# meffmadd/intro-tc-vae

Hardware: AMD Instinct MI355X
Metric: images/sec (64x64x3, z=128, bs=64) intro-TC step (higher is better)
Workload: dtype f32 in/out/accumulate, conv products on split-fp16 MFMA (two scaled fp16 planes, 3 products, fp32-class)

## Files before the change

intro-tc-vae_amd/csrc/abi.hip:

```cpp
#include "conv_shared.h"

#include <vector>

namespace itcv {
thread_local char g_err[512] = "";

struct ProfRec {
  int code;
  double flop;
  hipEvent_t start, stop;
};
static bool g_prof_on = false;
static std::vector<ProfRec> g_prof;

static thread_local int g_prof_depth = 0;
ProfScope::ProfScope(hipStream_t stream, ProfKind kind, int ks, int bm, int up2, int ns, double flop) : st(stream), slot(-1) {
  if (++g_prof_depth > 1 || !g_prof_on) return;
  ProfRec r;
  r.code = kind | (ks << 4) | (bm << 8) | (up2 << 16) | (ns << 20);
  r.flop = flop;
  if (hipEventCreate(&r.start) != hipSuccess || hipEventCreate(&r.stop) != hipSuccess) return;
  g_prof.push_back(r);
  slot = (int)g_prof.size() - 1;
  g_prof_start = r.start, g_prof_stop = r.stop;
}
ProfScope::~ProfScope() {
  if (--g_prof_depth > 0) return;
  if (slot >= 0 && g_prof_start) {
    (void)hipEventDestroy(g_prof[slot].start);
    (void)hipEventDestroy(g_prof[slot].stop);
    g_prof.pop_back();
  }
  g_prof_start = g_prof_stop = nullptr;
}
thread_local hipEvent_t g_prof_start = nullptr, g_prof_stop = nullptr;
Options g_opt;
extern int g_sw_lds_rows, g_sw_max_blocks;
}

extern "C" {
int itcv_abi_version(void) { return ITCV_ABI_VERSION; }

int itcv_set_option(const char* name, int value) {
  if (!name) return itcv::fail("%s: null option name", "itcv_set_option");
  if (!strcmp(name, "band_m16")) {
    if (value != 0 && value != 1) return itcv::fail("%s: band_m16 takes 0 or 1 (got %lld)", "itcv_set_option", value);
    itcv::g_opt.band_m16 = value;
    return 0;
  }
  if (!strcmp(name, "band_persist_blocks")) {
    if (value < 0 || value > 1024) return itcv::fail("%s: band_persist_blocks takes 0..1024 (got %lld)", "itcv_set_option", value);
    itcv::g_opt.band_persist_blocks = value;
    return 0;
  }
  if (!strcmp(name, "wgrad_m16")) {
    if (value != 0 && value != 1) return itcv::fail("%s: wgrad_m16 takes 0 or 1 (got %lld)", "itcv_set_option", value);
    itcv::g_opt.wgrad_m16 = value;
    return 0;
  }
  if (!strcmp(name, "planes_mfma_waves")) {
    if (value != 4 && value != 8) return itcv::fail("%s: planes_mfma_waves takes 4 or 8 (got %lld)", "itcv_set_option", value);
    itcv::g_opt.planes_mfma_waves = value;
    return 0;
  }
  if (!strcmp(name, "sw_lds_rows")) {
    if (value < 0 || value > 4096) return itcv::fail("%s: sw_lds_rows takes 0..4096 (got %lld)", "itcv_set_option", value);
    itcv::g_sw_lds_rows = value;
    return 0;
  }
  if (!strcmp(name, "sw_max_blocks")) {
    if (value < 0 || value > 1024) return itcv::fail("%s: sw_max_blocks takes 0..1024 (got %lld)", "itcv_set_option", value);
    itcv::g_sw_max_blocks = value;
    return 0;
  }
  return itcv::fail("%s: unknown option", "itcv_set_option");
}
int itcv_get_option(const char* name) {
  if (name && !strcmp(name, "band_m16")) return itcv::g_opt.band_m16;
  if (name && !strcmp(name, "band_persist_blocks")) return itcv::g_opt.band_persist_blocks;
  if (name && !strcmp(name, "wgrad_m16")) return itcv::g_opt.wgrad_m16;
  if (name && !strcmp(name, "planes_mfma_waves")) return itcv::g_opt.planes_mfma_waves;
  if (name && !strcmp(name, "sw_lds_rows")) return itcv::g_sw_lds_rows;
  if (name && !strcmp(name, "sw_max_blocks")) return itcv::g_sw_max_blocks;
  return -1;
}
const char* itcv_last_error(void) { return itcv::g_err; }

int itcv_profile_begin(void) {
  itcv::g_prof.clear();
  itcv::g_prof_on = true;
  return 0;
}
int itcv_profile_end(void) {
  itcv::g_prof_on = false;
  for (auto& r : itcv::g_prof) (void)hipEventSynchronize(r.stop);
  return (int)itcv::g_prof.size();
}
int itcv_profile_get(int i, int* code, double* flop, float* ms) {
  if (i < 0 || i >= (int)itcv::g_prof.size()) return itcv::fail("%s: index out of range", "itcv_profile_get");
  const auto& r = itcv::g_prof[i];
  *code = r.code;
  *flop = r.flop;
  if (hipEventElapsedTime(ms, r.start, r.stop) != hipSuccess) *ms = -1.f;
  return 0;
}
int itcv_profile_clear(void) {
  for (auto& r : itcv::g_prof) {
    (void)hipEventDestroy(r.start);
    (void)hipEventDestroy(r.stop);
  }
  itcv::g_prof.clear();
  return 0;
}
}
```

intro-tc-vae_amd/csrc/common.h:

```cpp
#pragma once
#include <hip/hip_runtime.h>
#include <hip/hip_ext.h>
#include <float.h>
#include <math.h>
#include <stdint.h>
#include <stdio.h>
#include <string.h>

#include <type_traits>

#include "../../include/itcv_hip.h"

namespace itcv {

extern thread_local char g_err[512];

inline int fail(const char* fmt, const char* a = "", long long b = 0, long long c = 0) {
  snprintf(g_err, sizeof(g_err), fmt, a, b, c);
  return 1;
}

#define ITCV_CHECK_LAUNCH(name)                                                        \
  do {                                                                                 \
    hipError_t e_ = hipGetLastError();                                                 \
    if (e_ != hipSuccess) return itcv::fail("%s: launch failed: %lld", name, (long long)e_); \
  } while (0)

#define ITCV_REQUIRE(cond, name)                                              \
  do {                                                                        \
    if (!(cond)) return itcv::fail("%s: requirement failed: " #cond, name);   \
  } while (0)

inline bool finite(double x) { return fabs(x) <= DBL_MAX; }

inline int need_pointers(const char* name, bool all) { return all ? 0 : fail("%s: a required pointer is NULL", name); }
inline int need_dim(const char* name, const char* what, long long v, long long lo, long long hi, const char* range) {
  if (v >= lo && v <= hi) return 0;
  char fmt[128];
  snprintf(fmt, sizeof(fmt), "%%s: %s is outside %s", what, range);
  return fail(fmt, name, v);
}
inline int need_stride(const char* name, const char* whose, size_t ld, const char* dim, long long width) {
  if (ld >= (size_t)width) return 0;
  char fmt[128];
  snprintf(fmt, sizeof(fmt), "%%s: %s row stride of %%lld is below %s = %%lld", whose, dim);
  return fail(fmt, name, (long long)ld, width);
}

inline hipStream_t S(void* s) { return reinterpret_cast<hipStream_t>(s); }

__host__ __device__ inline int cdiv(int a, int b) { return (a + b - 1) / b; }
inline size_t cdivz(size_t a, size_t b) { return (a + b - 1) / b; }
inline size_t align_up(size_t a, size_t b) { return cdivz(a, b) * b; }

constexpr int kWave = 64;

inline int stream_grid(size_t n, int per_thread) {
  size_t b = cdivz(cdivz(n, per_thread), 256);
  return (int)(b > 2048 ? 2048 : (b < 1 ? 1 : b));
}

template <typename T>
__device__ __forceinline__ T wave_sum(T v) {
#pragma unroll
  for (int o = 32; o > 0; o >>= 1) v += __shfl_xor(v, o, 64);
  return v;
}
template <typename T>
__device__ __forceinline__ T wave_max(T v) {
#pragma unroll
  for (int o = 32; o > 0; o >>= 1) {
    T u = __shfl_xor(v, o, 64);
    v = u > v ? u : v;
  }
  return v;
}
template <typename T>
__device__ __forceinline__ T wave_min(T v) {
#pragma unroll
  for (int o = 32; o > 0; o >>= 1) {
    T u = __shfl_xor(v, o, 64);
    v = u < v ? u : v;
  }
  return v;
}
template <typename T>
__device__ __forceinline__ T block_sum(T v, T* scratch) {
  const int lane = threadIdx.x & 63, wid = threadIdx.x >> 6, nw = (blockDim.x + 63) >> 6;
  v = wave_sum(v);
  __syncthreads();
  if (lane == 0) scratch[wid] = v;
  __syncthreads();
  T r = 0;
  for (int i = 0; i < nw; ++i) r += scratch[i];
  return r;
}

__device__ __forceinline__ __amdgpu_buffer_rsrc_t make_rsrc(const void* p, uint32_t num_bytes) {
  return __builtin_amdgcn_make_buffer_rsrc(const_cast<void*>(p), 0, num_bytes, 0x00020000);
}
__device__ __forceinline__ float buf_load(__amdgpu_buffer_rsrc_t r, uint32_t byte_off) {
  return __builtin_bit_cast(float, __builtin_amdgcn_raw_buffer_load_b32(r, byte_off, 0, 0));
}
constexpr uint32_t kOOB = 0xFFFFFFFFu;

template <typename T>
__device__ __forceinline__ T fold_strided(T init, const T* __restrict__ p, size_t stride, int n) {
  T s = init;
  int k = 0;
  for (; k + 8 <= n; k += 8) {
    T v[8];
#pragma unroll
    for (int u = 0; u < 8; ++u) v[u] = p[(size_t)(k + u) * stride];
#pragma unroll
    for (int u = 0; u < 8; ++u) s += v[u];
  }
  for (; k + 2 <= n; k += 2) {
    const T v0 = p[(size_t)k * stride], v1 = p[(size_t)(k + 1) * stride];
    s += v0;
    s += v1;
  }
  for (; k < n; ++k) s += p[(size_t)k * stride];
  return s;
}

typedef __bf16 bf16x8 __attribute__((ext_vector_type(8)));
typedef _Float16 f16x8 __attribute__((ext_vector_type(8)));
typedef unsigned int u32x4 __attribute__((ext_vector_type(4)));

struct ScaleRec {
  float scale, inv;
  float pad[2];
};
constexpr int kWeightScaleLog2 = 8;

__host__ __device__ inline float scale_for_bound(float bound) {
  if (!(bound > 0.f) || !(bound < 3.0e38f)) return 1.f;
  int e;
  (void)frexpf(bound, &e);
  int k = 15 - e;
  k = k > 126 ? 126 : (k < -126 ? -126 : k);
  return ldexpf(1.f, k);
}

template <int NS, bool F16 = false>
__device__ __forceinline__ void split8(const float (&v)[8], u32x4 (&out)[NS], float scale = 1.f) {
  if constexpr (F16) {
    static_assert(NS == 2, "fp16 planes come in pairs");
    f16x8 hi, lo;
#pragma unroll
    for (int j = 0; j < 8; ++j) {
      const float r = v[j] * scale;
      const _Float16 h = (_Float16)r;
      hi[j] = h;
      lo[j] = (_Float16)(r - (float)h);
    }
    out[0] = __builtin_bit_cast(u32x4, hi), out[1] = __builtin_bit_cast(u32x4, lo);
  } else {
    bf16x8 pl[NS];
#pragma unroll
    for (int j = 0; j < 8; ++j) {
      float r = v[j];
#pragma unroll
      for (int p = 0; p < NS; ++p) {
        const __bf16 b = (__bf16)r;
        pl[p][j] = b;
        r -= (float)b;
      }
    }
#pragma unroll
    for (int p = 0; p < NS; ++p) out[p] = __builtin_bit_cast(u32x4, pl[p]);
  }
}

typedef float mm_f32x4 __attribute__((ext_vector_type(4)));
typedef float mm_f32x16 __attribute__((ext_vector_type(16)));
template <bool F16>
__device__ __forceinline__ mm_f32x4 mma16x16x32(bf16x8 a, bf16x8 b, mm_f32x4 c) {
  if constexpr (F16)
    return __builtin_amdgcn_mfma_f32_16x16x32_f16(__builtin_bit_cast(f16x8, a), __builtin_bit_cast(f16x8, b), c, 0, 0, 0);
  else
    return __builtin_amdgcn_mfma_f32_16x16x32_bf16(a, b, c, 0, 0, 0);
}
template <bool F16>
__device__ __forceinline__ mm_f32x16 mma32x32x16(bf16x8 a, bf16x8 b, mm_f32x16 c) {
  if constexpr (F16)
    return __builtin_amdgcn_mfma_f32_32x32x16_f16(__builtin_bit_cast(f16x8, a), __builtin_bit_cast(f16x8, b), c, 0, 0, 0);
  else
    return __builtin_amdgcn_mfma_f32_32x32x16_bf16(a, b, c, 0, 0, 0);
}

__device__ __forceinline__ float inv_scale_of(const ScaleRec* r) {
  return __builtin_bit_cast(float, __builtin_amdgcn_readfirstlane(__builtin_bit_cast(int, r->inv)));
}

__device__ __forceinline__ float wave_absmax_of(const float* __restrict__ p, int n) {
  float m = 0.f;
  for (int i = threadIdx.x & 63; i < n; i += 64) m = fmaxf(m, p[i]);
#pragma unroll
  for (int o = 32; o > 0; o >>= 1) m = fmaxf(m, __shfl_xor(m, o, 64));
  return m;
}
constexpr int kAbsmaxParts = 256;

enum ProfKind : int {
  kProfFwd = 0,
  kProfFwdB = 1,
  kProfWgrad = 2,
  kProfWgradB = 3,
  kProfSmallCout = 4,
  kProfSmallCin = 5,
  kProfFwdP = 6,
  kProfWgradP = 7,
  kProfFwdBand = 8,
  kProfFwdBandPersist = 9,
  kProfSmallCoutP = 10,
  kProfSmallCinMfma = 11,
  kProfWgrad5 = 12,
  kProfBnFwd = 13,
  kProfBnBwd = 14,
};
struct ProfScope {
  hipStream_t st;
  int slot;
  ProfScope(hipStream_t stream, ProfKind kind, int ks, int bm, int up2, int ns, double flop);
  ~ProfScope();
};
extern thread_local hipEvent_t g_prof_start, g_prof_stop;

template <typename K, typename... Args>
inline void launch_timed(K kernel, dim3 grid, dim3 block, size_t lds, hipStream_t st, Args... args) {
  if (g_prof_start) {
    hipExtLaunchKernelGGL(kernel, grid, block, lds, st, g_prof_start, g_prof_stop, 0, args...);
    g_prof_start = nullptr;
  } else {
    hipLaunchKernelGGL(kernel, grid, block, lds, st, args...);
  }
}

template <auto Kernel, typename... Args>
inline void launch_lds(dim3 grid, dim3 block, size_t lds, hipStream_t st, Args... args) {
  static size_t have = 0;
  if (have < lds) {
    (void)hipFuncSetAttribute(reinterpret_cast<const void*>(Kernel), hipFuncAttributeMaxDynamicSharedMemorySize, (int)lds);
    have = lds;
  }
  launch_timed(Kernel, grid, block, lds, st, args...);
}

template <int N, typename F>
inline void pick(int v, F&& f) {
  if constexpr (N > 1) {
    if (v == N - 1) return f(std::integral_constant<int, N - 1>{});
    return pick<N - 1>(v, f);
  } else {
    f(std::integral_constant<int, 0>{});
  }
}
template <int V0, int... Vs, typename F>
inline void pick_of(int v, F&& f) {
  if constexpr (sizeof...(Vs) > 0) {
    if (v != V0) return pick_of<Vs...>(v, f);
  }
  f(std::integral_constant<int, V0>{});
}

}
```

intro-tc-vae_amd/csrc/conv_igemm.hip:

```cpp
#include <float.h>

#include "conv_shared.h"

namespace itcv {



constexpr uint32_t kOobBase = 0x80000000u;

__device__ __forceinline__ float buf_load_s(__amdgpu_buffer_rsrc_t r, uint32_t voff, uint32_t soff) {
  return __builtin_bit_cast(float, __builtin_amdgcn_raw_buffer_load_b32(r, voff, __builtin_amdgcn_readfirstlane(soff), 0));
}

__host__ __device__ inline int tile_rows_for(int M) { return M <= 32 ? 32 : (M <= 64 ? 64 : 128); }

struct ConvArgs {
  const float* x;
  const float* wp;
  const float* bias;
  float* y;
  int B, Ci, H, W, Co;
  int Cip, Mp, N;
  int mt, nt;
  int ktiles, ktiles_per_split, cpt;
// ... 1368 lines not shown
    const int lw = wid - 8;
    const int Hs = UP2 ? H / 2 : H, Ws = UP2 ? Wi / 2 : Wi, HWs = Hs * Ws;
    const int Co8 = a.Co >> 3, Ci8 = a.Ci >> 3, dh = dhi - 1;
    const u32x4* zero = &g_zero_chunk;
    const int hp = (lw & 1) * 64 + lane;
    const bool hp_active = hp < NP;
    const int R = hp / WP, w = hp - R * WP - 1;

    auto issue = [&](int st, int stage) {
      const uint32_t sbase = smem_base + (uint32_t)(stage * SSZ) * 16u;
      {
        const int g = st * 64 + lane, b = g / HW, pix = g - b * HW;
#pragma unroll
        for (int j = 0; j < 2 * ACH / NLW; ++j) {
          const int qq = j * NLW + lw, pl = qq / ACH, c8 = qq % ACH;
          const int gc8 = (co0 >> 3) + c8;
          const u32x4* src = a.dyp + ((size_t)pl * a.dyplane + ((size_t)b * Co8 + gc8) * HW + pix);
          lds_dma16(gc8 < Co8 ? src : zero, sbase + (uint32_t)((pl * ACH + c8) * PXA) * 16u);
        }
      }
      {
        const int gr = (st >> wsh) * NR + R, b = gr >> a.h_shift, h = gr & (H - 1), hh = h + dh;
        const int wi = ((st & ((1 << wsh) - 1)) << 6) + w;
        const bool valid = (unsigned)wi < (unsigned)Wi && (unsigned)hh < (unsigned)H;
        const int spix = UP2 ? (hh >> 1) * Ws + (wi >> 1) : hh * Wi + wi;
#pragma unroll
        for (int j = 0; j < 4 * BCH / NLW; ++j) {
          const int qq = (j * NLW + lw) >> 1, pl = qq / BCH, c8 = qq % BCH;
          const int gc8 = (ci0 >> 3) + c8;
          const u32x4* src = a.xp + ((size_t)pl * a.xplane + ((size_t)b * Ci8 + gc8) * HWs + spix);
          if (hp_active)
            lds_dma16((valid && gc8 < Ci8) ? src : zero,
                      sbase + (uint32_t)(ASZ + (pl * BCH + c8) * PXB + (lw & 1) * 64) * 16u);
        }
      }
    };
    constexpr int PST = 2 * ACH / NLW + 4 * BCH / NLW;
    issue(s0, 0);
    if (NST == 3 && s0 + 1 < s1) {
      issue(s0 + 1, 1);
      wait_vmcnt<PST>();
    } else {
      wait_vmcnt<0>();
    }
    __builtin_amdgcn_s_barrier();
    int stage = NST - 1;
    for (int st = s0; st < s1; ++st) {
      if (st + NST - 1 < s1) {
        issue(st + NST - 1, stage);
        if (NST == 3) wait_vmcnt<PST>();
        else wait_vmcnt<0>();
      } else {
        wait_vmcnt<0>();
      }
      if (++stage == NST) stage = 0;
      __builtin_amdgcn_s_barrier();
    }
    return;
  }

  const int kh = wid / (8 / KH), w8 = wid % (8 / KH);
  const int wm = w8 / WNn, wn = w8 % WNn;
  const int G = lane >> 4, i16 = lane & 15, q = i16 >> 2, pp = i16 & 3, half = G >> 1, rb = G & 1;
  const int l31 = lane & 31;
  if constexpr (M16) {
    typedef float f32x4m __attribute__((ext_vector_type(4)));
    constexpr int KP32 = 2 / KH;
    f32x4m acc[3][TNw][2][2];
#pragma unroll
    for (int tp = 0; tp < 3; ++tp)
#pragma unroll
      for (int j = 0; j < TNw; ++j)
#pragma unroll
        for (int bi = 0; bi < 2; ++bi)
#pragma unroll
          for (int bj = 0; bj < 2; ++bj) acc[tp][j][bi][bj] = f32x4m{0.f, 0.f, 0.f, 0.f};
    if (s0 < s1) {
      const uint32_t aoff = (uint32_t)(((4 * wm + (pp >> 1)) * PXA + G * 8 + q) * 16 + (pp & 1) * 8);
      const uint32_t boff = (uint32_t)((ASZ + (4 * wn * TNw + (pp >> 1)) * PXB) * 16 + (pp & 1) * 8);
      uint32_t hidx[2 * KP32];
#pragma unroll
      for (int u = 0; u < 2 * KP32; ++u) {
        const int k = ((u >> 1) + kh * KP32) * 32 + G * 8 + (u & 1) * 4 + q;
        hidx[u] = (uint32_t)(((k >> LOG2W) * WP + (k & (W - 1)) + 1) * 16);
      }
      __builtin_amdgcn_s_barrier();
      int stage = 0;
      for (int st = s0; st < s1; ++st) {
        const uint32_t sb = smem_base + (uint32_t)(stage * SSZ) * 16u;
        if constexpr (TNw == 1) {
          bf16x8 af[2][2][2], bfr[2][2];
          auto fetch_a = [&](int kk, int kb) {
#pragma unroll
            for (int bi = 0; bi < 2; ++bi)
#pragma unroll
              for (int pl = 0; pl < 2; ++pl) {
                const uint32_t ad = sb + aoff + (uint32_t)((pl * ACH + 2 * bi) * PXA * 16 + (kh * KP32 + kk) * 512);
                tr_read8(af[kb][bi][pl], ad, ad + 64);
              }
          };
          auto fetch_b = [&](int u, int ub) {
            const int kk = u / 6, tp = (u % 6) >> 1, bj = u & 1;
#pragma unroll
            for (int pl = 0; pl < 2; ++pl) {
              const uint32_t bd = sb + boff + (uint32_t)((pl * BCH + 2 * bj) * PXB * 16 + (tp - 1) * 16);
              tr_read8(bfr[ub][pl], bd + hidx[kk * 2], bd + hidx[kk * 2 + 1]);
            }
          };
          constexpr int NU = KP32 * 6;
          fetch_a(0, 0);
          fetch_b(0, 0);
#pragma unroll
          for (int u = 0; u < NU; ++u) {
            const int kk = u / 6, tp = (u % 6) >> 1, bj = u & 1, ub = u & 1, kb = kk & 1;
            if (u + 1 < NU) {
              if ((u + 1) % 6 == 0) fetch_a(kk + 1, kb ^ 1);
              fetch_b(u + 1, ub ^ 1);
            }
#pragma unroll
            for (int bi = 0; bi < 2; ++bi) {
              f32x4m c = acc[tp][0][bi][bj];
              c = mma16x16x32<F16>(af[kb][bi][0], bfr[ub][1], c);
              c = mma16x16x32<F16>(af[kb][bi][1], bfr[ub][0], c);
              c = mma16x16x32<F16>(af[kb][bi][0], bfr[ub][0], c);
              acc[tp][0][bi][bj] = c;
            }
          }
        } else {
#pragma unroll
        for (int kk = 0; kk < KP32; ++kk) {
          bf16x8 af[2][2];
#pragma unroll
          for (int bi = 0; bi < 2; ++bi)
#pragma unroll
            for (int pl = 0; pl < 2; ++pl) {
              const uint32_t ad = sb + aoff + (uint32_t)((pl * ACH + 2 * bi) * PXA * 16 + (kh * KP32 + kk) * 512);
              tr_read8(af[bi][pl], ad, ad + 64);
            }
#pragma unroll
          for (int tp = 0; tp < 3; ++tp)
#pragma unroll
            for (int j = 0; j < TNw; ++j)
#pragma unroll
              for (int bj = 0; bj < 2; ++bj) {
                bf16x8 bfr[2];
#pragma unroll
                for (int pl = 0; pl < 2; ++pl) {
                  const uint32_t bd = sb + boff + (uint32_t)((pl * BCH + 4 * j + 2 * bj) * PXB * 16 + (tp - 1) * 16);
                  tr_read8(bfr[pl], bd + hidx[kk * 2], bd + hidx[kk * 2 + 1]);
                }
#pragma unroll
                for (int bi = 0; bi < 2; ++bi) {
                  f32x4m c = acc[tp][j][bi][bj];
                  c = mma16x16x32<F16>(af[bi][0], bfr[1], c);
                  c = mma16x16x32<F16>(af[bi][1], bfr[0], c);
                  c = mma16x16x32<F16>(af[bi][0], bfr[0], c);
                  acc[tp][j][bi][bj] = c;
                }
              }
        }
        }
        if (++stage == NST) stage = 0;
        asm volatile("s_waitcnt lgkmcnt(0)" ::: "memory");
        __builtin_amdgcn_s_barrier();
      }
    }
    const float oscale = F16 ? inv_scale_of(a.xscale) * inv_scale_of(a.dyscale) : 1.f;
#pragma unroll
    for (int j = 0; j < TNw; ++j)
#pragma unroll
      for (int bj = 0; bj < 2; ++bj) {
        const int ci = ci0 + 32 * (wn * TNw + j) + 16 * bj + i16;
        if (ci >= a.Ci) continue;
#pragma unroll
        for (int tp = 0; tp < 3; ++tp) {
          float* out = a.slab + ((size_t)((split * KH + kh) * 9 + dhi * 3 + tp) * a.Co) * a.Ci + ci;
#pragma unroll
          for (int bi = 0; bi < 2; ++bi)
#pragma unroll
            for (int r = 0; r < 4; ++r) {
              const int co = co0 + 32 * wm + 16 * bi + 4 * G + r;
              if (co < a.Co) out[(size_t)co * a.Ci] = F16 ? acc[tp][j][bi][bj][r] * oscale : acc[tp][j][bi][bj][r];
            }
        }
      }
    return;
  }
  f32x16 acc[3][TNw];
#pragma unroll
  for (int tp = 0; tp < 3; ++tp)
#pragma unroll
    for (int j = 0; j < TNw; ++j)
#pragma unroll
      for (int r = 0; r < 16; ++r) acc[tp][j][r] = 0.f;
  if (s0 < s1) {
    const uint32_t aoff = (uint32_t)(((4 * wm + 2 * rb + (pp >> 1)) * PXA + half * 8 + q) * 16 + (pp & 1) * 8);
    const uint32_t boff = (uint32_t)((ASZ + (4 * wn * TNw + 2 * rb + (pp >> 1)) * PXB) * 16 + (pp & 1) * 8);
    uint32_t hidx16[2 * KPW];
#pragma unroll
    for (int u = 0; u < 2 * KPW; ++u) {
      const int k = ((u >> 1) + kh * KPW) * 16 + half * 8 + (u & 1) * 4 + q;
      hidx16[u] = (uint32_t)(((k >> LOG2W) * WP + (k & (W - 1)) + 1) * 16);
    }
    __builtin_amdgcn_s_barrier();
    int stage = 0;
    const long long dbg_c0 = ITCV_DBG(a) ? clock64() : 0;
    for (int st = s0; st < s1; ++st) {
      const uint32_t sb = smem_base + (uint32_t)(stage * SSZ) * 16u;
      if constexpr (TNw == 1) {
        bf16x8 af[2][2], bfr[2][3][2];
        auto fetch = [&](int kk, int bufi) {
#pragma unroll
          for (int pl = 0; pl < 2; ++pl) {
            const uint32_t ad = sb + aoff + (uint32_t)(pl * ACH * PXA * 16 + (kh * KPW + kk) * 256);
            tr_read8(af[bufi][pl], ad, ad + 64);
          }
#pragma unroll
          for (int tp = 0; tp < 3; ++tp)
#pragma unroll
            for (int pl = 0; pl < 2; ++pl) {
              const uint32_t bd = sb + boff + (uint32_t)(pl * BCH * PXB * 16 + (tp - 1) * 16);
              tr_read8(bfr[bufi][tp][pl], bd + hidx16[kk * 2], bd + hidx16[kk * 2 + 1]);
            }
        };
        fetch(0, 0);
#pragma unroll
        for (int kk = 0; kk < KPW; ++kk) {
          const int cur = kk & 1;
          if (kk + 1 < KPW) fetch(kk + 1, cur ^ 1);
#pragma unroll
          for (int tp = 0; tp < 3; ++tp) {
            f32x16 c = acc[tp][0];
            c = mma32x32x16<F16>(af[cur][0], bfr[cur][tp][1], c);
            c = mma32x32x16<F16>(af[cur][1], bfr[cur][tp][0], c);
            c = mma32x32x16<F16>(af[cur][0], bfr[cur][tp][0], c);
            acc[tp][0] = c;
          }
          if (kk == 0) __builtin_amdgcn_sched_group_barrier(0x100, 16, 0);
          if (kk + 1 < KPW) {
#pragma unroll
            for (int r = 0; r < 8; ++r) {
              __builtin_amdgcn_sched_group_barrier(0x008, 1, 0);
              __builtin_amdgcn_sched_group_barrier(0x100, 2, 0);
            }
            __builtin_amdgcn_sched_group_barrier(0x008, 1, 0);
          } else {
            __builtin_amdgcn_sched_group_barrier(0x008, 9, 0);
          }
        }
      } else {
      static_assert(TNw == 1 || KH == 1, "k-halves only with one accumulator column per wave");
#pragma unroll
      for (int kk = 0; kk < 4; ++kk) {
        bf16x8 af[2];
#pragma unroll
        for (int pl = 0; pl < 2; ++pl) {
          const uint32_t ad = sb + aoff + (uint32_t)(pl * ACH * PXA * 16 + kk * 256);
          tr_read8(af[pl], ad, ad + 64);
        }
#pragma unroll
        for (int tp = 0; tp < 3; ++tp)
#pragma unroll
          for (int j = 0; j < TNw; ++j) {
            bf16x8 bfr[2];
#pragma unroll
            for (int pl = 0; pl < 2; ++pl) {
              const uint32_t bd = sb + boff + (uint32_t)((pl * BCH + 4 * j) * PXB * 16 + (tp - 1) * 16);
              tr_read8(bfr[pl], bd + hidx16[kk * 2], bd + hidx16[kk * 2 + 1]);
            }
            f32x16 c = acc[tp][j];
            c = mma32x32x16<F16>(af[0], bfr[1], c);
            c = mma32x32x16<F16>(af[1], bfr[0], c);
            c = mma32x32x16<F16>(af[0], bfr[0], c);
            acc[tp][j] = c;
          }
      }
      }
      if (++stage == NST) stage = 0;
      asm volatile("s_waitcnt lgkmcnt(0)" ::: "memory");
      __builtin_amdgcn_s_barrier();
    }
    if (ITCV_DBG(a) && t == 0 && blockIdx.x == 0) {
      a.slab[0] = (float)(clock64() - dbg_c0), a.slab[1] = (float)(s1 - s0);
      return;
    }
  }
  const float oscale = F16 ? inv_scale_of(a.xscale) * inv_scale_of(a.dyscale) : 1.f;
#pragma unroll
  for (int j = 0; j < TNw; ++j) {
    const int ci = ci0 + 32 * (wn * TNw + j) + l31;
    if (ci >= a.Ci) continue;
#pragma unroll
    for (int tp = 0; tp < 3; ++tp) {
      float* out = a.slab + ((size_t)((split * KH + kh) * 9 + dhi * 3 + tp) * a.Co) * a.Ci + ci;
#pragma unroll
      for (int r = 0; r < 16; ++r) {
        const int co = co0 + 32 * wm + (r & 3) + 8 * (r >> 2) + 4 * (lane >> 5);
        if (co < a.Co) out[(size_t)co * a.Ci] = F16 ? acc[tp][j][r] * oscale : acc[tp][j][r];
      }
    }
  }
}

template <int SG, bool F16 = false>
__global__ __launch_bounds__(256) void conv_wgrad5_planes_kernel(const float* __restrict__ sm, const u32x4* __restrict__ tp,
                                                                float* __restrict__ slab, int B, int CS, int H, int W,
                                                                int rows_per_job, int njobs, size_t plane_stride,
                                                                const float* __restrict__ sm_amax) {
  constexpr int PXS = 68;
  constexpr int RSZ = 2 * 8 * PXS;
  __shared__ u32x4 rows[4][RSZ];
  const int lane = threadIdx.x & 63, wv = threadIdx.x >> 6;
  const int job = blockIdx.x * 4 + wv;
  if (job >= njobs) return;
  const int jobs_per_img = (H + rows_per_job - 1) / rows_per_job;
  const int b = job / jobs_per_img, h_lo = (job - b * jobs_per_img) * rows_per_job, h_hi = min(H, h_lo + rows_per_job);
  const size_t HW = (size_t)H * W;
  const int n = lane & 15, kg = lane >> 4;
  const int cs = n / 5, dw = n - cs * 5;
  const bool row_used = cs < CS;
  const int i16 = lane & 15, q = i16 >> 2, pp = i16 & 3;
  const uint32_t rbase = lds_addr(rows[wv]);
  float sscale = 1.f, oscale = 1.f;
  if constexpr (F16) {
    if (sm_amax) sscale = scale_for_bound(wave_absmax_of(sm_amax, kAbsmaxParts));
    oscale = inv_scale_of(reinterpret_cast<const ScaleRec*>(tp + 2 * plane_stride)) / sscale;
  }
  f32x4_t acc[5][4];
#pragma unroll
  for (int dh = 0; dh < 5; ++dh)
#pragma unroll
    for (int nt = 0; nt < 4; ++nt) acc[dh][nt] = f32x4_t{0.f, 0.f, 0.f, 0.f};

  for (int h = h_lo; h < h_hi; ++h) {
   for (int seg = 0; seg < W; seg += 64) {
    const int segw = min(64, W - seg);
    asm volatile("s_waitcnt lgkmcnt(0)" ::: "memory");
    if (lane < segw) {
#pragma unroll
      for (int pl = 0; pl < 2; ++pl)
#pragma unroll
        for (int c8 = 0; c8 < 8; ++c8)
          rows[wv][(pl * 8 + c8) * PXS + lane] =
              tp[(size_t)pl * plane_stride + ((size_t)b * 8 + c8) * HW + (size_t)h * W + seg + lane];
    }
    asm volatile("s_waitcnt vmcnt(0) lgkmcnt(0)" ::: "memory");
    for (int w0 = 0; w0 < segw; w0 += 32) {
      bf16x8 bfr[4][2];
#pragma unroll
      for (int nt = 0; nt < 4; ++nt)
#pragma unroll
        for (int pl = 0; pl < 2; ++pl) {
          const uint32_t ad = rbase + (uint32_t)(((pl * 8 + 2 * nt + (pp >> 1)) * PXS + w0 + 8 * kg + q) * 16 + (pp & 1) * 8);
          tr_read8(bfr[nt][pl], ad, ad + 64);
        }
      float sv[5][8];
      const int ws0 = seg + w0 + 8 * kg + SG * (dw - 2);
      const float* spc = sm + ((size_t)b * CS + (row_used ? cs : 0)) * HW;
#pragma unroll
      for (int dh = 0; dh < 5; ++dh) {
        const int hs = h + SG * (dh - 2);
        const float* sp = spc + (size_t)min(max(hs, 0), H - 1) * W;
#pragma unroll
        for (int j = 0; j < 8; ++j) sv[dh][j] = sp[min(max(ws0 + j, 0), W - 1)];
      }
#pragma unroll
      for (int dh = 0; dh < 5; ++dh) {
        const int hs = h + SG * (dh - 2);
        float v[8];
        const bool hok = row_used && (unsigned)hs < (unsigned)H;
#pragma unroll
        for (int j = 0; j < 8; ++j) v[j] = (hok && (unsigned)(ws0 + j) < (unsigned)W) ? sv[dh][j] : 0.f;
        u32x4 ap[2];
        split8<2, F16>(v, ap, sscale);
        const bf16x8 a0 = __builtin_bit_cast(bf16x8, ap[0]), a1 = __builtin_bit_cast(bf16x8, ap[1]);
#pragma unroll
        for (int nt = 0; nt < 4; ++nt) {
          f32x4_t c = acc[dh][nt];
          c = mma16x16x32<F16>(a0, bfr[nt][1], c);
          c = mma16x16x32<F16>(a1, bfr[nt][0], c);
          c = mma16x16x32<F16>(a0, bfr[nt][0], c);
          acc[dh][nt] = c;
        }
      }
    }
   }
  }
  float* out = slab + (size_t)job * 16 * 5 * 64;
#pragma unroll
  for (int dh = 0; dh < 5; ++dh)
#pragma unroll
    for (int nt = 0; nt < 4; ++nt)
#pragma unroll
      for (int i = 0; i < 4; ++i) out[((4 * kg + i) * 5 + dh) * 64 + nt * 16 + n] = F16 ? acc[dh][nt][i] * oscale : acc[dh][nt][i];
}

__global__ __launch_bounds__(256) void wgrad5_reduce(const float* __restrict__ slab, float* __restrict__ dwt, int CS,
                                                    int njobs, int stem, int accumulate) {
  __shared__ float part[16][17];
  const int e = threadIdx.x & 15, g = threadIdx.x >> 4;
  const int total = CS * 5 * 5 * 64, i = blockIdx.x * 16 + e;
  float s = 0.f;
  int dst = 0;
  if (i < total) {
    const int cb = i & 63, r = i >> 6, dh = r % 5, m = r / 5, cs = m / 5, dwi = m - cs * 5;
    const float* p = slab + (size_t)((m * 5 + dh) * 64 + cb);
    for (int k = g; k < njobs; k += 16 * 8) {
      float v[8];
#pragma unroll
      for (int u = 0; u < 8; ++u) v[u] = p[(size_t)min(k + 16 * u, njobs - 1) * (16 * 5 * 64)];
#pragma unroll
      for (int u = 0; u < 8; ++u) s += (k + 16 * u < njobs) ? v[u] : 0.f;
    }
    dst = stem ? ((cb * CS + cs) * 5 + dh) * 5 + dwi : ((cs * 64 + cb) * 5 + dh) * 5 + dwi;
  }
  part[g][e] = s;
  __syncthreads();
  if (g == 0 && i < total) {
    float t = accumulate ? dwt[dst] : 0.f;
#pragma unroll
    for (int k = 0; k < 16; ++k) t += part[k][e];
    dwt[dst] = t;
  }
}

struct WgReduceDesc {
  const float* slab[4];
  float* dw;
  int splits[4];
  int nsrc, coci, accumulate, block0, nblocks, fine;
};
static_assert(sizeof(WgReduceDesc) == 80, "WgReduceDesc layout is part of the ABI (itcv_wgrad_reduce_desc_bytes)");

__device__ __forceinline__ void wgrad_reduce_tile(const WgReduceDesc& d, int tile) {
  const int e = (tile * 256 + (int)threadIdx.x) * 4;
  if (e >= d.coci) return;
  const size_t plane = (size_t)d.coci, stride = 9 * plane;
  float* dwp = d.dw + (size_t)e * 9;
  const bool vec = ((size_t)dwp & 15) == 0;
  float tot[36];
  if (d.accumulate) {
    if (vec) {
#pragma unroll
      for (int q = 0; q < 9; ++q) {
        const float4 t = reinterpret_cast<const float4*>(dwp)[q];
        tot[4 * q] = t.x, tot[4 * q + 1] = t.y, tot[4 * q + 2] = t.z, tot[4 * q + 3] = t.w;
      }
    } else {
#pragma unroll
      for (int q = 0; q < 36; ++q) tot[q] = dwp[q];
    }
  } else {
#pragma unroll
    for (int q = 0; q < 36; ++q) tot[q] = 0.f;
  }
  for (int k = 0; k < d.nsrc; ++k) {
    const float* p = d.slab[k] + e;
    float acc[36];
#pragma unroll
    for (int q = 0; q < 36; ++q) acc[q] = 0.f;
    int sl = 0;
    for (; sl + 2 <= d.splits[k]; sl += 2) {
      float4 v[2][9];
#pragma unroll
      for (int u = 0; u < 2; ++u)
#pragma unroll
        for (int tp = 0; tp < 9; ++tp) v[u][tp] = *reinterpret_cast<const float4*>(p + (size_t)(sl + u) * stride + (size_t)tp * plane);
#pragma unroll
      for (int u = 0; u < 2; ++u)
#pragma unroll
        for (int tp = 0; tp < 9; ++tp)
          acc[tp] += v[u][tp].x, acc[9 + tp] += v[u][tp].y, acc[18 + tp] += v[u][tp].z, acc[27 + tp] += v[u][tp].w;
    }
    if (sl < d.splits[k]) {
      float4 v[9];
#pragma unroll
      for (int tp = 0; tp < 9; ++tp) v[tp] = *reinterpret_cast<const float4*>(p + (size_t)sl * stride + (size_t)tp * plane);
#pragma unroll
      for (int tp = 0; tp < 9; ++tp) acc[tp] += v[tp].x, acc[9 + tp] += v[tp].y, acc[18 + tp] += v[tp].z, acc[27 + tp] += v[tp].w;
    }
#pragma unroll
    for (int q = 0; q < 36; ++q) tot[q] += acc[q];
  }
  if (vec) {
#pragma unroll
    for (int q = 0; q < 9; ++q) reinterpret_cast<float4*>(dwp)[q] = make_float4(tot[4 * q], tot[4 * q + 1], tot[4 * q + 2], tot[4 * q + 3]);
  } else {
#pragma unroll
    for (int q = 0; q < 36; ++q) dwp[q] = tot[q];
  }
}

constexpr int kWgFineSplits = 64;
constexpr int kWgFineTiles = 4;
constexpr int kWgFineElems = 16 * kWgFineTiles, kWgFineOut = 9 * kWgFineElems;
constexpr int kWgPartFloats = 16 * kWgFineOut;
static_assert(kWgFineElems == 64 && kWgFineOut <= 3 * 256, "lane mapping of wgrad_reduce_tile_fine");

template <int U>
__device__ __forceinline__ void wgrad_fine_add(float (&acc)[36], const float* p, int sl, size_t stride, size_t plane) {
  float4 v[U][9];
#pragma unroll
  for (int u = 0; u < U; ++u)
#pragma unroll
    for (int tp = 0; tp < 9; ++tp) v[u][tp] = *reinterpret_cast<const float4*>(p + (size_t)(sl + u) * stride + (size_t)tp * plane);
#pragma unroll
  for (int u = 0; u < U; ++u)
#pragma unroll
    for (int tp = 0; tp < 9; ++tp)
      acc[tp] += v[u][tp].x, acc[9 + tp] += v[u][tp].y, acc[18 + tp] += v[u][tp].z, acc[27 + tp] += v[u][tp].w;
}

__device__ __forceinline__ void wgrad_reduce_tile_fine(const WgReduceDesc& d, int item, float* part ) {
  const int lane = threadIdx.x & 63, wave = threadIdx.x >> 6, el4 = lane & 15, sg = wave * 4 + (lane >> 4);
  const int e0 = item * kWgFineElems, e = e0 + el4 * 4;
  const bool live = e < d.coci;
  const size_t plane = (size_t)d.coci, stride = 9 * plane;
  const int nout = min(kWgFineOut, (d.coci - e0) * 9);
  float* dwp = d.dw + (size_t)e0 * 9;
  float tot[3];
#pragma unroll
  for (int r = 0; r < 3; ++r) {
    const int o = (int)threadIdx.x + 256 * r;
    tot[r] = (d.accumulate && o < nout) ? dwp[o] : 0.f;
  }
  for (int k = 0; k < d.nsrc; ++k) {
    const int q = (d.splits[k] + 15) >> 4;
    const int s0 = sg * q, s1 = min(s0 + q, d.splits[k]);
    float acc[36];
#pragma unroll
    for (int f = 0; f < 36; ++f) acc[f] = 0.f;
    if (live) {
      const float* p = d.slab[k] + e;
      int sl = s0;
      for (; sl + 4 <= s1; sl += 4) wgrad_fine_add<4>(acc, p, sl, stride, plane);
      if (sl + 2 <= s1) wgrad_fine_add<2>(acc, p, sl, stride, plane), sl += 2;
      if (sl < s1) wgrad_fine_add<1>(acc, p, sl, stride, plane);
    }
    if (k) __syncthreads();
    float4* pw = reinterpret_cast<float4*>(part + sg * kWgFineOut + el4 * 36);
#pragma unroll
    for (int c = 0; c < 9; ++c) pw[c] = make_float4(acc[4 * c], acc[4 * c + 1], acc[4 * c + 2], acc[4 * c + 3]);
    __syncthreads();
#pragma unroll
    for (int r = 0; r < 3; ++r) {
      const int o = (int)threadIdx.x + 256 * r;
      if (o < kWgFineOut) {
        float sum = 0.f;
#pragma unroll
        for (int g = 0; g < 16; ++g) sum += part[g * kWgFineOut + o];
        tot[r] += sum;
      }
    }
  }
#pragma unroll
  for (int r = 0; r < 3; ++r) {
    const int o = (int)threadIdx.x + 256 * r;
    if (o < nout) dwp[o] = tot[r];
  }
}
static inline bool wgrad_reduce_fine(const int* splits, int nsrc) {
  for (int k = 0; k < nsrc; ++k)
    if (splits[k] >= kWgFineSplits) return true;
  return false;
}
static inline int wgrad_reduce_blocks(int coci, bool fine) { return fine ? cdiv(coci, 16) : cdiv(coci, 1024); }

__global__ __launch_bounds__(256) void wgrad_p_reduce(const float* __restrict__ slab, float* __restrict__ dw, int CoCi,
                                                     int splits, int accumulate, int fine) {
  __shared__ __attribute__((aligned(16))) float part[kWgPartFloats];
  WgReduceDesc d;
  d.slab[0] = slab, d.dw = dw, d.splits[0] = splits, d.nsrc = 1, d.coci = CoCi, d.accumulate = accumulate;
  if (fine) wgrad_reduce_tile_fine(d, blockIdx.x, part);
  else wgrad_reduce_tile(d, blockIdx.x);
}

constexpr int kWgMaxDesc = 96;
__device__ __forceinline__ int wgrad_desc_items(const WgReduceDesc& d) {
  return d.fine ? (d.nblocks + kWgFineTiles - 1) / kWgFineTiles : d.nblocks;
}
__global__ __launch_bounds__(256) void wgrad_p_reduce_many(const WgReduceDesc* __restrict__ tab, int n) {
  __shared__ __attribute__((aligned(16))) float part[kWgPartFloats];
  __shared__ WgReduceDesc s_desc[kWgMaxDesc];
  __shared__ int s_cost[kWgMaxDesc], s_items[kWgMaxDesc], s_ord[kWgMaxDesc], s_first[kWgMaxDesc + 1];
  const int tid = threadIdx.x;
  {
    const int* src = reinterpret_cast<const int*>(tab);
    int* dst = reinterpret_cast<int*>(s_desc);
    for (int i = tid; i < n * (int)(sizeof(WgReduceDesc) / 4); i += blockDim.x) dst[i] = src[i];
  }
  __syncthreads();
  if (tid < n) {
    const WgReduceDesc& d = s_desc[tid];
    int slices = 0;
    for (int k = 0; k < d.nsrc; ++k) slices += d.splits[k];
    s_cost[tid] = slices * (d.fine ? kWgFineElems : 1024);
    s_items[tid] = wgrad_desc_items(d);
  }
  __syncthreads();
  if (tid < n) {
    const int mine = s_cost[tid];
    int rank = 0, first = 0;
    for (int j = 0; j < n; ++j) {
      const int cj = s_cost[j];
      if (cj > mine || (cj == mine && j < tid)) ++rank, first += s_items[j];
    }
    s_ord[rank] = tid, s_first[rank] = first;
    if (rank == n - 1) s_first[n] = first + s_items[tid];
  }
  __syncthreads();
  const int total = s_first[n];
  int r = 0;
  for (int w = (int)blockIdx.x; w < total; w += (int)gridDim.x) {
    while (s_first[r + 1] <= w) ++r;
    const WgReduceDesc& d = s_desc[s_ord[r]];
    if (d.fine) {
      wgrad_reduce_tile_fine(d, w - s_first[r], part);
      __syncthreads();
    } else {
      wgrad_reduce_tile(d, w - s_first[r]);
    }
  }
}

__global__ __launch_bounds__(256) void splitk_reduce_wgrad_small(const float* __restrict__ slab, float* __restrict__ dw,
                                                                 int Co, int Ci, int KK, int Cip, int cb, int Np,
                                                                 size_t slab_stride, int splits, int accumulate,
                                                                 int swapped) {
  __shared__ float part[16][17];
  const int e = threadIdx.x & 15, g = threadIdx.x >> 4;
  const size_t total = (size_t)Co * Ci * KK, i = (size_t)blockIdx.x * 16 + e;
  float s = 0.f;
  if (i < total) {
    int tap = (int)(i % KK);
    const size_t r = i / KK;
    int ci = (int)(r % Ci), co = (int)(r / Ci);
    if (swapped) {
      const int tmp = ci;
      ci = co, co = tmp, tap = KK - 1 - tap;
    }
    int col;
    if (cb == 128) {
      const int per_tap = Cip / 128;
      col = (tap * per_tap + ci / 128) * 128 + (ci & 127);
    } else {
      const int tpb = 128 / cb;
      col = (tap / tpb) * 128 + (tap % tpb) * cb + ci;
    }
    const float* p = slab + (size_t)co * Np + col;
    for (int k = g; k < splits; k += 16) s += p[(size_t)k * slab_stride];
  }
  part[g][e] = s;
  __syncthreads();
  if (g == 0 && i < total) {
    float t = accumulate ? dw[i] : 0.f;
#pragma unroll
    for (int k = 0; k < 16; ++k) t += part[k][e];
    dw[i] = t;
  }
}

__global__ void splitk_reduce_wgrad(const float* __restrict__ slab, float* __restrict__ dw, int Co, int Ci, int KK,
                                    int Cip, int cb, int Np, size_t slab_stride, int splits, int accumulate,
                                    int swapped) {
  const size_t total = (size_t)Co * Ci * KK;
  for (size_t i = (size_t)blockIdx.x * blockDim.x + threadIdx.x; i < total; i += (size_t)gridDim.x * blockDim.x) {
    int tap = (int)(i % KK);
    const size_t r = i / KK;
    int ci = (int)(r % Ci), co = (int)(r / Ci);
    if (swapped) {
      const int tmp = ci;
      ci = co, co = tmp, tap = KK - 1 - tap;
    }
    int col;
    if (cb == 128) {
      const int per_tap = Cip / 128;
      col = (tap * per_tap + ci / 128) * 128 + (ci & 127);
    } else {
      const int tpb = 128 / cb;
      col = (tap / tpb) * 128 + (tap % tpb) * cb + ci;
    }
    dw[i] = fold_strided(accumulate ? dw[i] : 0.f, slab + (size_t)co * Np + col, slab_stride, splits);
  }
}

__global__ __launch_bounds__(256) void bias_grad_partial(const float* __restrict__ dy, double* __restrict__ part, int B,
                                                         int C, int HW, int splits) {
  __shared__ double scratch[4];
  const int c = blockIdx.x, s = blockIdx.y;
  const size_t total = (size_t)B * HW;
  const size_t chunk = (total + splits - 1) / splits;
  const size_t beg = (size_t)s * chunk, end = beg + chunk < total ? beg + chunk : total;
  double acc = 0.0;
  for (size_t i = beg + threadIdx.x; i < end; i += 256) {
    const size_t b = i / HW, hw = i - b * HW;
    acc += (double)dy[(b * C + c) * HW + hw];
  }
  acc = block_sum(acc, scratch);
  if (threadIdx.x == 0) part[(size_t)s * C + c] = acc;
}
__global__ void bias_grad_combine(const double* __restrict__ part, float* __restrict__ db, int C, int splits,
                                  int accumulate) {
  const int c = blockIdx.x * blockDim.x + threadIdx.x;
  if (c >= C) return;
  const double s = fold_strided(0.0, part + c, (size_t)C, splits);
  db[c] = (accumulate ? db[c] : 0.f) + (float)s;
}

static inline int pad_to(int c, int m) { return (c + m - 1) / m * m; }
static inline int pad16(int c) { return pad_to(c, 16); }
static inline int pad32(int c) { return pad_to(c, 32); }

static int check_ws(const char* name, const void* ws, size_t ws_bytes, size_t need) {
  if (need && (!ws || ws_bytes < need)) return fail("%s: workspace too small (need %lld bytes)", name, (long long)need);
  return 0;
}

static int reduce_fwd_splits(const char* name, const void* ws, const float* bias, float* y, size_t out_elems, int splits,
                             int HW, int Co, hipStream_t st) {
  if (splits <= 1) return 0;
  const int blocks = (int)(cdivz(out_elems, 256) < 2048 ? cdivz(out_elems, 256) : 2048);
  hipLaunchKernelGGL(splitk_reduce_fwd, dim3(blocks), dim3(256), 0, st, static_cast<const float*>(ws), bias, y, out_elems,
                     out_elems, splits, HW, Co);
  ITCV_CHECK_LAUNCH(name);
  return 0;
}

struct FwdRule {
  int kchunk;
  bool rows32;
  int split_target;
};
constexpr FwdRule kFwdF32 = {16, true, 512};
constexpr FwdRule kFwdSplit = {32, false, 256};

struct FwdPlan {
  int bm, bn, mt, nt, cip, ktiles, splits, kps;
  size_t ws_need;
};
static FwdPlan plan_fwd(const FwdRule& r, int B, int Ci, int H, int W, int Co, int KS) {
  FwdPlan p;
  const long long N = (long long)B * H * W;
  p.bm = r.rows32 ? tile_rows_for(Co) : (Co <= 64 ? 64 : 128);
  p.bn = p.bm == 128 ? 128 : 256;
  p.mt = cdiv(Co, p.bm);
  p.nt = (int)((N + p.bn - 1) / p.bn);
  p.cip = pad_to(Ci, r.kchunk);
  p.ktiles = KS * KS * (p.cip / r.kchunk);
  const int tiles = p.mt * p.nt;
  int splits = 1;
  if (tiles < 192 && p.ktiles >= 8) {
    splits = cdiv(r.split_target, tiles);
    if (splits > p.ktiles / 4) splits = p.ktiles / 4;
    if (splits > 64) splits = 64;
    if (splits < 1) splits = 1;
  }
  p.kps = cdiv(p.ktiles, splits);
  p.splits = cdiv(p.ktiles, p.kps);
  p.ws_need = p.splits > 1 ? (size_t)p.splits * B * Co * H * W * sizeof(float) : 0;
  return p;
}

static FwdPlanP plan_fwd_planes(int B, int Ci, int H, int W, int Co, int KS, int ns, bool stats) {
  FwdPlanP p;
  if (plan_fwd_band(p, B, Ci, H, W, Co, KS, ns)) {
    const int ids = cdiv(p.nt, 8) * 8 * p.mt, pb = g_opt.band_persist_blocks;
    p.path = p.bn == 128 ? FwdPath::WidePersistent : ((!stats && pb > 0 && ids > pb) ? FwdPath::BandPersistent : FwdPath::Band);
    p.stat_tiles = (p.splits == 1 && p.bn == 256) ? p.nt : 0;
  } else {
    const FwdPlan t = plan_fwd(kFwdSplit, B, Ci, H, W, Co, KS);
    memset(&p, 0, sizeof(p));
    p.path = FwdPath::Planes128;
    p.bm = t.bm, p.bn = t.bn, p.mt = t.mt, p.nt = t.nt, p.splits = t.splits, p.ktiles = t.ktiles, p.kps = t.kps;
  }
  p.ws_need = p.splits > 1 ? (size_t)p.splits * B * Co * H * W * sizeof(float) : 0;
  return p;
}

static inline bool wgrad_swapped(int Ci, int Co) { return Co <= 4 && Ci > 4; }

struct WgPlan {
  int bm, cb, cip, mt, nt, tiles, ktiles, splits, kps;
  int grid;
  size_t slab;
  size_t ws_need;
};

static WgPlan plan_wgrad(int B, int Ci, int H, int W, int Co, int KS, int min_bm = 32) {
  WgPlan p;
  const long long Ktot = (long long)B * H * W;
  p.bm = tile_rows_for(Co);
  if (p.bm < min_bm) p.bm = min_bm;
  p.cb = Ci <= 4 ? 4 : (Ci <= 16 ? 16 : (Ci <= 32 ? 32 : (Ci <= 64 ? 64 : 128)));
  p.cip = p.cb < 128 ? p.cb : (Ci + 127) / 128 * 128;
  p.nt = p.cb == 128 ? KS * KS * (p.cip / 128) : cdiv(KS * KS, 128 / p.cb);
  const int tiles = cdiv(Co, tile_rows_for(Co)) * p.nt;
  p.ktiles = (int)((Ktot + 31) / 32);
  int splits = cdiv(768, tiles);
  if (p.cb == 4) splits = cdiv(256, tiles);
  if (splits > p.ktiles / 8) splits = p.ktiles / 8;
  if (splits > 256) splits = 256;
  if (splits < 1) splits = 1;
  p.kps = cdiv(p.ktiles, splits);
  p.splits = cdiv(p.ktiles, p.kps);
  p.mt = cdiv(Co, p.bm);
  p.tiles = p.mt * p.nt;
  p.grid = cdiv(p.splits, 8) * 8 * p.tiles;
  p.slab = (size_t)Co * p.nt * 128;
  p.ws_need = (size_t)p.splits * p.slab * sizeof(float);
  return p;
}

static WgPlan plan_wgrad_call(WgradArgs& a, const float* x, const float* dy, void* ws, int B, int Ci, int H, int W, int Co,
                              int KS, int up2, bool swap, int min_bm) {
  if (swap) {
    const float* tp = x;
    x = dy, dy = tp;
    const int tc = Ci;
    Ci = Co, Co = tc;
  }
  const WgPlan p = plan_wgrad(B, Ci, H, W, Co, KS, min_bm);
  a.x = x, a.dy = dy;
  a.out = static_cast<float*>(ws);
  a.B = B, a.Ci = Ci, a.H = H, a.W = W, a.Co = Co;
  a.Cip = p.cip;
  a.Np = p.nt * 128;
  a.Ktot = B * H * W;
  a.mt = p.mt, a.nt = p.nt, a.tiles = p.tiles;
  a.ktiles = p.ktiles, a.ktiles_per_split = p.kps, a.splits = p.splits;
  a.w_shift = log2_exact(W), a.hw_shift = log2_exact(H * W);
  a.x_bytes = (uint32_t)((size_t)B * Ci * (up2 ? (H / 2) * (W / 2) : H * W) * sizeof(float));
  a.dy_bytes = (uint32_t)((size_t)B * Co * H * W * sizeof(float));
  a.slab_stride = p.slab;
  return p;
}

struct WgPlanP {
  int bm, bn, tiles_m, tiles_n, steps, splits, sps;
  int kh;
  int slabs;
  int groups, blocks;
  size_t ws_need;
};
static WgPlanP plan_wgrad_p(int B, int Ci, int H, int W, int Co) {
  WgPlanP p;
  p.bm = (Co <= 64 && Ci >= 128) ? 64 : 128;
  p.bn = 8192 / p.bm;
  p.kh = 1;
  if (Co <= 64 && Ci <= 64) p.bm = 64, p.bn = 64, p.kh = 2;
  if (p.bm == 128 && Ci >= 512 && Co >= 256 && W >= 8) p.bn = 128;
  p.tiles_m = cdiv(Co, p.bm), p.tiles_n = cdiv(Ci, p.bn);
  p.steps = (int)(((long long)B * H * W) / 64);
  const int T = p.tiles_m * p.tiles_n * 3;
  constexpr int target = 256;
  int splits = (8 * (target / 24)) / (T / 3);
  if (splits > p.steps / 2) splits = p.steps / 2;
  if (splits < 1) splits = 1;
  p.sps = cdiv(p.steps, splits);
  p.splits = cdiv(p.steps, p.sps);
  p.slabs = p.splits * p.kh;
  p.groups = p.tiles_m * p.tiles_n * p.splits;
  p.blocks = cdiv(p.groups, 8) * 24;
  p.ws_need = (size_t)p.slabs * 9 * Co * Ci * sizeof(float);
  return p;
}

template <typename F>
static inline void pick_fmt(int fmt, F&& f) {
  pick<3>(fmt == ITCV_PLANES_F16X2 ? 2 : (fmt == 2 ? 0 : 1), [&](auto i) {
    f(std::integral_constant<int, i.value == 1 ? 3 : 2>{}, std::integral_constant<bool, i.value == 2>{});
  });
}

template <int BM>
struct IgemmTile {
  static constexpr int BN = BM == 128 ? 128 : 256, WM = BM == 128 ? 2 : 1, WN = BM == 128 ? 2 : 4;
};

static void launch_fwd(const ConvArgs& a, const FwdPlan& p, int KS, int up2, hipStream_t st) {
  const dim3 grid(cdiv(a.nt, 8) * 8 * a.mt, p.splits);
  pick_of<1, 3, 5>(KS, [&](auto ks) {
    pick_of<32, 64, 128>(p.bm, [&](auto bm) {
      pick<2>(up2 ? 1 : 0, [&](auto u) {
        pick<2>((a.Ci & 15) ? 1 : 0, [&](auto tail) {
          using T = IgemmTile<bm.value>;
          launch_timed((conv_fwd_kernel<ks.value, bm.value, T::BN, T::WM, T::WN, u.value != 0, tail.value != 0>), grid,
                       dim3(T::WM * T::WN * 64), 0, st, a);
        });
      });
    });
  });
}

static void launch_fwd_b(const ConvArgsB& a, const FwdPlan& p, int KS, int up2, int ns, hipStream_t st) {
  const dim3 grid(cdiv(a.nt, 8) * 8 * a.mt, p.splits);
  pick_of<1, 3>(KS, [&](auto ks) {
    pick_of<2, 3>(ns, [&](auto nsc) {
      pick_of<64, 128>(p.bm, [&](auto bm) {
        pick<2>(up2 ? 1 : 0, [&](auto u) {
          using T = IgemmTile<bm.value>;
          launch_timed((conv_fwd_bf16s_ws_kernel<ks.value, bm.value, T::BN, T::WM, T::WN, u.value != 0, nsc.value>), grid,
                       dim3(512), 0, st, a);
        });
      });
    });
  });
}

static void launch_fwd_p(const ConvArgsP& a, const FwdPlanP& p, int KS, int up2, int fmt, hipStream_t st) {
  const dim3 grid(cdiv(a.nt, 8) * 8 * a.mt, p.splits);
  const bool m16 = fmt == ITCV_PLANES_F16X2 || (fmt == 2 && band_m16());
  const bool waves8 = m16 && p.bm == 128 && g_opt.planes_mfma_waves == 8;
  pick_of<1, 3>(KS, [&](auto ks) {
    pick_fmt(fmt, [&](auto nsc, auto f16) {
      pick_of<64, 128>(p.bm, [&](auto bm) {
        pick<2>(up2 ? 1 : 0, [&](auto u) {
          pick<2>(waves8 ? 1 : 0, [&](auto w8) {
            pick<2>(m16 ? 1 : 0, [&](auto m) {
              constexpr int NS = nsc.value, BM = bm.value, NSTAGE = NS == 2 ? 3 : 2;
              constexpr bool F16 = f16.value, M16 = m.value != 0, W8 = w8.value != 0;
              using T = IgemmTile<BM>;
              constexpr int WN = W8 ? 4 : T::WN;
              constexpr size_t lds = (size_t)NSTAGE * NS * 4 * (BM + T::BN) * 16;
              static_assert(lds <= 160 * 1024, "LDS ring too large");
              if constexpr ((M16 || !F16) && !(M16 && NS == 3) && !(W8 && !(NS == 2 && BM == 128)))
                launch_lds<conv_fwd_bf16p_kernel<ks.value, BM, T::BN, T::WM, WN, u.value != 0, NS, NSTAGE, M16, F16>>(
                    grid, dim3(64 * (T::WM * WN + 4)), lds, st, a);
            });
          });
        });
      });
    });
  });
}

static void launch_wgrad(const WgradArgs& a, const WgPlan& p, int KS, int up2, hipStream_t st) {
  pick_of<1, 3, 5>(KS, [&](auto ks) {
    pick<2>(up2 ? 1 : 0, [&](auto u) {
      pick_of<4, 16, 32, 64, 128>(p.cb, [&](auto cb) {
        pick_of<32, 64, 128>(p.bm, [&](auto bm) {
          using T = IgemmTile<bm.value>;
          launch_timed((conv_wgrad_kernel<ks.value, bm.value, cb.value, T::WM, T::WN, u.value != 0, 1>), dim3(p.grid),
                       dim3(256), 0, st, a);
        });
      });
    });
  });
}

static void launch_wgrad_b(const WgradArgs& a, const WgPlan& p, int KS, int ns, hipStream_t st) {
  pick_of<1, 3>(KS, [&](auto ks) {
    pick_of<2, 3>(ns, [&](auto nsc) {
      pick_of<32, 64, 128>(p.cb, [&](auto cb) {
        pick_of<64, 128>(p.bm, [&](auto bm) {
          using T = IgemmTile<bm.value>;
          launch_timed((conv_wgrad_bf16s_kernel<ks.value, bm.value, cb.value, T::WM, T::WN, nsc.value>), dim3(p.grid),
                       dim3(256), 0, st, a);
        });
      });
    });
  });
}

static void launch_wgrad_p(const WgradArgsP& a, const WgPlanP& p, int lw, int up2, int f16, hipStream_t st) {
  const bool m16 = g_opt.wgrad_m16 != 0;
  pick_of<2, 3, 4, 5, 6>(lw, [&](auto lwc) {
    pick<2>(f16 ? 1 : 0, [&](auto f) {
      pick_of<64, 128>(p.bm, [&](auto bm) {
        pick_of<64, 128>(p.bn, [&](auto bn) {
          pick<2>(up2 ? 1 : 0, [&](auto u) {
            pick<2>(m16 ? 1 : 0, [&](auto m) {
              constexpr int LOG2W = lwc.value, BM = bm.value, BN = bn.value, KH = (BM == 64 && BN == 64) ? 2 : 1;
              constexpr int W = 1 << LOG2W, NP = (64 >> LOG2W) * (W + 2), PXB = ((NP + 11) / 16) * 16 + 4;
              constexpr size_t stage_bytes = (size_t)(2 * (BM / 8) * 68 + 2 * (BN / 8) * PXB) * 16;
              constexpr int NST = 3 * stage_bytes <= 160 * 1024 ? 3 : 2;
              constexpr size_t lds = NST * stage_bytes;
              constexpr int NLW = 4;
              if constexpr (lds <= 160 * 1024)
                launch_lds<conv_wgrad_bf16p_kernel<LOG2W, u.value != 0, BM, BN, NST, NLW, KH, f.value != 0, m.value != 0>>(
                    dim3(p.blocks), dim3(512 + 64 * NLW), lds, st, a);
            });
          });
        });
      });
    });
  });
}

static int check_dims(const char* name, int B, int Ci, int H, int W, int Co, int KS) {
  if (!(KS == 1 || KS == 3 || KS == 5)) return fail("%s: kernel size must be 1, 3 or 5 (got %lld)", name, KS);
  if (B <= 0 || Ci <= 0 || H <= 0 || W <= 0 || Co <= 0) return fail("%s: empty or negative dimension", name);
  const long long in_elems = (long long)B * pad16(Ci) * H * W, out_elems = (long long)B * Co * H * W;
  if (in_elems >= (1LL << 29) || out_elems >= (1LL << 29))
    return fail("%s: tensor too large for 31-bit buffer offsets (%lld / %lld elements)", name, in_elems, out_elems);
  return 0;
}

constexpr int kBiasSplitsMax = 256;
static inline int bias_splits(int B, int C, int HW) {
  int s = cdiv(1024, C);
  const size_t maxs = cdivz((size_t)B * HW, 2048);
  if ((size_t)s > maxs) s = (int)maxs;
  if (s > kBiasSplitsMax) s = kBiasSplitsMax;
  return s < 1 ? 1 : s;
}
}

using namespace itcv;

// ... 349 lines not shown
  size_t n = plan_wgrad(B, Ci, H, W, Co, KS).ws_need;
  if (wgrad_swapped(Ci, Co)) {
    const size_t m = plan_wgrad(B, Co, H, W, Ci, KS).ws_need;
    if (m > n) n = m;
  }
  return n;
}

int itcv_conv2d_wgrad(const float* x, const float* dy, float* dw, int B, int Ci, int H, int W, int Co, int KS,
                      int up2, int accumulate, void* ws, size_t ws_bytes, void* stream) {
  if (int e = check_dims("itcv_conv2d_wgrad", B, Ci, H, W, Co, KS)) return e;
  ITCV_REQUIRE(x && dy && dw, "itcv_conv2d_wgrad");
  if (up2) ITCV_REQUIRE(H % 2 == 0 && W % 2 == 0, "itcv_conv2d_wgrad(up2)");
  const bool swapped = !up2 && wgrad_swapped(Ci, Co);
  WgradArgs a;
  const WgPlan p = plan_wgrad_call(a, x, dy, ws, B, Ci, H, W, Co, KS, up2, swapped, 32);
  if (int e = check_ws("itcv_conv2d_wgrad", ws, ws_bytes, p.ws_need)) return e;
  hipStream_t st = S(stream);
  {
    ProfScope prof(st, kProfWgrad, KS, p.bm, up2 ? 1 : 0, 0, 2.0 * B * H * W * (double)Co * Ci * KS * KS);
    launch_wgrad(a, p, KS, up2, st);
  }
  ITCV_CHECK_LAUNCH("itcv_conv2d_wgrad");
  const size_t dw_elems = (size_t)Co * Ci * KS * KS;
  const int blocks = (int)(cdivz(dw_elems, 256) < 2048 ? cdivz(dw_elems, 256) : 2048);
  if (dw_elems <= 65536 && p.splits >= 32)
    hipLaunchKernelGGL(splitk_reduce_wgrad_small, dim3((int)cdivz(dw_elems, 16)), dim3(256), 0, st,
                       static_cast<const float*>(ws), dw, Co, Ci, KS * KS, p.cip, p.cb, a.Np, p.slab, p.splits,
                       accumulate, swapped ? 1 : 0);
  else
    hipLaunchKernelGGL(splitk_reduce_wgrad, dim3(blocks), dim3(256), 0, st, static_cast<const float*>(ws), dw, Co, Ci,
                       KS * KS, p.cip, p.cb, a.Np, p.slab, p.splits, accumulate, swapped ? 1 : 0);
  ITCV_CHECK_LAUNCH("itcv_conv2d_wgrad(reduce)");
  return 0;
}

int itcv_conv2d_wgrad_bf16s_supported(int Ci, int H, int W, int Co, int KS) {
  return (KS == 1 || KS == 3) && Ci % 32 == 0 && W % 8 == 0 && Co >= 33 && H > 0;
}

int itcv_conv2d_wgrad_bf16s(const float* x, const float* dy, float* dw, int B, int Ci, int H, int W, int Co, int KS,
                            int ns, int accumulate, void* ws, size_t ws_bytes, void* stream) {
  if (int e = check_dims("itcv_conv2d_wgrad_bf16s", B, Ci, H, W, Co, KS)) return e;
  ITCV_REQUIRE(x && dy && dw && (ns == 2 || ns == 3), "itcv_conv2d_wgrad_bf16s");
  if (!itcv_conv2d_wgrad_bf16s_supported(Ci, H, W, Co, KS))
    return fail("%s: shape not supported by the split-bf16 kernel (Ci %% 32, W %% 8, Co > 32, KS 1/3)",
                "itcv_conv2d_wgrad_bf16s");
  WgradArgs a;
  const WgPlan p = plan_wgrad_call(a, x, dy, ws, B, Ci, H, W, Co, KS, 0, false, 64);
  if (int e = check_ws("itcv_conv2d_wgrad_bf16s", ws, ws_bytes, p.ws_need)) return e;
  hipStream_t st = S(stream);
  {
    ProfScope prof(st, kProfWgradB, KS, p.bm, 0, ns, 2.0 * B * H * W * (double)Co * Ci * KS * KS);
    launch_wgrad_b(a, p, KS, ns, st);
  }
  ITCV_CHECK_LAUNCH("itcv_conv2d_wgrad_bf16s");
  const size_t dw_elems = (size_t)Co * Ci * KS * KS;
  const int blocks = (int)(cdivz(dw_elems, 256) < 2048 ? cdivz(dw_elems, 256) : 2048);
  hipLaunchKernelGGL(splitk_reduce_wgrad, dim3(blocks), dim3(256), 0, st, static_cast<const float*>(ws), dw, Co, Ci,
                     KS * KS, p.cip, p.cb, a.Np, p.slab, p.splits, accumulate, 0);
  ITCV_CHECK_LAUNCH("itcv_conv2d_wgrad_bf16s(reduce)");
  return 0;
}

int itcv_conv2d_wgrad_bf16p_supported(int B, int Ci, int H, int W, int Co, int KS) {
  if (KS != 3 || B <= 0 || Ci < 8 || Co < 8 || (Ci & 7) || (Co & 7)) return 0;
  if (log2_exact(W) < 2 || W > 256 || log2_exact(H) < 0) return 0;
  const long long px = (long long)B * H * W;
  if (px % 64) return 0;
  if (H * W < 64 && 64 % (H * W)) return 0;
  return 1;
}

size_t itcv_conv2d_wgrad_bf16p_workspace(int B, int Ci, int H, int W, int Co, int KS) {
  if (!itcv_conv2d_wgrad_bf16p_supported(B, Ci, H, W, Co, KS)) return 0;
  return plan_wgrad_p(B, Ci, H, W, Co).ws_need;
}

int itcv_conv2d_wgrad_bf16p(const void* xplanes, const void* dyplanes, float* dw, int B, int Ci, int H, int W, int Co,
                            int KS, int up2, int ns, int accumulate, void* ws, size_t ws_bytes, void* stream) {
  if (int e = check_dims("itcv_conv2d_wgrad_bf16p", B, Ci, H, W, Co, KS)) return e;
  ITCV_REQUIRE(xplanes && dyplanes && dw && (ns == 2 || ns == ITCV_PLANES_F16X2), "itcv_conv2d_wgrad_bf16p");
  const int f16 = ns == ITCV_PLANES_F16X2;
  if (!itcv_conv2d_wgrad_bf16p_supported(B, Ci, H, W, Co, KS))
    return fail("%s: shape not supported (KS 3, W a power of two in 4..256, H a power of two, C %% 8)", "itcv_conv2d_wgrad_bf16p");
  if (up2) ITCV_REQUIRE(H % 2 == 0 && W % 2 == 0, "itcv_conv2d_wgrad_bf16p(up2)");
  const WgPlanP p = plan_wgrad_p(B, Ci, H, W, Co);
  if (int e = check_ws("itcv_conv2d_wgrad_bf16p", ws, ws_bytes, p.ws_need)) return e;
  WgradArgsP a;
  a.xp = static_cast<const u32x4*>(xplanes), a.dyp = static_cast<const u32x4*>(dyplanes);
  a.slab = static_cast<float*>(ws);
  a.B = B, a.Ci = Ci, a.H = H, a.W = W, a.Co = Co;
  a.tiles_m = p.tiles_m, a.tiles_n = p.tiles_n;
  a.steps = p.steps, a.steps_per_split = p.sps, a.splits = p.splits;
  a.h_shift = log2_exact(H);
  a.wseg_shift = W > 64 ? log2_exact(W) - 6 : 0;
  a.xplane = (size_t)B * (Ci / 8) * (up2 ? (H / 2) * (W / 2) : H * W);
  a.dyplane = (size_t)B * (Co / 8) * H * W;
  a.xscale = f16 ? reinterpret_cast<const ScaleRec*>(a.xp + 2 * a.xplane) : nullptr;
  a.dyscale = f16 ? reinterpret_cast<const ScaleRec*>(a.dyp + 2 * a.dyplane) : nullptr;
#ifdef ITCV_DIAG
  a.debug = (diag_ablate() & 64) ? 1 : 0;
#endif
  hipStream_t st = S(stream);
  a.groups = p.groups;
  {
    ProfScope prof(st, kProfWgradP, log2_exact(W), p.bm, up2 ? 1 : 0, ns, 2.0 * B * H * W * (double)Co * Ci * KS * KS);
    launch_wgrad_p(a, p, log2_exact(W), up2, f16, st);
  }
  ITCV_CHECK_LAUNCH("itcv_conv2d_wgrad_bf16p");
  if (accumulate == 2) return 0;
  const int coci = Co * Ci;
  const bool fine = wgrad_reduce_fine(&p.slabs, 1);
  const int rblocks = fine ? cdiv(wgrad_reduce_blocks(coci, true), kWgFineTiles) : wgrad_reduce_blocks(coci, false);
  hipLaunchKernelGGL(wgrad_p_reduce, dim3(rblocks), dim3(256), 0, st, static_cast<const float*>(ws),
                     dw, coci, p.slabs, accumulate, fine ? 1 : 0);
  ITCV_CHECK_LAUNCH("itcv_conv2d_wgrad_bf16p(reduce)");
  return 0;
}

int itcv_conv2d_wgrad_bf16p_slabs(int B, int Ci, int H, int W, int Co, int KS) {
  if (!itcv_conv2d_wgrad_bf16p_supported(B, Ci, H, W, Co, KS)) return 0;
  return plan_wgrad_p(B, Ci, H, W, Co).slabs;
}
size_t itcv_wgrad_reduce_desc_bytes(void) { return sizeof(WgReduceDesc); }
int itcv_wgrad_reduce_desc(void* host_desc, const float* const* slabs, const int* splits, int nsrc, float* dw, int Co, int Ci,
                           int accumulate, int block0) {
  if (!(host_desc && slabs && splits && nsrc >= 1 && nsrc <= 4 && dw && Co > 0 && Ci > 0 && block0 >= 0)) {
    fail("%s: bad argument (1..4 slab sources, dw, Co/Ci > 0, block0 >= 0)", "itcv_wgrad_reduce_desc");
    return -1;
  }
  WgReduceDesc d;
  memset(&d, 0, sizeof(d));
  for (int k = 0; k < nsrc; ++k) {
    if (!slabs[k] || splits[k] < 1) {
      fail("%s: null slab or non-positive slice count", "itcv_wgrad_reduce_desc");
      return -1;
    }
    d.slab[k] = slabs[k], d.splits[k] = splits[k];
  }
  d.nsrc = nsrc, d.dw = dw, d.coci = Co * Ci, d.accumulate = accumulate ? 1 : 0, d.block0 = block0;
  d.fine = wgrad_reduce_fine(d.splits, nsrc) ? 1 : 0;
  d.nblocks = wgrad_reduce_blocks(d.coci, d.fine != 0);
  memcpy(host_desc, &d, sizeof(d));
  return d.nblocks;
}
int itcv_wgrad_reduce_max_descs(void) { return kWgMaxDesc; }
int itcv_wgrad_reduce_many(const void* dev_table, int n, int total_blocks, void* stream) {
  ITCV_REQUIRE(dev_table && n > 0 && total_blocks > 0, "itcv_wgrad_reduce_many");
  if (n > kWgMaxDesc) return fail("%s: at most %d descriptors per table (itcv_wgrad_reduce_max_descs)", "itcv_wgrad_reduce_many", kWgMaxDesc);
  const int grid = total_blocks < 2048 ? total_blocks : 2048;
  hipLaunchKernelGGL(wgrad_p_reduce_many, dim3(grid), dim3(256), 0, S(stream), static_cast<const WgReduceDesc*>(dev_table), n);
  ITCV_CHECK_LAUNCH("itcv_wgrad_reduce_many");
  return 0;
}

}

namespace itcv {
struct GemmPlan {
  int mt, nt, ktiles, splits, kps;
};
static GemmPlan plan_gemm64(int M, int N, int K) {
  GemmPlan p;
  p.mt = cdiv(M, 64), p.nt = cdiv(N, 64), p.ktiles = cdiv(K, 32);
  const int tiles = p.mt * p.nt;
  int splits = 1;
  if (tiles < 128 && p.ktiles >= 4) {
    splits = cdiv(256, tiles);
    if (splits > 32) splits = 32;
    if (splits > p.ktiles / 2) splits = p.ktiles / 2;
    if (splits < 1) splits = 1;
  }
  p.kps = cdiv(p.ktiles, splits);
  p.splits = cdiv(p.ktiles, p.kps);
  return p;
}
static size_t gemm64_ws(int M, int N, int K) {
  const GemmPlan p = plan_gemm64(M, N, K);
  return p.splits > 1 ? (size_t)p.splits * M * N * sizeof(float) : 0;
}
static int run_gemm64(const char* name, const float* A, const float* B, const float* bias, float* C, int M, int N,
                      int K, long long sam, long long sak, long long sbk, long long sbn, int accumulate, void* ws,
                      size_t ws_bytes, hipStream_t st, int epi = 0, const float* mask = nullptr, long long ldm = 0,
                      float slope = 0.f) {
  const GemmPlan p = plan_gemm64(M, N, K);
  const size_t need = p.splits > 1 ? (size_t)p.splits * M * N * sizeof(float) : 0;
  if (need && (!ws || ws_bytes < need)) return fail("%s: workspace too small (need %lld bytes)", name, (long long)need);
  GemmArgs a;
  a.A = A, a.B = B, a.bias = bias;
  a.C = p.splits > 1 ? static_cast<float*>(ws) : C;
  a.M = M, a.N = N, a.K = K;
  a.sam = sam, a.sak = sak, a.sbk = sbk, a.sbn = sbn;
  a.mt = p.mt, a.nt = p.nt, a.ktiles = p.ktiles, a.ktiles_per_split = p.kps;
  a.slab_stride = p.splits > 1 ? (size_t)M * N : 0;
  a.accumulate = p.splits > 1 ? 0 : accumulate;
  a.mask = mask, a.ldm = ldm, a.slope = slope;
  dim3 grid(p.mt * p.nt, p.splits), blk(256);
  const bool akc = sak == 1, bkc = sbk == 1;
  const auto al16 = [](const void* q) { return (reinterpret_cast<uintptr_t>(q) & 15) == 0; };
  const bool vec = al16(A) && al16(B) && al16(a.C) && N % 4 == 0 &&
                   (akc ? (K % 4 == 0 && sam % 4 == 0) : (sam == 1 && M % 4 == 0 && sak % 4 == 0)) &&
                   (bkc ? (K % 4 == 0 && sbn % 4 == 0) : (sbn == 1 && sbk % 4 == 0));
  if (vec && epi == 1 && p.splits == 1) hipLaunchKernelGGL((gemm64_vec_kernel<true, true, 1>), grid, blk, 0, st, a);
  else if (vec && epi == 2 && p.splits == 1) hipLaunchKernelGGL((gemm64_vec_kernel<true, false, 2>), grid, blk, 0, st, a);
  else if (vec && akc && bkc) hipLaunchKernelGGL((gemm64_vec_kernel<true, true>), grid, blk, 0, st, a);
  else if (vec && akc) hipLaunchKernelGGL((gemm64_vec_kernel<true, false>), grid, blk, 0, st, a);
  else if (vec && bkc) hipLaunchKernelGGL((gemm64_vec_kernel<false, true>), grid, blk, 0, st, a);
  else if (vec) hipLaunchKernelGGL((gemm64_vec_kernel<false, false>), grid, blk, 0, st, a);
  else if (epi == 1 && p.splits == 1) hipLaunchKernelGGL((gemm64_kernel<true, true, 1>), grid, blk, 0, st, a);
  else if (epi == 2 && p.splits == 1) hipLaunchKernelGGL((gemm64_kernel<true, false, 2>), grid, blk, 0, st, a);
  else if (akc && bkc) hipLaunchKernelGGL((gemm64_kernel<true, true>), grid, blk, 0, st, a);
  else if (akc) hipLaunchKernelGGL((gemm64_kernel<true, false>), grid, blk, 0, st, a);
  else if (bkc) hipLaunchKernelGGL((gemm64_kernel<false, true>), grid, blk, 0, st, a);
  else hipLaunchKernelGGL((gemm64_kernel<false, false>), grid, blk, 0, st, a);
  ITCV_CHECK_LAUNCH(name);
  if (p.splits > 1 && epi) {
    const size_t total = (size_t)M * N;
    const dim3 rgrid((int)(cdivz(total, 256) < 1024 ? cdivz(total, 256) : 1024));
    if (epi == 1)
      hipLaunchKernelGGL(gemm64_reduce_epi<1>, rgrid, dim3(256), 0, st, static_cast<const float*>(ws), bias, C, total, N,
                         p.splits, mask, ldm, slope);
    else
      hipLaunchKernelGGL(gemm64_reduce_epi<2>, rgrid, dim3(256), 0, st, static_cast<const float*>(ws), bias, C, total, N,
                         p.splits, mask, ldm, slope);
    ITCV_CHECK_LAUNCH(name);
  } else if (p.splits > 1) {
    const size_t total = (size_t)M * N;
    hipLaunchKernelGGL(gemm64_reduce, dim3((int)(cdivz(total, 256) < 1024 ? cdivz(total, 256) : 1024)), dim3(256), 0, st,
                       static_cast<const float*>(ws), bias, C, total, N, p.splits, accumulate);
    ITCV_CHECK_LAUNCH(name);
  }
  return 0;
}
}

extern "C" {

size_t itcv_linear_workspace(int B, int K, int N) {
  if (B <= 0 || K <= 0 || N <= 0) return 0;
  size_t n = gemm64_ws(B, N, K);
  const size_t d = gemm64_ws(B, K, N), w = gemm64_ws(N, K, B);
  if (d > n) n = d;
  if (w > n) n = w;
  return n;
}
int itcv_linear_fwd(const float* x, const float* w, const float* bias, float* y, int B, int K, int N, void* ws,
                    size_t ws_bytes, void* stream) {
  ITCV_REQUIRE(x && w && y && B > 0 && K > 0 && N > 0, "itcv_linear_fwd");
  return run_gemm64("itcv_linear_fwd", x, w, bias, y, B, N, K, K, 1, 1, K, 0, ws, ws_bytes, S(stream));
}
int itcv_linear_dgrad(const float* dy, const float* w, float* dx, int B, int K, int N, void* ws, size_t ws_bytes,
                      void* stream) {
  ITCV_REQUIRE(dy && w && dx && B > 0 && K > 0 && N > 0, "itcv_linear_dgrad");
  return run_gemm64("itcv_linear_dgrad", dy, w, nullptr, dx, B, K, N, N, 1, K, 1, 0, ws, ws_bytes, S(stream));
}
int itcv_linear_wgrad(const float* dy, const float* x, float* dw, int B, int K, int N, int accumulate, void* ws,
                      size_t ws_bytes, void* stream) {
  ITCV_REQUIRE(dy && x && dw && B > 0 && K > 0 && N > 0, "itcv_linear_wgrad");
  return run_gemm64("itcv_linear_wgrad", dy, x, nullptr, dw, N, K, B, 1, N, K, 1, accumulate, ws, ws_bytes, S(stream));
}

int itcv_linear_lrelu_fwd(const float* x, size_t ldx, const float* w, const float* bias, float* y, int B, int K, int N,
                          float slope, void* ws, size_t ws_bytes, void* stream) {
  ITCV_REQUIRE(x && w && y && B > 0 && K > 0 && N > 0, "itcv_linear_lrelu_fwd");
  ITCV_REQUIRE(ldx >= (size_t)K && slope > 0.f && slope <= FLT_MAX, "itcv_linear_lrelu_fwd");
  return run_gemm64("itcv_linear_lrelu_fwd", x, w, bias, y, B, N, K, (long long)ldx, 1, 1, K, 0, ws, ws_bytes, S(stream), 1,
                    nullptr, 0, slope);
}
int itcv_linear_dgrad_lrelu(const float* dy, size_t lddy, const float* w, const float* y_prev, size_t ldy, float* dx,
                            int B, int K, int N, float slope, void* ws, size_t ws_bytes, void* stream) {
  ITCV_REQUIRE(dy && w && y_prev && dx && B > 0 && K > 0 && N > 0, "itcv_linear_dgrad_lrelu");
  ITCV_REQUIRE(lddy >= (size_t)N && ldy >= (size_t)K && slope > 0.f && slope <= FLT_MAX, "itcv_linear_dgrad_lrelu");
  return run_gemm64("itcv_linear_dgrad_lrelu", dy, w, nullptr, dx, B, K, N, (long long)lddy, 1, K, 1, 0, ws, ws_bytes,
                    S(stream), 2, y_prev, (long long)ldy, slope);
}

int itcv_conv2d_wgrad5_bf16p_supported(int Cs, int Cb, int H, int W) {
  return Cs >= 1 && Cs <= 3 && Cb == 64 && H > 0 && W >= 32 && W <= 256 && W % 32 == 0;
}
static inline int wgrad5_rows_per_job(int B, int H) {
  int r = cdiv(B * H, 1024);
  return r < 1 ? 1 : r;
}
size_t itcv_conv2d_wgrad5_bf16p_workspace(int B, int H) {
  if (B <= 0 || H <= 0) return 0;
  const int rpj = wgrad5_rows_per_job(B, H);
  return (size_t)B * cdiv(H, rpj) * 16 * 5 * 64 * sizeof(float);
}
int itcv_conv2d_wgrad5_bf16p(const float* small, const void* big_planes, float* dw, int B, int Cs, int H, int W,
                             int stem, int ns, const float* small_amax, int accumulate, void* ws, size_t ws_bytes,
                             void* stream) {
  ITCV_REQUIRE(small && big_planes && dw && B > 0 && (ns == 2 || ns == ITCV_PLANES_F16X2), "itcv_conv2d_wgrad5_bf16p");
  ITCV_REQUIRE(!small_amax || ns == ITCV_PLANES_F16X2, "itcv_conv2d_wgrad5_bf16p(a scale only applies to fp16 planes)");
  const int f16 = ns == ITCV_PLANES_F16X2;
  if (!itcv_conv2d_wgrad5_bf16p_supported(Cs, 64, H, W))
    return fail("%s: needs Cs <= 3, 64 channels on the other side, W in {32, 64}", "itcv_conv2d_wgrad5_bf16p");
  const int rpj = wgrad5_rows_per_job(B, H), njobs = B * cdiv(H, rpj);
  if (int e = check_ws("itcv_conv2d_wgrad5_bf16p", ws, ws_bytes, itcv_conv2d_wgrad5_bf16p_workspace(B, H))) return e;
  hipStream_t st = S(stream);
  const size_t plane_stride = (size_t)B * 8 * H * W;
  {
    ProfScope prof(st, kProfWgrad5, 5, Cs, stem ? 1 : 0, ns, 2.0 * B * H * W * 64.0 * Cs * 25);
    pick<2>(stem ? 1 : 0, [&](auto stem_c) {
      pick<2>(f16 ? 1 : 0, [&](auto f16_c) {
        launch_timed((conv_wgrad5_planes_kernel<(stem_c.value ? 1 : -1), f16_c.value != 0>), dim3(cdiv(njobs, 4)), dim3(256), 0,
                     st, small, static_cast<const u32x4*>(big_planes), static_cast<float*>(ws), B, Cs, H, W, rpj, njobs,
                     plane_stride, small_amax);
      });
    });
  }
  ITCV_CHECK_LAUNCH("itcv_conv2d_wgrad5_bf16p");
  const int total = Cs * 25 * 64;
  hipLaunchKernelGGL(wgrad5_reduce, dim3(cdiv(total, 16)), dim3(256), 0, st, static_cast<const float*>(ws), dw, Cs, njobs,
                     stem ? 1 : 0, accumulate);
  ITCV_CHECK_LAUNCH("itcv_conv2d_wgrad5_bf16p(reduce)");
  return 0;
}

int itcv_conv2d_fwd_variant(int B, int Ci, int H, int W, int Co, int KS, int up2) {
  if (B <= 0 || Ci <= 0 || H <= 0 || W <= 0 || Co <= 0) return -1;
  const FwdPlan p = plan_fwd(kFwdF32, B, Ci, H, W, Co, KS);
  return p.bm | (KS << 8) | ((up2 ? 1 : 0) << 16) | (p.splits << 20);
}
int itcv_conv2d_wgrad_variant(int B, int Ci, int H, int W, int Co, int KS, int up2) {
  if (B <= 0 || Ci <= 0 || H <= 0 || W <= 0 || Co <= 0) return -1;
  const WgPlan p = plan_wgrad(B, Ci, H, W, Co, KS);
  return p.bm | (KS << 8) | ((up2 ? 1 : 0) << 16) | (p.splits << 20);
}

size_t itcv_bias_grad_workspace(int B, int C, int HW) {
  return B > 0 && C > 0 && HW > 0 ? (size_t)bias_splits(B, C, HW) * C * sizeof(double) : 0;
}

int itcv_bias_grad(const float* dy, float* db, int B, int C, int HW, int accumulate, void* ws, size_t ws_bytes,
                   void* stream) {
  ITCV_REQUIRE(dy && db && B > 0 && C > 0 && HW > 0, "itcv_bias_grad");
  const int splits = bias_splits(B, C, HW);
  ITCV_REQUIRE(ws && ws_bytes >= (size_t)splits * C * sizeof(double), "itcv_bias_grad(workspace)");
  double* part = static_cast<double*>(ws);
  hipLaunchKernelGGL(bias_grad_partial, dim3(C, splits), dim3(256), 0, S(stream), dy, part, B, C, HW, splits);
  ITCV_CHECK_LAUNCH("itcv_bias_grad");
  hipLaunchKernelGGL(bias_grad_combine, dim3(cdiv(C, 256)), dim3(256), 0, S(stream), part, db, C, splits, accumulate);
  ITCV_CHECK_LAUNCH("itcv_bias_grad(combine)");
  return 0;
}

}
```

intro-tc-vae_amd/csrc/conv_shared.h:

```cpp
#pragma once
#include <stdlib.h>

#include "common.h"

namespace itcv {

#ifdef ITCV_DIAG
#define ITCV_ABL(args, bits) (((args).ablate & (bits)) != 0)
#define ITCV_DBG(args) ((args).debug != 0)
static int diag_ablate() {
  static int v = -1;
  if (v < 0) {
    const char* e = getenv("ITCV_ABLATE");
    v = e ? atoi(e) : 0;
  }
  return v;
}
#else
#define ITCV_ABL(args, bits) (false)
#define ITCV_DBG(args) (false)
#endif

typedef float f32x16 __attribute__((ext_vector_type(16)));
typedef float f32x4_t __attribute__((ext_vector_type(4)));
typedef float f32x4 __attribute__((ext_vector_type(4)));

#pragma clang diagnostic ignored "-Winline-asm"
__device__ __forceinline__ void lds_dma16(const void* gptr, uint32_t lds_base) {
  asm volatile("s_mov_b32 m0, %0\n\ts_nop 0\n\tglobal_load_lds_dwordx4 %1, off"
               :
               : "s"(__builtin_amdgcn_readfirstlane(lds_base)), "v"(gptr)
               : "memory", "m0");
}
__device__ __forceinline__ uint32_t lds_addr(const void* p) {
  return (uint32_t)(size_t)(const __attribute__((address_space(3))) void*)p;
}
template <int N>
__device__ __forceinline__ void wait_vmcnt() {
  asm volatile("s_waitcnt vmcnt(%0)" ::"n"(N) : "memory");
}

static inline int log2_exact(int v) {
  if (v <= 0 || (v & (v - 1))) return -1;
  int s = 0;
  while ((1 << s) < v) ++s;
  return s;
}

struct ConvArgsP2 {
  const u32x4* xp;
  const u32x4* wp;
  const float* bias;
  float* y;
  int B, Ci, H, Co;
  int Mp, N;
  int mt, nt;
  int cpt, cpt_per_split;
  int SR, NSEG, NP, NPC, PXB;
  int h_shift;
  float* stats;
  int stat_T;
  const ScaleRec* xscale;
  size_t slab_stride, plane_stride;
#ifdef ITCV_DIAG
  int debug;
#endif
};

__host__ __device__ constexpr int band_taps_per_stage(int bm, int bn, int ) {
  return (bm == 64 || bn == 128) ? 2 : 1;
}

template <bool M16, bool F16 = false>
struct BandMfma;
template <bool F16>
struct BandMfma<false, F16> {
  typedef f32x16 acc_t;
  static constexpr int TS = 32, NR = 16, KSN = 2;
  static __device__ __forceinline__ acc_t mma(bf16x8 a, bf16x8 b, acc_t c) { return mma32x32x16<F16>(a, b, c); }
  static __device__ __forceinline__ int row(int r, int kq) { return (r & 3) + 8 * (r >> 2) + 4 * kq; }
};
template <bool F16>
struct BandMfma<true, F16> {
  typedef float acc_t __attribute__((ext_vector_type(4)));
  static constexpr int TS = 16, NR = 4, KSN = 1;
  static __device__ __forceinline__ acc_t mma(bf16x8 a, bf16x8 b, acc_t c) { return mma16x16x32<F16>(a, b, c); }
  static __device__ __forceinline__ int row(int r, int kq) { return 4 * kq + r; }
};

struct Options {
  int band_m16 = 1;
  int band_persist_blocks = 256;
  int wgrad_m16 = 1;
  int planes_mfma_waves = 8;
};
extern Options g_opt;
inline int band_m16() { return g_opt.band_m16; }

enum class FwdPath {
  Band,
  BandPersistent,
  WidePersistent,
  Planes128,
};
struct FwdPlanP {
  FwdPath path;
  int bm, bn, mt, nt, splits;
  int stat_tiles;
  size_t ws_need;
  int cpt, cps, SR, NSEG, NP, NPC, PXB;
  int rows2;
  size_t lds;
  int ktiles, kps;
};

bool plan_fwd_band(FwdPlanP& p, int B, int Ci, int H, int W, int Co, int KS, int ns);
void launch_fwd_band(const ConvArgsP2& a, const FwdPlanP& p, int W, int up2, int f16, hipStream_t st);
bool band_adj_form(const FwdPlanP& p, int W, int f16);
void launch_fwd_band_adj(const ConvArgsP2& a, const FwdPlanP& p, int W, int f16, hipStream_t st);

}
```

intro-tc-vae_amd/csrc/latent.hip:

```cpp
#include <math.h>

#include "common.h"

namespace itcv {

constexpr float kHalfLog2Pi = 0.9189385332046727f;
constexpr float kLog2Pi = 1.8378770664093453f;
constexpr float kVarEps = 1e-4f;
constexpr float kFloor = -50.f;

struct TcConst {
  float lw_n, lw_s, lw_m;
  float log_bn;
  int M;
};

__device__ __forceinline__ float log_iw(const TcConst& c, int jg, int i) {
  if (i == 0) return jg == c.M - 1 ? c.lw_s : c.lw_n;
  return i == 1 ? c.lw_s : c.lw_m;
}

template <bool EPS>
__device__ __forceinline__ float logdens(float d, float lv) {
  if (EPS) {
    const float vh = fmaxf(expf(lv), kVarEps);
    return -(0.5f * (logf(vh) + d * d / vh) + kHalfLog2Pi);
  }
  return -0.5f * (d * d * expf(-lv) + lv + kLog2Pi);
}

constexpr int kTcIC = 16;
constexpr int kTcRW = kTcIC / 4;
constexpr int kTcDLMax = 8;

__host__ __device__ inline int tc_chunks(int Bt) { return (Bt + kTcIC - 1) / kTcIC; }

template <bool EPS>
__device__ __forceinline__ void dens_coef(float lv, float& A, float& Bv) {
  if (EPS) {
    const float vh = fmaxf(expf(lv), kVarEps);
    A = logf(vh), Bv = 1.f / vh;
  } else {
    A = lv, Bv = expf(-lv);
  }
}

template <int DL, bool VROW, bool EPS, bool MWS>
__global__ __launch_bounds__(256) void tc_fwd_part_kernel(const float* __restrict__ z, const float* __restrict__ mu_all,
                                                          const float* __restrict__ logvar, float* __restrict__ pmax,
                                                          float* __restrict__ psum, float* __restrict__ sjoint, int Bt,
                                                          int row_offset, int D, int nch, TcConst c, int ldm,
                                                          float* __restrict__ ivar) {
  extern __shared__ __attribute__((aligned(16))) float sm[];
  float* mu_s = sm;
  float* A_s = mu_s + kTcIC * D;
  float* B_s = A_s + (VROW ? 0 : kTcIC * D);
  float* cm = B_s + (VROW ? 0 : kTcIC * D);
  float* cs = cm + 4 * D;
  const int j = blockIdx.x, ch = blockIdx.y, jg = row_offset + j;
  const int tid = threadIdx.x, lane = tid & 63, wid = tid >> 6;
  const int i0 = ch * kTcIC, rows = min(kTcIC, Bt - i0);
  if (VROW || ldm == D) {
    for (int e = tid; e < rows * D; e += 256) {
      mu_s[e] = mu_all[(size_t)i0 * D + e];
      if (!VROW) dens_coef<EPS>(logvar[(size_t)i0 * D + e], A_s[e], B_s[e]);
    }
  } else {
    for (int e = tid; e < rows * D; e += 256) {
      const int r = e / D, l = e - r * D;
      mu_s[e] = mu_all[(size_t)(i0 + r) * ldm + l];
      if (!VROW) dens_coef<EPS>(logvar[(size_t)(i0 + r) * ldm + l], A_s[e], B_s[e]);
    }
  }
  float zj[DL], Aj[DL], Bj[DL];
#pragma unroll
  for (int k = 0; k < DL; ++k) {
    const int l = lane + 64 * k;
    zj[k] = 0.f, Aj[k] = 0.f, Bj[k] = 0.f;
    if (l < D) {
      zj[k] = z[(size_t)j * D + l];
      if (VROW) dens_coef<EPS>(logvar[(size_t)j * D + l], Aj[k], Bj[k]);
    }
  }
  __syncthreads();
  if (!VROW && ivar && j == 0)
    for (int e = tid; e < rows * D; e += 256) ivar[(size_t)i0 * D + e] = B_s[e];
  float v[kTcRW][DL];
#pragma unroll
  for (int r = 0; r < kTcRW; ++r) {
    const int ii = wid + 4 * r;
    const bool have = ii < rows;
    const float liw = (have && !MWS) ? log_iw(c, jg, i0 + ii) : 0.f;
    float part = 0.f;
#pragma unroll
    for (int k = 0; k < DL; ++k) {
      const int l = lane + 64 * k;
      v[r][k] = -INFINITY;
      if (have && l < D) {
        const float d = zj[k] - mu_s[ii * D + l];
        const float A = VROW ? Aj[k] : A_s[ii * D + l], Bv = VROW ? Bj[k] : B_s[ii * D + l];
        const float lp = fmaxf(-0.5f * (A + d * d * Bv) - kHalfLog2Pi, kFloor);
        part += lp;
        v[r][k] = lp + liw;
      }
    }
    if (have) {
      part = wave_sum(part);
      if (lane == 0) sjoint[(size_t)j * Bt + i0 + ii] = part + liw;
    }
  }
#pragma unroll
  for (int k = 0; k < DL; ++k) {
    const int l = lane + 64 * k;
    float m = v[0][k];
#pragma unroll
    for (int r = 1; r < kTcRW; ++r) m = fmaxf(m, v[r][k]);
    float se = 0.f;
    if (m > -INFINITY) {
#pragma unroll
      for (int r = 0; r < kTcRW; ++r) se += expf(v[r][k] - m);
    }
    if (l < D) cm[wid * D + l] = m, cs[wid * D + l] = se;
  }
  __syncthreads();
  for (int l = tid; l < D; l += 256) {
    float m = fmaxf(fmaxf(cm[l], cm[D + l]), fmaxf(cm[2 * D + l], cm[3 * D + l]));
    float se = 0.f;
#pragma unroll
    for (int w = 0; w < 4; ++w) {
      const float mw = cm[w * D + l];
      if (mw > -INFINITY) se += cs[w * D + l] * expf(mw - m);
    }
    pmax[((size_t)j * nch + ch) * D + l] = m;
    psum[((size_t)j * nch + ch) * D + l] = se;
  }
}

struct TcKlOut {
  const float* mu_loc;
  const float* lv_loc;
  float* rows;
  float coef_tc, coef_kl;
};

struct TcFullOut {
  const float* z;
  const float* mu_d;
  const float* lv_d;
  float* rows;
  float* comps;
  int ld, Bl;
  float a, b, g;
};

__device__ __forceinline__ float diag_lp(float zz, float m, float lv) { return logdens<false>(zz - m, lv); }
__device__ __forceinline__ float prior_lp(float zz) { return logdens<false>(zz, 0.f); }

template <bool MWS>
__global__ __launch_bounds__(256) void tc_fwd_finish_kernel(const float* __restrict__ pmax, const float* __restrict__ psum,
                                                            const float* __restrict__ sjoint, float* __restrict__ prodm,
                                                            float* __restrict__ logqz, float* __restrict__ lse, int Bt, int D,
                                                            int nch, TcConst c, TcKlOut kk, TcFullOut ff) {
  __shared__ float red[4];
  const int j = blockIdx.x, tid = threadIdx.x, lane = tid & 63, wid = tid >> 6;
  float prod_acc = 0.f;
  for (int l = tid; l < D; l += 256) {
    const float* pm = pmax + (size_t)j * nch * D + l;
    const float* ps = psum + (size_t)j * nch * D + l;
    float m = -INFINITY;
    for (int k = 0; k < nch; ++k) m = fmaxf(m, pm[(size_t)k * D]);
    float se = 0.f;
    for (int k = 0; k < nch; ++k) se += ps[(size_t)k * D] * expf(pm[(size_t)k * D] - m);
    float r = m + logf(se);
    lse[(size_t)j * D + l] = r;
    if (MWS) r -= c.log_bn;
    prod_acc += r;
  }
  float mx = -INFINITY;
  for (int i = tid; i < Bt; i += 256) mx = fmaxf(mx, sjoint[(size_t)j * Bt + i]);
  mx = wave_max(mx);
  if (lane == 0) red[wid] = mx;
  __syncthreads();
  mx = fmaxf(fmaxf(red[0], red[1]), fmaxf(red[2], red[3]));
  __syncthreads();
  float se = 0.f;
  for (int i = tid; i < Bt; i += 256) se += expf(sjoint[(size_t)j * Bt + i] - mx);
  se = block_sum(se, red);
  const float pm = block_sum(prod_acc, red);
  float klj = 0.f;
  if (kk.rows) {
    float a = 0.f;
    for (int l = tid; l < D; l += 256) {
      const float v = kk.lv_loc[(size_t)j * D + l], m = kk.mu_loc[(size_t)j * D + l];
      a += 1.f + v - expf(v) - m * m;
    }
    klj = -0.5f * block_sum(a, red);
  }
  float lcx = 0.f, lpz = 0.f;
  if (ff.rows) {
    float a = 0.f, b = 0.f;
    for (int l = tid; l < D; l += 256) {
      const float zz = ff.z[(size_t)j * D + l];
      a += fmaxf(diag_lp(zz, ff.mu_d[(size_t)j * ff.ld + l], ff.lv_d[(size_t)j * ff.ld + l]), kFloor);
      b += fmaxf(prior_lp(zz), kFloor);
    }
    lcx = block_sum(a, red);
    lpz = block_sum(b, red);
  }
  if (tid == 0) {
    const float lq = mx + logf(se) - (MWS ? c.log_bn : 0.f);
    logqz[j] = lq;
    prodm[j] = pm;
    if (kk.rows) kk.rows[j] = kk.coef_tc * (lq - pm) + kk.coef_kl * klj;
    if (ff.rows) {
      const float mi = lcx - lq, tc = lq - pm, dw = pm - lpz;
      ff.rows[j] = ff.a * mi + ff.b * tc + ff.g * dw;
      if (ff.comps) ff.comps[j] = mi, ff.comps[ff.Bl + j] = tc, ff.comps[2 * ff.Bl + j] = dw;
    }
  }
}

__global__ __launch_bounds__(256) void rows_reduce_kernel(const float* __restrict__ rows, float* __restrict__ out, int B,
                                                         int mean, float scale) {
  __shared__ double red[4];
  double a = 0.0;
  for (int j = threadIdx.x; j < B; j += 256) a += (double)rows[j];
  a = block_sum(a, red);
  if (threadIdx.x == 0) out[0] = scale * (float)(mean ? a / (double)B : a);
}

struct TcGrad {
  const float* g;
  int bcast;
  float coef_tc, coef_kl;
};
__device__ __forceinline__ float tc_g(const TcGrad& t, int j) { return t.bcast ? t.g[0] : t.g[j]; }
constexpr int kTcBwdU = 16;

__global__ __launch_bounds__(256) void tc_bwd_rows_kernel(
    TcGrad tg, const float* __restrict__ z, const float* __restrict__ mu_all,
    const float* __restrict__ logvar, const float* __restrict__ logqz, const float* __restrict__ lse,
    const float* __restrict__ sjoint, float* __restrict__ wq, float* __restrict__ dz, float* __restrict__ dlogvar, int Bt,
    int row_offset, int D, TcConst c) {
  __shared__ float raz[4][64], rav[4][64];
  const int j = blockIdx.x, jg = row_offset + j, l = blockIdx.y * 64 + (threadIdx.x & 63);
  const int lane = threadIdx.x & 63, wid = threadIdx.x >> 6;
  const bool act = l < D;
  const float gr = tc_g(tg, j), gj = tg.coef_tc * gr, gk = tg.coef_kl * gr, lq = logqz[j];
  const float zj = act ? z[(size_t)j * D + l] : 0.f, lvj = act ? logvar[(size_t)j * D + l] : 0.f;
  const float var = expf(lvj), vh = fmaxf(var, kVarEps), lvh = logf(vh), ivh = 1.f / vh;
  const float ls = act ? lse[(size_t)j * D + l] : 0.f;
  float az = 0.f, av = 0.f;
  const int lc = min(l, D - 1);
  for (int i0 = wid; i0 < Bt; i0 += 4 * kTcBwdU) {
    float mv[kTcBwdU], sv[kTcBwdU];
#pragma unroll
    for (int u = 0; u < kTcBwdU; ++u) {
      const int ic = min(i0 + 4 * u, Bt - 1);
      mv[u] = mu_all[(size_t)ic * D + lc];
      sv[u] = sjoint[(size_t)j * Bt + ic];
    }
#pragma unroll
    for (int u = 0; u < kTcBwdU; ++u) {
      const int i = i0 + 4 * u;
      if (i < Bt) {
        const float liw = log_iw(c, jg, i);
        const float q = gj * expf(sv[u] - lq);
        if (blockIdx.y == 0 && lane == 0) wq[(size_t)j * Bt + i] = q;
        const float d = zj - mv[u];
        const float lp = -(0.5f * (lvh + d * d * ivh) + kHalfLog2Pi);
        if (act && lp >= kFloor) {
          const float G = q - gj * expf(lp + liw - ls);
          const float dv = d * ivh;
          az -= G * dv;
          av -= G * 0.5f * (ivh - dv * dv);
        }
      }
    }
  }
  raz[wid][lane] = az, rav[wid][lane] = av;
  __syncthreads();
  if (wid == 0 && act) {
    dz[(size_t)j * D + l] = (raz[0][lane] + raz[1][lane]) + (raz[2][lane] + raz[3][lane]);
    const float dl = ((rav[0][lane] + rav[1][lane]) + (rav[2][lane] + rav[3][lane])) * var;
    dlogvar[(size_t)j * D + l] = gk != 0.f ? dl + gk * (-0.5f) * (1.f - var) : dl;
  }
}

__global__ __launch_bounds__(256) void tc_bwd_cols_kernel(
    TcGrad tg, const float* __restrict__ z, const float* __restrict__ mu_all,
    const float* __restrict__ logvar, const float* __restrict__ lse, const float* __restrict__ wq,
    float* __restrict__ dmu_all, int Bl, int Bt, int row_offset, int D, TcConst c) {
  __shared__ float racc[4][64];
  const int i = blockIdx.x, l = blockIdx.y * 64 + (threadIdx.x & 63);
  const int lane = threadIdx.x & 63, wid = threadIdx.x >> 6;
  const bool act = l < D;
  const float mi = act ? mu_all[(size_t)i * D + l] : 0.f;
  float acc = 0.f;
  const int lc = min(l, D - 1);
  for (int j0 = wid; j0 < Bl; j0 += 4 * kTcBwdU) {
    float lvv[kTcBwdU], zv[kTcBwdU], lsv[kTcBwdU], qv[kTcBwdU], gv[kTcBwdU];
#pragma unroll
    for (int u = 0; u < kTcBwdU; ++u) {
      const int jc = min(j0 + 4 * u, Bl - 1);
      lvv[u] = logvar[(size_t)jc * D + lc];
      zv[u] = z[(size_t)jc * D + lc];
      lsv[u] = lse[(size_t)jc * D + lc];
      qv[u] = wq[(size_t)jc * Bt + i];
      gv[u] = tg.g[tg.bcast ? 0 : jc];
    }
#pragma unroll
    for (int u = 0; u < kTcBwdU; ++u) {
      const int j = j0 + 4 * u;
      if (j < Bl) {
        const float gj = tg.coef_tc * gv[u], q = qv[u], liw = log_iw(c, row_offset + j, i);
        const float vh = fmaxf(expf(lvv[u]), kVarEps), ivh = 1.f / vh;
        const float d = zv[u] - mi;
        const float lp = -(0.5f * (logf(vh) + d * d * ivh) + kHalfLog2Pi);
        if (act && lp >= kFloor) acc += (q - gj * expf(lp + liw - lsv[u])) * d * ivh;
      }
    }
  }
  racc[wid][lane] = acc;
  __syncthreads();
  if (wid == 0 && act) {
    float v = (racc[0][lane] + racc[1][lane]) + (racc[2][lane] + racc[3][lane]);
    if (tg.coef_kl != 0.f && i >= row_offset && i < row_offset + Bl) v += tg.coef_kl * tc_g(tg, i - row_offset) * mi;
    dmu_all[(size_t)i * D + l] = v;
  }
}

struct TcFullGrad {
  const float* g;
  int bcast;
  float a, cq, cp, c;
};
__device__ __forceinline__ float tcf_g(const TcFullGrad& t, int j) { return t.bcast ? t.g[0] : t.g[j]; }

__global__ __launch_bounds__(256) void tc_full_bwd_rows_kernel(
    TcFullGrad tg, const float* __restrict__ z, const float* __restrict__ mu_all, const float* __restrict__ lv_all, int ld,
    const float* __restrict__ ivar, const float* __restrict__ logqz, const float* __restrict__ lse,
    const float* __restrict__ sjoint, float* __restrict__ wq, float* __restrict__ dz, int Bt, int row_offset, int D,
    TcConst c) {
  __shared__ float raz[4][64];
  const int j = blockIdx.x, jg = row_offset + j, l = blockIdx.y * 64 + (threadIdx.x & 63);
  const int lane = threadIdx.x & 63, wid = threadIdx.x >> 6;
  const bool act = l < D;
  const float gr = tcf_g(tg, j), cq = tg.cq * gr, cp = tg.cp * gr, lq = logqz[j];
  const float zj = act ? z[(size_t)j * D + l] : 0.f, ls = act ? lse[(size_t)j * D + l] : 0.f;
  float az = 0.f;
#pragma unroll 4
  for (int i = wid; i < Bt; i += 4) {
    const float liw = log_iw(c, jg, i);
    const float q = cq * expf(sjoint[(size_t)j * Bt + i] - lq);
    if (blockIdx.y == 0 && lane == 0) wq[(size_t)j * Bt + i] = q;
    if (act) {
      const float d = zj - mu_all[(size_t)i * ld + l], iv = ivar[(size_t)i * D + l];
      const float lp = -0.5f * (lv_all[(size_t)i * ld + l] + d * d * iv) - kHalfLog2Pi;
      if (lp >= kFloor) az -= (q + cp * expf(lp + liw - ls)) * d * iv;
    }
  }
  raz[wid][lane] = az;
  __syncthreads();
  if (wid == 0 && act) {
    float v = (raz[0][lane] + raz[1][lane]) + (raz[2][lane] + raz[3][lane]);
    const float m = mu_all[(size_t)jg * ld + l], lv = lv_all[(size_t)jg * ld + l], d = zj - m;
    if (diag_lp(zj, m, lv) >= kFloor) v += tg.a * gr * (-d * expf(-lv));
    if (prior_lp(zj) >= kFloor) v += tg.c * gr * zj;
    dz[(size_t)j * D + l] = v;
  }
}

__global__ __launch_bounds__(256) void tc_full_bwd_cols_kernel(
    TcFullGrad tg, const float* __restrict__ z, const float* __restrict__ mu_all, const float* __restrict__ lv_all, int ld,
    const float* __restrict__ ivar, const float* __restrict__ lse, const float* __restrict__ wq,
    float* __restrict__ dmu_all, float* __restrict__ dlv_all, int Bl, int Bt, int row_offset, int D, TcConst c) {
  __shared__ float ram[4][64], rav[4][64];
  const int i = blockIdx.x, l = blockIdx.y * 64 + (threadIdx.x & 63);
  const int lane = threadIdx.x & 63, wid = threadIdx.x >> 6;
  const bool act = l < D;
  const float mi = act ? mu_all[(size_t)i * ld + l] : 0.f, lvi = act ? lv_all[(size_t)i * ld + l] : 0.f;
  const float iv = act ? ivar[(size_t)i * D + l] : 0.f;
  float am = 0.f, av = 0.f;
#pragma unroll 2
  for (int j = wid; j < Bl; j += 4) {
    const float cp = tg.cp * tcf_g(tg, j), q = wq[(size_t)j * Bt + i], liw = log_iw(c, row_offset + j, i);
    if (act) {
      const float d = z[(size_t)j * D + l] - mi;
      const float lp = -0.5f * (lvi + d * d * iv) - kHalfLog2Pi;
      if (lp >= kFloor) {
        const float G = q + cp * expf(lp + liw - lse[(size_t)j * D + l]);
        am += G * d * iv;
        av += G * (1.f - d * d * iv);
      }
    }
  }
  ram[wid][lane] = am, rav[wid][lane] = av;
  __syncthreads();
  if (wid == 0 && act) {
    float vm = (ram[0][lane] + ram[1][lane]) + (ram[2][lane] + ram[3][lane]);
    float vl = -0.5f * ((rav[0][lane] + rav[1][lane]) + (rav[2][lane] + rav[3][lane]));
    if (i >= row_offset && i < row_offset + Bl) {
      const int jl = i - row_offset;
      const float zz = z[(size_t)jl * D + l], d = zz - mi, e = expf(-lvi), ga = tg.a * tcf_g(tg, jl);
      if (diag_lp(zz, mi, lvi) >= kFloor) vm += ga * d * e, vl += ga * (-0.5f) * (1.f - d * d * e);
    }
    dmu_all[(size_t)i * ld + l] = vm;
    dlv_all[(size_t)i * ld + l] = vl;
  }
}

__global__ __launch_bounds__(256) void diag_logdensity_kernel(const float* __restrict__ z,
                                                             const float* __restrict__ mu,
                                                             const float* __restrict__ logvar,
                                                             float* __restrict__ logq, float* __restrict__ logp,
                                                             int D) {
  __shared__ float red[4];
  const int j = blockIdx.x;
  float a = 0.f, b = 0.f;
  for (int l = threadIdx.x; l < D; l += 256) {
    const float zz = z[(size_t)j * D + l];
    a += fmaxf(logdens<false>(zz - mu[(size_t)j * D + l], logvar[(size_t)j * D + l]), kFloor);
    b += fmaxf(logdens<false>(zz, 0.f), kFloor);
  }
  a = block_sum(a, red);
  b = block_sum(b, red);
  if (threadIdx.x == 0) logq[j] = a, logp[j] = b;
}

__global__ void reparam_fwd_kernel(const float* __restrict__ mu, const float* __restrict__ lv,
                                   const float* __restrict__ eps, float* __restrict__ z, size_t n) {
  for (size_t i = (size_t)blockIdx.x * blockDim.x + threadIdx.x; i < n; i += (size_t)gridDim.x * blockDim.x)
    z[i] = mu[i] + eps[i] * expf(0.5f * lv[i]);
}
__global__ void reparam_bwd_kernel(const float* __restrict__ dz, const float* __restrict__ lv,
                                   const float* __restrict__ eps, float* __restrict__ dmu,
                                   float* __restrict__ dlv, size_t n) {
  for (size_t i = (size_t)blockIdx.x * blockDim.x + threadIdx.x; i < n; i += (size_t)gridDim.x * blockDim.x) {
    const float d = dz[i];
    dmu[i] = d;
    dlv[i] = d * eps[i] * 0.5f * expf(0.5f * lv[i]);
  }
}
__global__ __launch_bounds__(256) void kl_rows_fwd_kernel(const float* __restrict__ lv, const float* __restrict__ mu,
                                                         float* __restrict__ kl, int D) {
  __shared__ float red[4];
  const int j = blockIdx.x;
  float a = 0.f;
  for (int l = threadIdx.x; l < D; l += 256) {
    const float v = lv[(size_t)j * D + l], m = mu[(size_t)j * D + l];
    a += 1.f + v - expf(v) - m * m;
  }
  a = block_sum(a, red);
  if (threadIdx.x == 0) kl[j] = -0.5f * a;
}
__global__ void kl_rows_bwd_kernel(const float* __restrict__ g, const float* __restrict__ lv,
                                   const float* __restrict__ mu, float* __restrict__ dlv, float* __restrict__ dmu,
                                   int D, size_t n) {
  for (size_t i = (size_t)blockIdx.x * blockDim.x + threadIdx.x; i < n; i += (size_t)gridDim.x * blockDim.x) {
    const float gj = g[i / D];
    dlv[i] = gj * (-0.5f) * (1.f - expf(lv[i]));
    dmu[i] = gj * mu[i];
  }
}

struct Bc3 {
  int n1, n2;
  long long sx[3], sm[3], sl[3];
};

template <bool EPS>
__global__ void gauss_logdensity_fwd_kernel(const float* __restrict__ x, const float* __restrict__ mu,
                                            const float* __restrict__ lv, float* __restrict__ out, Bc3 b, size_t n) {
  for (size_t e = (size_t)blockIdx.x * blockDim.x + threadIdx.x; e < n; e += (size_t)gridDim.x * blockDim.x) {
    const long long i2 = (long long)(e % b.n2), r = (long long)(e / b.n2), i1 = r % b.n1, i0 = r / b.n1;
    const float d = x[i0 * b.sx[0] + i1 * b.sx[1] + i2 * b.sx[2]] - mu[i0 * b.sm[0] + i1 * b.sm[1] + i2 * b.sm[2]];
    out[e] = fmaxf(logdens<EPS>(d, lv[i0 * b.sl[0] + i1 * b.sl[1] + i2 * b.sl[2]]), kFloor);
  }
}

template <bool EPS>
__global__ void gauss_logdensity_bwd_kernel(const float* __restrict__ g, const float* __restrict__ x,
                                            const float* __restrict__ mu, const float* __restrict__ lv,
                                            float* __restrict__ dx, float* __restrict__ dlv, Bc3 b, size_t n) {
  for (size_t e = (size_t)blockIdx.x * blockDim.x + threadIdx.x; e < n; e += (size_t)gridDim.x * blockDim.x) {
    const long long i2 = (long long)(e % b.n2), r = (long long)(e / b.n2), i1 = r % b.n1, i0 = r / b.n1;
    const float d = x[i0 * b.sx[0] + i1 * b.sx[1] + i2 * b.sx[2]] - mu[i0 * b.sm[0] + i1 * b.sm[1] + i2 * b.sm[2]];
    const float l = lv[i0 * b.sl[0] + i1 * b.sl[1] + i2 * b.sl[2]];
    const float gg = g[e];
    float gx = 0.f, gl = 0.f;
    if (logdens<EPS>(d, l) >= kFloor) {
      if (EPS) {
        const float var = expf(l), ivh = 1.f / fmaxf(var, kVarEps), dv = d * ivh;
        gx = -gg * dv;
        gl = -gg * 0.5f * (ivh - dv * dv) * var;
      } else {
        const float iv = expf(-l);
        gx = -gg * d * iv;
        gl = -gg * 0.5f * (1.f - d * d * iv);
      }
    }
    dx[e] = gx, dlv[e] = gl;
  }
}

template <bool MWS>
__global__ __launch_bounds__(256) void sampling_fwd_kernel(const float* __restrict__ lp, float* __restrict__ prodm,
                                                           float* __restrict__ logqz, float* __restrict__ lse,
                                                           float* __restrict__ sj, int B, int D, TcConst c) {
  __shared__ float red[4];
  const int j = blockIdx.x, tid = threadIdx.x, lane = tid & 63, wid = tid >> 6;
  const float* row = lp + (size_t)j * B * D;
  for (int i = wid; i < B; i += 4) {
    float s = 0.f;
    for (int l = lane; l < D; l += 64) s += row[(size_t)i * D + l];
    s = wave_sum(s);
    if (lane == 0) sj[(size_t)j * B + i] = s + (MWS ? 0.f : log_iw(c, j, i));
  }
  float prod_acc = 0.f;
  for (int l = tid; l < D; l += 256) {
    float m = -INFINITY;
    for (int i = 0; i < B; ++i) m = fmaxf(m, row[(size_t)i * D + l] + (MWS ? 0.f : log_iw(c, j, i)));
    float se = 0.f;
    for (int i = 0; i < B; ++i) se += expf(row[(size_t)i * D + l] + (MWS ? 0.f : log_iw(c, j, i)) - m);
    const float r = m + logf(se);
    lse[(size_t)j * D + l] = r;
    prod_acc += MWS ? r - c.log_bn : r;
  }
  __syncthreads();
  float mx = -INFINITY;
  for (int i = tid; i < B; i += 256) mx = fmaxf(mx, sj[(size_t)j * B + i]);
  mx = wave_max(mx);
  if (lane == 0) red[wid] = mx;
  __syncthreads();
  mx = fmaxf(fmaxf(red[0], red[1]), fmaxf(red[2], red[3]));
  __syncthreads();
  float se = 0.f;
  for (int i = tid; i < B; i += 256) se += expf(sj[(size_t)j * B + i] - mx);
  se = block_sum(se, red);
  const float pm = block_sum(prod_acc, red);
  if (tid == 0) {
    logqz[j] = mx + logf(se) - (MWS ? c.log_bn : 0.f);
    prodm[j] = pm;
  }
}

template <bool MWS>
__global__ __launch_bounds__(256) void sampling_bwd_kernel(const float* __restrict__ gp, const float* __restrict__ gq,
                                                           const float* __restrict__ lp, const float* __restrict__ lse,
                                                           const float* __restrict__ sj, const float* __restrict__ logqz,
                                                           float* __restrict__ dlp, int B, int D, TcConst c) {
  const int j = blockIdx.x, i = blockIdx.y;
  const float liw = MWS ? 0.f : log_iw(c, j, i);
  const float lq = logqz[j] + (MWS ? c.log_bn : 0.f);
  const float wq = gq[j] * expf(sj[(size_t)j * B + i] - lq), g1 = gp[j];
  const size_t base = ((size_t)j * B + i) * D;
  for (int l = threadIdx.x; l < D; l += 256) dlp[base + l] = g1 * expf(lp[base + l] + liw - lse[(size_t)j * D + l]) + wq;
}

__global__ void on_off_diag_kernel(const float* __restrict__ x, float* __restrict__ diag, float* __restrict__ off, int m,
                                   int n) {
  const size_t total = (size_t)m * n * n;
  for (size_t e = (size_t)blockIdx.x * blockDim.x + threadIdx.x; e < total; e += (size_t)gridDim.x * blockDim.x) {
    const int k = (int)(e % n), i = (int)((e / n) % n), a = (int)(e / ((size_t)n * n));
    const float xv = x[(size_t)(m == 1 ? 0 : i) * n + k];
    off[e] = xv - (i == k ? x[(size_t)a * n + i] : 0.f);
    if (e < (size_t)(m < n ? m : n)) diag[e] = x[e * n + e];
  }
}

__global__ __launch_bounds__(1024) void kl_loss_fwd_kernel(const float* __restrict__ lv, const float* __restrict__ mu,
                                                          float* __restrict__ out, int B, int D, int reduction, float scale) {
  __shared__ double part[16];
  const int lane = threadIdx.x & 63, w = threadIdx.x >> 6;
  double acc = 0.0;
  for (int j = w; j < B; j += 16) {
    float a = 0.f;
    for (int l = lane; l < D; l += 64) {
      const float v = lv[(size_t)j * D + l], m = mu[(size_t)j * D + l];
      a += 1.f + v - expf(v) - m * m;
    }
    const float kl = -0.5f * wave_sum(a);
    if (reduction == 0) {
      if (lane == 0) out[j] = scale * kl;
    } else {
      acc += (double)kl;
    }
  }
  if (reduction == 0) return;
  if (lane == 0) part[w] = acc;
  __syncthreads();
  if (threadIdx.x == 0) {
    double t = 0.0;
    for (int k = 0; k < 16; ++k) t += part[k];
    out[0] = scale * (float)(reduction == 2 ? t / (double)B : t);
  }
}
__global__ void kl_loss_bwd_kernel(const float* __restrict__ g, const float* __restrict__ lv, const float* __restrict__ mu,
                                   float* __restrict__ dlv, float* __restrict__ dmu, int D, size_t n, int reduction,
                                   float coef) {
  const float g0 = reduction ? g[0] * coef : 0.f;
  for (size_t i = (size_t)blockIdx.x * blockDim.x + threadIdx.x; i < n; i += (size_t)gridDim.x * blockDim.x) {
    const float gj = reduction ? g0 : g[i / D] * coef;
    dlv[i] = gj * (-0.5f) * (1.f - expf(lv[i]));
    dmu[i] = gj * mu[i];
  }
}

static int make_const(const char* name, int Bt, int64_t N, TcConst* c) {
  if (Bt < 2) return fail("%s: batch size must be >= 2 (M = B-1 divides the weights; ops.py:43-45)", name);
  if (N <= 0) return fail("%s: dataset_size must be positive", name);
  const double n = (double)N, m = (double)(Bt - 1);
  c->lw_n = logf((float)(1.0 / n));
  c->lw_s = logf((float)((n - m) / (n * m)));
  c->lw_m = logf((float)(1.0 / m));
  c->log_bn = (float)log((double)Bt * n);
  c->M = Bt - 1;
  return 0;
}

static inline int ew_grid(size_t n) {
  size_t b = cdivz(n, 256);
  return (int)(b > 2048 ? 2048 : (b < 1 ? 1 : b));
}

}

using namespace itcv;

extern "C" {

int itcv_reparam_fwd(const float* mu, const float* logvar, const float* eps, float* z, size_t n, void* stream) {
  ITCV_REQUIRE(mu && logvar && eps && z, "itcv_reparam_fwd");
  if (!n) return 0;
  hipLaunchKernelGGL(reparam_fwd_kernel, dim3(ew_grid(n)), dim3(256), 0, S(stream), mu, logvar, eps, z, n);
  ITCV_CHECK_LAUNCH("itcv_reparam_fwd");
  return 0;
}
int itcv_reparam_bwd(const float* dz, const float* logvar, const float* eps, float* dmu, float* dlogvar, size_t n,
                     void* stream) {
  ITCV_REQUIRE(dz && logvar && eps && dmu && dlogvar, "itcv_reparam_bwd");
  if (!n) return 0;
  hipLaunchKernelGGL(reparam_bwd_kernel, dim3(ew_grid(n)), dim3(256), 0, S(stream), dz, logvar, eps, dmu, dlogvar, n);
  ITCV_CHECK_LAUNCH("itcv_reparam_bwd");
  return 0;
}
int itcv_kl_rows_fwd(const float* logvar, const float* mu, float* kl, int B, int D, void* stream) {
  ITCV_REQUIRE(logvar && mu && kl && B > 0 && D > 0, "itcv_kl_rows_fwd");
  hipLaunchKernelGGL(kl_rows_fwd_kernel, dim3(B), dim3(256), 0, S(stream), logvar, mu, kl, D);
  ITCV_CHECK_LAUNCH("itcv_kl_rows_fwd");
  return 0;
}
int itcv_kl_rows_bwd(const float* g, const float* logvar, const float* mu, float* dlogvar, float* dmu, int B, int D,
                     void* stream) {
  ITCV_REQUIRE(g && logvar && mu && dlogvar && dmu && B > 0 && D > 0, "itcv_kl_rows_bwd");
  const size_t n = (size_t)B * D;
  hipLaunchKernelGGL(kl_rows_bwd_kernel, dim3(ew_grid(n)), dim3(256), 0, S(stream), g, logvar, mu, dlogvar, dmu, D, n);
  ITCV_CHECK_LAUNCH("itcv_kl_rows_bwd");
  return 0;
}

size_t itcv_tc_fwd_workspace(int Bl, int Bt, int D) {
  return Bl > 0 && Bt > 0 && D > 0 ? (size_t)2 * Bl * tc_chunks(Bt) * D * sizeof(float) : 0;
}

}
static int tc_fwd_impl(const float* z, const float* mu_all, const float* logvar, float* prodm, float* logqz, float* lse,
                       float* sjoint, int Bl, int Bt, int row_offset, int D, int64_t dataset_size, int flags, void* ws,
                       size_t ws_bytes, const TcKlOut& kk, void* stream, int ldm = 0, float* ivar = nullptr,
                       const TcFullOut& ff = TcFullOut{}) {
  ITCV_REQUIRE(z && mu_all && logvar && prodm && logqz && lse && sjoint && Bl > 0 && D > 0, "itcv_tc_fwd");
  ITCV_REQUIRE(row_offset >= 0 && row_offset + Bl <= Bt, "itcv_tc_fwd(rows must lie inside the global batch)");
  if (D > 64 * kTcDLMax) return fail("%s: latent size %lld > 512 is not supported", "itcv_tc_fwd", D);
  if (ldm == 0) ldm = D;
  TcConst c;
  if (int e = make_const("itcv_tc_fwd", Bt, dataset_size, &c)) return e;
  const int nch = tc_chunks(Bt);
  ITCV_REQUIRE(ws && ws_bytes >= itcv_tc_fwd_workspace(Bl, Bt, D), "itcv_tc_fwd(workspace)");
  float* pmax = static_cast<float*>(ws);
  float* psum = pmax + (size_t)Bl * nch * D;
  const bool vrow = flags & ITCV_TC_VAR_FROM_ROW, eps = flags & ITCV_TC_EPS_DENSITY, mws = flags & ITCV_TC_WEIGHTED;
  const size_t lds = ((size_t)(vrow ? 1 : 3) * kTcIC * D + (size_t)8 * D) * sizeof(float);
  const int dl = D <= 64 ? 1 : (D <= 128 ? 2 : (D <= 256 ? 4 : 8));
  dim3 grid(Bl, nch), block(256);
  hipStream_t st = S(stream);
#define ITCV_TC_PART(DL, V, E, W)                                                                               \
  do {                                                                                                          \
    if (lds > 64 * 1024) {                                                                                      \
      const hipError_t e_ = hipFuncSetAttribute(reinterpret_cast<const void*>(&tc_fwd_part_kernel<DL, V, E, W>), \
                                                hipFuncAttributeMaxDynamicSharedMemorySize, (int)lds);          \
      if (e_ != hipSuccess)                                                                                     \
        return fail("%s: %lld bytes of LDS refused (hipFuncSetAttribute: %lld)", "itcv_tc_fwd", (long long)lds,  \
                    (long long)e_);                                                                             \
    }                                                                                                           \
    hipLaunchKernelGGL((tc_fwd_part_kernel<DL, V, E, W>), grid, block, lds, st, z, mu_all, logvar, pmax, psum,   \
                       sjoint, Bt, row_offset, D, nch, c, ldm, ivar);                                           \
  } while (0)
#define ITCV_TC_DL(V, E, W)                \
  do {                                     \
    if (dl == 1) ITCV_TC_PART(1, V, E, W); \
    else if (dl == 2) ITCV_TC_PART(2, V, E, W); \
    else if (dl == 4) ITCV_TC_PART(4, V, E, W); \
    else ITCV_TC_PART(8, V, E, W);         \
  } while (0)
  if (vrow && eps && !mws) ITCV_TC_DL(true, true, false);
  else if (vrow && eps && mws) ITCV_TC_DL(true, true, true);
  else if (vrow && !eps && !mws) ITCV_TC_DL(true, false, false);
  else if (vrow && !eps && mws) ITCV_TC_DL(true, false, true);
  else if (!vrow && eps && !mws) ITCV_TC_DL(false, true, false);
  else if (!vrow && eps && mws) ITCV_TC_DL(false, true, true);
  else if (!vrow && !eps && !mws) ITCV_TC_DL(false, false, false);
  else ITCV_TC_DL(false, false, true);
#undef ITCV_TC_DL
#undef ITCV_TC_PART
  ITCV_CHECK_LAUNCH("itcv_tc_fwd(partials)");
  if (mws)
    hipLaunchKernelGGL(tc_fwd_finish_kernel<true>, dim3(Bl), block, 0, st, pmax, psum, sjoint, prodm, logqz, lse, Bt, D, nch, c, kk, ff);
  else
    hipLaunchKernelGGL(tc_fwd_finish_kernel<false>, dim3(Bl), block, 0, st, pmax, psum, sjoint, prodm, logqz, lse, Bt, D, nch, c, kk, ff);
  ITCV_CHECK_LAUNCH("itcv_tc_fwd(finish)");
  return 0;
}
extern "C" {
int itcv_tc_fwd(const float* z, const float* mu_all, const float* logvar, float* prodm, float* logqz, float* lse,
                float* sjoint, int Bl, int Bt, int row_offset, int D, int64_t dataset_size, int flags, void* ws,
                size_t ws_bytes, void* stream) {
  return tc_fwd_impl(z, mu_all, logvar, prodm, logqz, lse, sjoint, Bl, Bt, row_offset, D, dataset_size, flags, ws, ws_bytes,
                     TcKlOut{nullptr, nullptr, nullptr, 0.f, 0.f}, stream);
}

int itcv_tc_kl_fwd(const float* z, const float* mu_all, const float* logvar, float* out, float* rows, float* prodm,
                   float* logqz, float* lse, float* sjoint, int Bl, int Bt, int row_offset, int D, int64_t dataset_size,
                   float coef_tc, float coef_kl, int reduction, void* ws, size_t ws_bytes, void* stream) {
  ITCV_REQUIRE(out && (reduction == 0 || rows) && reduction >= 0 && reduction <= 2, "itcv_tc_kl_fwd");
  ITCV_REQUIRE(mu_all && row_offset >= 0 && row_offset + Bl <= Bt, "itcv_tc_kl_fwd(rows must lie inside the global batch)");
  const TcKlOut kk{mu_all + (size_t)row_offset * D, logvar, reduction == 0 ? out : rows, coef_tc, coef_kl};
  if (int e = tc_fwd_impl(z, mu_all, logvar, prodm, logqz, lse, sjoint, Bl, Bt, row_offset, D, dataset_size, ITCV_TC_LIVE, ws,
                          ws_bytes, kk, stream))
    return e;
  if (reduction) {
    hipLaunchKernelGGL(rows_reduce_kernel, dim3(1), dim3(256), 0, S(stream), rows, out, Bl, reduction == 2 ? 1 : 0, 1.f);
    ITCV_CHECK_LAUNCH("itcv_tc_kl_fwd(reduce)");
  }
  return 0;
}

size_t itcv_tc_bwd_workspace(int Bl, int Bt) { return Bl > 0 && Bt > 0 ? (size_t)Bl * Bt * sizeof(float) : 0; }

}
static int tc_bwd_impl(const TcGrad& tg, const float* z, const float* mu_all, const float* logvar, const float* logqz,
                       const float* lse, const float* sjoint, float* dz, float* dmu_all, float* dlogvar, int Bl, int Bt,
                       int row_offset, int D, int64_t dataset_size, int flags, void* ws, size_t ws_bytes, void* stream) {
  ITCV_REQUIRE(tg.g && z && mu_all && logvar && logqz && lse && sjoint && dz && dmu_all && dlogvar && Bl > 0 && D > 0,
               "itcv_tc_bwd");
  ITCV_REQUIRE(row_offset >= 0 && row_offset + Bl <= Bt, "itcv_tc_bwd(rows must lie inside the global batch)");
  if (flags != ITCV_TC_LIVE)
    return fail("%s: gradients exist for the live estimator only (flags == ITCV_TC_LIVE)", "itcv_tc_bwd");
  ITCV_REQUIRE(ws && ws_bytes >= (size_t)Bl * Bt * sizeof(float), "itcv_tc_bwd(workspace)");
  TcConst c;
  if (int e = make_const("itcv_tc_bwd", Bt, dataset_size, &c)) return e;
  float* wq = static_cast<float*>(ws);
  hipStream_t st = S(stream);
  const int lch = cdiv(D, 64);
  hipLaunchKernelGGL(tc_bwd_rows_kernel, dim3(Bl, lch), dim3(256), 0, st, tg, z, mu_all, logvar, logqz, lse, sjoint, wq, dz,
                     dlogvar, Bt, row_offset, D, c);
  ITCV_CHECK_LAUNCH("itcv_tc_bwd(rows)");
  hipLaunchKernelGGL(tc_bwd_cols_kernel, dim3(Bt, lch), dim3(256), 0, st, tg, z, mu_all, logvar, lse, wq, dmu_all, Bl, Bt,
                     row_offset, D, c);
  ITCV_CHECK_LAUNCH("itcv_tc_bwd(cols)");
  return 0;
}
extern "C" {
int itcv_tc_bwd(const float* g, const float* z, const float* mu_all, const float* logvar, const float* logqz,
                const float* lse, const float* sjoint, float* dz, float* dmu_all, float* dlogvar, int Bl, int Bt,
                int row_offset, int D, int64_t dataset_size, int flags, void* ws, size_t ws_bytes, void* stream) {
  return tc_bwd_impl(TcGrad{g, 0, 1.f, 0.f}, z, mu_all, logvar, logqz, lse, sjoint, dz, dmu_all, dlogvar, Bl, Bt, row_offset,
                     D, dataset_size, flags, ws, ws_bytes, stream);
}
int itcv_tc_kl_bwd(const float* g, const float* z, const float* mu_all, const float* logvar, const float* logqz,
                   const float* lse, const float* sjoint, float* dz, float* dmu_all, float* dlogvar, int Bl, int Bt,
                   int row_offset, int D, int64_t dataset_size, float coef_tc, float coef_kl, int reduction, void* ws,
                   size_t ws_bytes, void* stream) {
  ITCV_REQUIRE(reduction >= 0 && reduction <= 2, "itcv_tc_kl_bwd");
  const float r = reduction == 2 ? 1.f / (float)Bl : 1.f;
  return tc_bwd_impl(TcGrad{g, reduction ? 1 : 0, coef_tc * r, coef_kl * r}, z, mu_all, logvar, logqz, lse, sjoint, dz, dmu_all,
                     dlogvar, Bl, Bt, row_offset, D, dataset_size, ITCV_TC_LIVE, ws, ws_bytes, stream);
}

size_t itcv_tc_full_fwd_workspace(int Bl, int Bt, int D) { return itcv_tc_fwd_workspace(Bl, Bt, D); }
size_t itcv_tc_full_bwd_workspace(int Bl, int Bt) { return itcv_tc_bwd_workspace(Bl, Bt); }

static int tc_full_check(const char* name, bool ptrs, int Bl, int Bt, int row_offset, int D, int ld, int reduction) {
  if (!ptrs) return fail("%s: a required pointer is NULL", name);
  if (Bl <= 0 || D <= 0) return fail("%s: Bl = %lld and D = %lld must be positive", name, Bl, D);
  if (D > 64 * kTcDLMax) return fail("%s: latent size %lld > 512 is not supported", name, D);
  if (row_offset < 0 || row_offset + Bl > Bt)
    return fail("%s: rows must lie inside the global batch (row_offset = %lld, Bt = %lld)", name, row_offset, Bt);
  if (ld < D) return fail("%s: row stride %lld of mu_all / logvar_all is below D = %lld", name, ld, D);
  if (reduction < 0 || reduction > 2) return fail("%s: reduction %lld is not 0 (none), 1 (sum) or 2 (mean)", name, reduction);
  return 0;
}

int itcv_tc_full_fwd(const float* z, const float* mu_all, const float* logvar_all, int ld, float* out, float* rows,
                     float* comps, float* prodm, float* logqz, float* lse, float* sjoint, float* ivar, int Bl, int Bt,
                     int row_offset, int D, int64_t dataset_size, float alpha, float beta, float gamma, int reduction,
                     void* ws, size_t ws_bytes, void* stream) {
  if (int e = tc_full_check("itcv_tc_full_fwd",
                            z && mu_all && logvar_all && out && (reduction == 0 || rows) && prodm && logqz && lse && sjoint &&
                                ivar && ws,
                            Bl, Bt, row_offset, D, ld, reduction))
    return e;
  const size_t off = (size_t)row_offset * ld;
  const TcFullOut ff{z, mu_all + off, logvar_all + off, reduction == 0 ? out : rows, comps, ld, Bl, alpha, beta, gamma};
  if (int e = tc_fwd_impl(z, mu_all, logvar_all, prodm, logqz, lse, sjoint, Bl, Bt, row_offset, D, dataset_size, 0, ws,
                          ws_bytes, TcKlOut{nullptr, nullptr, nullptr, 0.f, 0.f}, stream, ld, ivar, ff))
    return e;
  if (reduction) {
    hipLaunchKernelGGL(rows_reduce_kernel, dim3(1), dim3(256), 0, S(stream), rows, out, Bl, reduction == 2 ? 1 : 0, 1.f);
    ITCV_CHECK_LAUNCH("itcv_tc_full_fwd(reduce)");
  }
  return 0;
}

int itcv_tc_full_bwd(const float* g, const float* z, const float* mu_all, const float* logvar_all, int ld,
                     const float* logqz, const float* lse, const float* sjoint, const float* ivar, float* dz, float* dmu_all,
                     float* dlogvar_all, int Bl, int Bt, int row_offset, int D, int64_t dataset_size, float alpha,
                     float beta, float gamma, int reduction, void* ws, size_t ws_bytes, void* stream) {
  if (int e = tc_full_check("itcv_tc_full_bwd",
                            g && z && mu_all && logvar_all && logqz && lse && sjoint && ivar && dz && dmu_all && dlogvar_all,
                            Bl, Bt, row_offset, D, ld, reduction))
    return e;
  ITCV_REQUIRE(ws && ws_bytes >= itcv_tc_full_bwd_workspace(Bl, Bt), "itcv_tc_full_bwd(workspace)");
  TcConst c;
  if (int e = make_const("itcv_tc_full_bwd", Bt, dataset_size, &c)) return e;
  const float r = reduction == 2 ? 1.f / (float)Bl : 1.f;
  const TcFullGrad tg{g, reduction ? 1 : 0, alpha * r, (beta - alpha) * r, (gamma - beta) * r, gamma * r};
  float* wq = static_cast<float*>(ws);
  hipStream_t st = S(stream);
  const int lch = cdiv(D, 64);
  hipLaunchKernelGGL(tc_full_bwd_rows_kernel, dim3(Bl, lch), dim3(256), 0, st, tg, z, mu_all, logvar_all, ld, ivar, logqz,
                     lse, sjoint, wq, dz, Bt, row_offset, D, c);
  ITCV_CHECK_LAUNCH("itcv_tc_full_bwd(rows)");
  hipLaunchKernelGGL(tc_full_bwd_cols_kernel, dim3(Bt, lch), dim3(256), 0, st, tg, z, mu_all, logvar_all, ld, ivar, lse, wq,
                     dmu_all, dlogvar_all, Bl, Bt, row_offset, D, c);
  ITCV_CHECK_LAUNCH("itcv_tc_full_bwd(cols)");
  return 0;
}

int itcv_kl_loss_fwd(const float* logvar, const float* mu, float* out, int B, int D, int reduction, float scale, void* stream) {
  ITCV_REQUIRE(logvar && mu && out && B > 0 && D > 0 && reduction >= 0 && reduction <= 2, "itcv_kl_loss_fwd");
  hipLaunchKernelGGL(kl_loss_fwd_kernel, dim3(1), dim3(1024), 0, S(stream), logvar, mu, out, B, D, reduction, scale);
  ITCV_CHECK_LAUNCH("itcv_kl_loss_fwd");
  return 0;
}
int itcv_kl_loss_bwd(const float* g, const float* logvar, const float* mu, float* dlogvar, float* dmu, int B, int D,
                     int reduction, float scale, void* stream) {
  ITCV_REQUIRE(g && logvar && mu && dlogvar && dmu && B > 0 && D > 0 && reduction >= 0 && reduction <= 2, "itcv_kl_loss_bwd");
  const size_t n = (size_t)B * D;
  hipLaunchKernelGGL(kl_loss_bwd_kernel, dim3(ew_grid(n)), dim3(256), 0, S(stream), g, logvar, mu, dlogvar, dmu, D, n, reduction,
                     reduction == 2 ? scale / (float)B : scale);
  ITCV_CHECK_LAUNCH("itcv_kl_loss_bwd");
  return 0;
}

static Bc3 make_bc3(const int64_t* dims, const int64_t* sx, const int64_t* sm, const int64_t* sl) {
  Bc3 b;
  b.n1 = (int)dims[1], b.n2 = (int)dims[2];
  for (int k = 0; k < 3; ++k) b.sx[k] = sx[k], b.sm[k] = sm[k], b.sl[k] = sl[k];
  return b;
}

int itcv_gauss_logdensity_fwd(const float* x, const float* mu, const float* logvar, float* out, const int64_t* dims,
                              const int64_t* sx, const int64_t* sm, const int64_t* sl, int eps_density, void* stream) {
  ITCV_REQUIRE(x && mu && logvar && out && dims && sx && sm && sl, "itcv_gauss_logdensity_fwd");
  ITCV_REQUIRE(dims[0] > 0 && dims[1] > 0 && dims[2] > 0 && dims[1] < (1ll << 31) && dims[2] < (1ll << 31),
               "itcv_gauss_logdensity_fwd(shape)");
  const size_t n = (size_t)dims[0] * dims[1] * dims[2];
  const Bc3 b = make_bc3(dims, sx, sm, sl);
  if (eps_density)
    hipLaunchKernelGGL(gauss_logdensity_fwd_kernel<true>, dim3(ew_grid(n)), dim3(256), 0, S(stream), x, mu, logvar, out, b, n);
  else
    hipLaunchKernelGGL(gauss_logdensity_fwd_kernel<false>, dim3(ew_grid(n)), dim3(256), 0, S(stream), x, mu, logvar, out, b, n);
  ITCV_CHECK_LAUNCH("itcv_gauss_logdensity_fwd");
  return 0;
}

int itcv_gauss_logdensity_bwd(const float* g, const float* x, const float* mu, const float* logvar, float* dx,
                              float* dlogvar, const int64_t* dims, const int64_t* sx, const int64_t* sm,
                              const int64_t* sl, int eps_density, void* stream) {
  ITCV_REQUIRE(g && x && mu && logvar && dx && dlogvar && dims && sx && sm && sl, "itcv_gauss_logdensity_bwd");
  ITCV_REQUIRE(dims[0] > 0 && dims[1] > 0 && dims[2] > 0 && dims[1] < (1ll << 31) && dims[2] < (1ll << 31),
               "itcv_gauss_logdensity_bwd(shape)");
  const size_t n = (size_t)dims[0] * dims[1] * dims[2];
  const Bc3 b = make_bc3(dims, sx, sm, sl);
  if (eps_density)
    hipLaunchKernelGGL(gauss_logdensity_bwd_kernel<true>, dim3(ew_grid(n)), dim3(256), 0, S(stream), g, x, mu, logvar, dx,
                       dlogvar, b, n);
  else
    hipLaunchKernelGGL(gauss_logdensity_bwd_kernel<false>, dim3(ew_grid(n)), dim3(256), 0, S(stream), g, x, mu, logvar, dx,
                       dlogvar, b, n);
  ITCV_CHECK_LAUNCH("itcv_gauss_logdensity_bwd");
  return 0;
}

int itcv_sampling_fwd(const float* lp, float* prodm, float* logqz, float* lse, float* sjoint, int B, int D,
                      int64_t dataset_size, int weighted, void* stream) {
  ITCV_REQUIRE(lp && prodm && logqz && lse && sjoint && B > 0 && D > 0, "itcv_sampling_fwd");
  TcConst c;
  if (int e = make_const("itcv_sampling_fwd", B, dataset_size, &c)) return e;
  if (weighted)
    hipLaunchKernelGGL(sampling_fwd_kernel<true>, dim3(B), dim3(256), 0, S(stream), lp, prodm, logqz, lse, sjoint, B, D, c);
  else
    hipLaunchKernelGGL(sampling_fwd_kernel<false>, dim3(B), dim3(256), 0, S(stream), lp, prodm, logqz, lse, sjoint, B, D, c);
  ITCV_CHECK_LAUNCH("itcv_sampling_fwd");
  return 0;
}

int itcv_sampling_bwd(const float* g_prodm, const float* g_logqz, const float* lp, const float* lse, const float* sjoint,
                      const float* logqz, float* dlp, int B, int D, int64_t dataset_size, int weighted, void* stream) {
  ITCV_REQUIRE(g_prodm && g_logqz && lp && lse && sjoint && logqz && dlp && B > 0 && D > 0, "itcv_sampling_bwd");
  ITCV_REQUIRE(B <= 65535, "itcv_sampling_bwd(batch)");
  TcConst c;
  if (int e = make_const("itcv_sampling_bwd", B, dataset_size, &c)) return e;
  if (weighted)
    hipLaunchKernelGGL(sampling_bwd_kernel<true>, dim3(B, B), dim3(256), 0, S(stream), g_prodm, g_logqz, lp, lse, sjoint,
                       logqz, dlp, B, D, c);
  else
    hipLaunchKernelGGL(sampling_bwd_kernel<false>, dim3(B, B), dim3(256), 0, S(stream), g_prodm, g_logqz, lp, lse, sjoint,
                       logqz, dlp, B, D, c);
  ITCV_CHECK_LAUNCH("itcv_sampling_bwd");
  return 0;
}

int itcv_on_off_diag(const float* x, float* diag, float* off, int m, int n, void* stream) {
  ITCV_REQUIRE(x && diag && off && m > 0 && n > 0 && (m == n || m == 1), "itcv_on_off_diag");
  hipLaunchKernelGGL(on_off_diag_kernel, dim3(ew_grid((size_t)m * n * n)), dim3(256), 0, S(stream), x, diag, off, m, n);
  ITCV_CHECK_LAUNCH("itcv_on_off_diag");
  return 0;
}

int itcv_diag_logdensity_rows(const float* z, const float* mu, const float* logvar, float* logq_cx, float* logpz,
                              int B, int D, void* stream) {
  ITCV_REQUIRE(z && mu && logvar && logq_cx && logpz && B > 0 && D > 0, "itcv_diag_logdensity_rows");
  hipLaunchKernelGGL(diag_logdensity_kernel, dim3(B), dim3(256), 0, S(stream), z, mu, logvar, logq_cx, logpz, D);
  ITCV_CHECK_LAUNCH("itcv_diag_logdensity_rows");
  return 0;
}

}
```

intro-tc-vae_amd/csrc/loss_optim.hip:

```cpp
#include <math.h>

#include "common.h"
#include "recon_rows.h"

namespace itcv {

template <int LT>
__global__ __launch_bounds__(256) void recon_partial_kernel(const float* __restrict__ x,
                                                           const float* __restrict__ recon,
                                                           double* __restrict__ part, size_t P, int splits, int vec4) {
  __shared__ double scratch[4];
  const int b = blockIdx.x, s = blockIdx.y;
  size_t beg, end;
  recon_slice(P, splits, s, beg, end);
  double acc = recon_slice_acc<LT>(x + (size_t)b * P, recon + (size_t)b * P, beg, end, vec4);
  acc = block_sum(acc, scratch);
  if (threadIdx.x == 0) part[(size_t)b * splits + s] = acc;
}
__global__ void recon_combine_kernel(const double* __restrict__ part, float* __restrict__ rows, int B, int splits) {
  const int b = blockIdx.x * blockDim.x + threadIdx.x;
  if (b >= B) return;
  rows[b] = (float)fold_strided(0.0, part + (size_t)b * splits, (size_t)1, splits);
}
template <int LT>
__global__ void recon_bwd_kernel(const float* __restrict__ x, const float* __restrict__ recon,
                                 const float* __restrict__ g, float* __restrict__ drecon, size_t P, size_t n) {
  for (size_t i = (size_t)blockIdx.x * blockDim.x + threadIdx.x; i < n; i += (size_t)gridDim.x * blockDim.x)
    drecon[i] = g[i / P] * rec_derr<LT>(recon[i], x[i]);
}

__global__ __launch_bounds__(256) void recon_finish_kernel(const double* __restrict__ part, float* __restrict__ out, int B,
                                                          int splits, int reduction, float scale) {
  __shared__ double scratch[4];
  double acc = 0.0;
  for (int b = threadIdx.x; b < B; b += 256) {
    const float row = (float)fold_strided(0.0, part + (size_t)b * splits, (size_t)1, splits);
    if (reduction == 0) out[b] = scale * row;
    acc += (double)row;
  }
  if (reduction == 0) return;
  acc = block_sum(acc, scratch);
  if (threadIdx.x == 0) out[0] = scale * (float)(reduction == 2 ? acc / (double)B : acc);
}
template <int LT>
__global__ void recon_loss_bwd_kernel(const float* __restrict__ x, const float* __restrict__ recon,
                                      const float* __restrict__ g, float* __restrict__ drecon, size_t P, size_t n,
                                      int reduction, float coef) {
  const float g0 = reduction ? g[0] * coef : 0.f;
  for (size_t i = (size_t)blockIdx.x * blockDim.x + threadIdx.x; i < n; i += (size_t)gridDim.x * blockDim.x)
    drecon[i] = (reduction ? g0 : g[i / P] * coef) * rec_derr<LT>(recon[i], x[i]);
}

__global__ __launch_bounds__(256) void exp_elbo_fwd_kernel(const float* __restrict__ a, const float* __restrict__ b,
                                                          float* __restrict__ out, float* __restrict__ w, int B, float c) {
  __shared__ float scratch[4];
  float acc = 0.f;
  for (int j = threadIdx.x; j < B; j += 256) {
    const float e = expf(c * (a[j] + b[j]));
    w[j] = e * c / (float)B;
    acc += e;
  }
  acc = block_sum(acc, scratch);
  if (threadIdx.x == 0) out[0] = acc / (float)B;
}
__global__ void exp_elbo_bwd_kernel(const float* __restrict__ g, const float* __restrict__ w, float* __restrict__ da,
                                    float* __restrict__ db, int B) {
  const int j = blockIdx.x * blockDim.x + threadIdx.x;
  if (j >= B) return;
  const float v = g[0] * w[j];
  da[j] = v;
  if (db) db[j] = v;
}

struct LinComb {
  const float* term[8];
  float weight[8];
  int n;
};
__global__ void lincomb_fwd_kernel(LinComb a, float* __restrict__ out) {
  if (threadIdx.x || blockIdx.x) return;
  float s = 0.f;
  for (int k = 0; k < a.n; ++k) s += a.weight[k] * a.term[k][0];
  out[0] = s;
}
__global__ void lincomb_bwd_kernel(const float* __restrict__ g, LinComb a, float* __restrict__ grads) {
  const int k = threadIdx.x;
  if (k < a.n) grads[k] = g[0] * a.weight[k];
}

static bool launch_recon_partial(const float* x, const float* recon, double* part, int B, size_t P, int splits,
                                 int loss_type, hipStream_t st) {
  const int vec4 = (P & 3) == 0 && (((uintptr_t)x | (uintptr_t)recon) & 15) == 0;
  dim3 grid(B, splits);
  if (loss_type == ITCV_LOSS_MSE)
    hipLaunchKernelGGL(recon_partial_kernel<ITCV_LOSS_MSE>, grid, dim3(256), 0, st, x, recon, part, P, splits, vec4);
  else if (loss_type == ITCV_LOSS_L1)
    hipLaunchKernelGGL(recon_partial_kernel<ITCV_LOSS_L1>, grid, dim3(256), 0, st, x, recon, part, P, splits, vec4);
  else if (loss_type == ITCV_LOSS_BCE)
    hipLaunchKernelGGL(recon_partial_kernel<ITCV_LOSS_BCE>, grid, dim3(256), 0, st, x, recon, part, P, splits, vec4);
  else
    return false;
  return true;
}

__global__ __launch_bounds__(256) void sumsq_partial_kernel(const float* __restrict__ x, size_t n,
                                                           double* __restrict__ part) {
  __shared__ double scratch[4];
  double acc = 0.0;
  const size_t n4 = n / 4;
  for (size_t i = (size_t)blockIdx.x * 256 + threadIdx.x; i < n4; i += (size_t)gridDim.x * 256) {
    const float4 v = reinterpret_cast<const float4*>(x)[i];
    acc += (double)v.x * v.x + (double)v.y * v.y + (double)v.z * v.z + (double)v.w * v.w;
  }
  if (blockIdx.x == 0)
    for (size_t i = n4 * 4 + threadIdx.x; i < n; i += 256) acc += (double)x[i] * x[i];
  acc = block_sum(acc, scratch);
  if (threadIdx.x == 0) part[blockIdx.x] = acc;
}
__global__ __launch_bounds__(256) void sumsq_final_kernel(const double* __restrict__ part, int nparts,
                                                         double* __restrict__ out) {
  __shared__ double scratch[4];
  double acc = 0.0;
  for (int i = threadIdx.x; i < nparts; i += 256) acc += part[i];
  acc = block_sum(acc, scratch);
  if (threadIdx.x == 0) out[0] = acc;
}
__global__ void clip_coef_kernel(const double* sumsq, int nparts, double clip, float* norm_out, float* coef_out) {
  double s = 0.0;
  for (int i = 0; i < nparts; ++i) s += sumsq[i];
  const double total = sqrt(s);
  double coef = clip / (total + 1e-6);
  if (coef > 1.0) coef = 1.0;
  norm_out[0] = (float)total;
  coef_out[0] = (float)coef;
}
__global__ void scale_by_dev_kernel(float* __restrict__ x, size_t n, const float* __restrict__ coef) {
  const float c = coef[0];
  const size_t n4 = n / 4;
  for (size_t i = (size_t)blockIdx.x * blockDim.x + threadIdx.x; i < n4; i += (size_t)gridDim.x * blockDim.x) {
    float4 v = reinterpret_cast<float4*>(x)[i];
    v.x *= c, v.y *= c, v.z *= c, v.w *= c;
    reinterpret_cast<float4*>(x)[i] = v;
  }
  if (blockIdx.x == 0)
    for (size_t i = n4 * 4 + threadIdx.x; i < n; i += blockDim.x) x[i] *= c;
}
__global__ void adam_kernel(float* __restrict__ p, const float* __restrict__ g, float* __restrict__ m,
                            float* __restrict__ v, size_t n, float step_size, float b1, float b2, float eps,
                            float sqrt_bc2) {
  for (size_t i = (size_t)blockIdx.x * blockDim.x + threadIdx.x; i < n; i += (size_t)gridDim.x * blockDim.x) {
    const float gi = g[i];
    const float mi = m[i] + (1.f - b1) * (gi - m[i]);
    const float vi = b2 * v[i] + (1.f - b2) * gi * gi;
    m[i] = mi;
    v[i] = vi;
    p[i] -= step_size * (mi / (sqrtf(vi) / sqrt_bc2 + eps));
  }
}
__global__ void adam_dev_kernel(float* __restrict__ p, const float* __restrict__ g, float* __restrict__ m,
                                float* __restrict__ v, size_t n, float lr, float b1, float b2, float eps,
                                const int* __restrict__ step_dev) {
  const int step = step_dev[0] + 1;
  const double bc1 = 1.0 - pow((double)b1, (double)step), bc2 = 1.0 - pow((double)b2, (double)step);
  const float step_size = (float)((double)lr / bc1), sqrt_bc2 = (float)sqrt(bc2);
  for (size_t i = (size_t)blockIdx.x * blockDim.x + threadIdx.x; i < n; i += (size_t)gridDim.x * blockDim.x) {
    const float gi = g[i];
    const float mi = m[i] + (1.f - b1) * (gi - m[i]);
    const float vi = b2 * v[i] + (1.f - b2) * gi * gi;
    m[i] = mi;
    v[i] = vi;
    p[i] -= step_size * (mi / (sqrtf(vi) / sqrt_bc2 + eps));
  }
}
__global__ void bump_step_kernel(int* step_dev) { step_dev[0] += 1; }

__global__ void hflip_kernel(const float* __restrict__ x, float* __restrict__ y, const unsigned char* __restrict__ flip,
                             size_t rows_per_image, int W, size_t n) {
  for (size_t i = (size_t)blockIdx.x * blockDim.x + threadIdx.x; i < n; i += (size_t)gridDim.x * blockDim.x) {
    const size_t row = i / W;
    const int w = (int)(i - row * W);
    y[i] = flip[row / rows_per_image] ? x[row * W + (W - 1 - w)] : x[i];
  }
}

__global__ void fill_kernel(float* __restrict__ x, size_t n, float value) {
  for (size_t i = (size_t)blockIdx.x * blockDim.x + threadIdx.x; i < n; i += (size_t)gridDim.x * blockDim.x)
    x[i] = value;
}

constexpr int kSumsqBlocks = 1024;

}

using namespace itcv;

extern "C" {

size_t itcv_recon_workspace(int B, size_t P) {
  return B > 0 && P > 0 ? (size_t)B * recon_splits(B, P) * sizeof(double) : 0;
}

int itcv_recon_rows_fwd(const float* x, const float* recon, float* rows, int B, size_t P, int loss_type, void* ws,
                        size_t ws_bytes, void* stream) {
  ITCV_REQUIRE(x && recon && rows && B > 0 && P > 0, "itcv_recon_rows_fwd");
  const int splits = recon_splits(B, P);
  ITCV_REQUIRE(ws && ws_bytes >= (size_t)B * splits * sizeof(double), "itcv_recon_rows_fwd(workspace)");
  double* part = static_cast<double*>(ws);
  hipStream_t st = S(stream);
  if (!launch_recon_partial(x, recon, part, B, P, splits, loss_type, st))
    return fail("%s: unknown loss type %lld", "itcv_recon_rows_fwd", loss_type);
  ITCV_CHECK_LAUNCH("itcv_recon_rows_fwd");
  hipLaunchKernelGGL(recon_combine_kernel, dim3(cdiv(B, 256)), dim3(256), 0, st, part, rows, B, splits);
  ITCV_CHECK_LAUNCH("itcv_recon_rows_fwd(combine)");
  return 0;
}

int itcv_recon_rows_bwd(const float* x, const float* recon, const float* g, float* drecon, int B, size_t P,
                        int loss_type, void* stream) {
  ITCV_REQUIRE(x && recon && g && drecon && B > 0 && P > 0, "itcv_recon_rows_bwd");
  const size_t n = (size_t)B * P;
  dim3 grid(stream_grid(n, 1));
  hipStream_t st = S(stream);
  if (loss_type == ITCV_LOSS_MSE)
    hipLaunchKernelGGL(recon_bwd_kernel<ITCV_LOSS_MSE>, grid, dim3(256), 0, st, x, recon, g, drecon, P, n);
  else if (loss_type == ITCV_LOSS_L1)
    hipLaunchKernelGGL(recon_bwd_kernel<ITCV_LOSS_L1>, grid, dim3(256), 0, st, x, recon, g, drecon, P, n);
  else if (loss_type == ITCV_LOSS_BCE)
    hipLaunchKernelGGL(recon_bwd_kernel<ITCV_LOSS_BCE>, grid, dim3(256), 0, st, x, recon, g, drecon, P, n);
  else
    return fail("%s: unknown loss type %lld", "itcv_recon_rows_bwd", loss_type);
  ITCV_CHECK_LAUNCH("itcv_recon_rows_bwd");
  return 0;
}

int itcv_recon_loss_fwd(const float* x, const float* recon, float* out, int B, size_t P, int loss_type, int reduction,
                        float scale, void* ws, size_t ws_bytes, void* stream) {
  ITCV_REQUIRE(x && recon && out && B > 0 && P > 0 && reduction >= 0 && reduction <= 2, "itcv_recon_loss_fwd");
  const int splits = recon_splits(B, P);
  ITCV_REQUIRE(ws && ws_bytes >= (size_t)B * splits * sizeof(double), "itcv_recon_loss_fwd(workspace)");
  double* part = static_cast<double*>(ws);
  hipStream_t st = S(stream);
  if (!launch_recon_partial(x, recon, part, B, P, splits, loss_type, st))
    return fail("%s: unknown loss type %lld", "itcv_recon_loss_fwd", loss_type);
  ITCV_CHECK_LAUNCH("itcv_recon_loss_fwd");
  hipLaunchKernelGGL(recon_finish_kernel, dim3(1), dim3(256), 0, st, part, out, B, splits, reduction, scale);
  ITCV_CHECK_LAUNCH("itcv_recon_loss_fwd(finish)");
  return 0;
}

int itcv_recon_loss_bwd(const float* x, const float* recon, const float* g, float* drecon, int B, size_t P, int loss_type,
                        int reduction, float scale, void* stream) {
  ITCV_REQUIRE(x && recon && g && drecon && B > 0 && P > 0 && reduction >= 0 && reduction <= 2, "itcv_recon_loss_bwd");
  const size_t n = (size_t)B * P;
  dim3 grid(stream_grid(n, 1));
  hipStream_t st = S(stream);
  const float coef = reduction == 2 ? scale / (float)B : scale;
  if (loss_type == ITCV_LOSS_MSE)
    hipLaunchKernelGGL(recon_loss_bwd_kernel<ITCV_LOSS_MSE>, grid, dim3(256), 0, st, x, recon, g, drecon, P, n, reduction, coef);
  else if (loss_type == ITCV_LOSS_L1)
    hipLaunchKernelGGL(recon_loss_bwd_kernel<ITCV_LOSS_L1>, grid, dim3(256), 0, st, x, recon, g, drecon, P, n, reduction, coef);
  else if (loss_type == ITCV_LOSS_BCE)
    hipLaunchKernelGGL(recon_loss_bwd_kernel<ITCV_LOSS_BCE>, grid, dim3(256), 0, st, x, recon, g, drecon, P, n, reduction, coef);
  else
    return fail("%s: unknown loss type %lld", "itcv_recon_loss_bwd", loss_type);
  ITCV_CHECK_LAUNCH("itcv_recon_loss_bwd");
  return 0;
}

int itcv_exp_elbo_fwd(const float* a, const float* b, float* out, float* w, int B, float c, void* stream) {
  ITCV_REQUIRE(a && b && out && w && B > 0, "itcv_exp_elbo_fwd");
  hipLaunchKernelGGL(exp_elbo_fwd_kernel, dim3(1), dim3(256), 0, S(stream), a, b, out, w, B, c);
  ITCV_CHECK_LAUNCH("itcv_exp_elbo_fwd");
  return 0;
}
int itcv_exp_elbo_bwd(const float* g, const float* w, float* da, float* db, int B, void* stream) {
  ITCV_REQUIRE(g && w && da && B > 0, "itcv_exp_elbo_bwd");
  hipLaunchKernelGGL(exp_elbo_bwd_kernel, dim3(cdiv(B, 256)), dim3(256), 0, S(stream), g, w, da, db, B);
  ITCV_CHECK_LAUNCH("itcv_exp_elbo_bwd");
  return 0;
}

int itcv_lincomb_fwd(const float* const* terms, const float* weights, int n, float* out, void* stream) {
  ITCV_REQUIRE(terms && weights && out && n >= 1 && n <= 8, "itcv_lincomb_fwd");
  LinComb a;
  memset(&a, 0, sizeof(a));
  a.n = n;
  for (int k = 0; k < n; ++k) {
    ITCV_REQUIRE(terms[k], "itcv_lincomb_fwd(term)");
    a.term[k] = terms[k], a.weight[k] = weights[k];
  }
  hipLaunchKernelGGL(lincomb_fwd_kernel, dim3(1), dim3(64), 0, S(stream), a, out);
  ITCV_CHECK_LAUNCH("itcv_lincomb_fwd");
  return 0;
}
int itcv_lincomb_bwd(const float* g, const float* weights, int n, float* grads, void* stream) {
  ITCV_REQUIRE(g && weights && grads && n >= 1 && n <= 8, "itcv_lincomb_bwd");
  LinComb a;
  memset(&a, 0, sizeof(a));
  a.n = n;
  for (int k = 0; k < n; ++k) a.weight[k] = weights[k];
  hipLaunchKernelGGL(lincomb_bwd_kernel, dim3(1), dim3(64), 0, S(stream), g, a, grads);
  ITCV_CHECK_LAUNCH("itcv_lincomb_bwd");
  return 0;
}

size_t itcv_sumsq_workspace(size_t n) {
  (void)n;
  return kSumsqBlocks * sizeof(double);
}

int itcv_sumsq(const float* x, size_t n, double* out, void* ws, size_t ws_bytes, void* stream) {
  ITCV_REQUIRE(x && out && ws && ws_bytes >= kSumsqBlocks * sizeof(double), "itcv_sumsq");
  ITCV_REQUIRE(((uintptr_t)x & 15) == 0, "itcv_sumsq(16-byte aligned input)");
  int blocks = stream_grid(n, 4);
  if (blocks > kSumsqBlocks) blocks = kSumsqBlocks;
  double* part = static_cast<double*>(ws);
  hipLaunchKernelGGL(sumsq_partial_kernel, dim3(blocks), dim3(256), 0, S(stream), x, n, part);
  ITCV_CHECK_LAUNCH("itcv_sumsq");
  hipLaunchKernelGGL(sumsq_final_kernel, dim3(1), dim3(256), 0, S(stream), part, blocks, out);
  ITCV_CHECK_LAUNCH("itcv_sumsq(final)");
  return 0;
}

int itcv_clip_coef(const double* sumsq, int nparts, double clip, float* norm_out, float* coef_out, void* stream) {
  ITCV_REQUIRE(sumsq && nparts > 0 && norm_out && coef_out, "itcv_clip_coef");
  hipLaunchKernelGGL(clip_coef_kernel, dim3(1), dim3(1), 0, S(stream), sumsq, nparts, clip, norm_out, coef_out);
  ITCV_CHECK_LAUNCH("itcv_clip_coef");
  return 0;
}

int itcv_scale_by_dev(float* x, size_t n, const float* coef_dev, void* stream) {
  ITCV_REQUIRE(x && coef_dev, "itcv_scale_by_dev");
  ITCV_REQUIRE(((uintptr_t)x & 15) == 0, "itcv_scale_by_dev(16-byte aligned input)");
  if (!n) return 0;
  hipLaunchKernelGGL(scale_by_dev_kernel, dim3(stream_grid(n, 4)), dim3(256), 0, S(stream), x, n, coef_dev);
  ITCV_CHECK_LAUNCH("itcv_scale_by_dev");
  return 0;
}

int itcv_adam_step(float* p, const float* g, float* m, float* v, size_t n, float lr, float beta1, float beta2,
                   float eps, int step, void* stream) {
  ITCV_REQUIRE(p && g && m && v && step >= 1, "itcv_adam_step");
  if (!n) return 0;
  const double bc1 = 1.0 - pow((double)beta1, step), bc2 = 1.0 - pow((double)beta2, step);
  const float step_size = (float)((double)lr / bc1), sqrt_bc2 = (float)sqrt(bc2);
  hipLaunchKernelGGL(adam_kernel, dim3(stream_grid(n, 1)), dim3(256), 0, S(stream), p, g, m, v, n, step_size, beta1,
                     beta2, eps, sqrt_bc2);
  ITCV_CHECK_LAUNCH("itcv_adam_step");
  return 0;
}

int itcv_adam_step_dev(float* p, const float* g, float* m, float* v, size_t n, float lr, float beta1, float beta2,
                       float eps, int* step_dev, void* stream) {
  ITCV_REQUIRE(p && g && m && v && step_dev, "itcv_adam_step_dev");
  if (!n) return 0;
  hipLaunchKernelGGL(adam_dev_kernel, dim3(stream_grid(n, 1)), dim3(256), 0, S(stream), p, g, m, v, n, lr, beta1, beta2,
                     eps, step_dev);
  ITCV_CHECK_LAUNCH("itcv_adam_step_dev");
  hipLaunchKernelGGL(bump_step_kernel, dim3(1), dim3(1), 0, S(stream), step_dev);
  ITCV_CHECK_LAUNCH("itcv_adam_step_dev(bump)");
  return 0;
}

int itcv_hflip(const float* x, float* y, const unsigned char* flip, int B, int rows_per_image, int W, void* stream) {
  ITCV_REQUIRE(x && y && flip && x != y && B > 0 && rows_per_image > 0 && W > 0, "itcv_hflip");
  const size_t n = (size_t)B * rows_per_image * W;
  hipLaunchKernelGGL(hflip_kernel, dim3(stream_grid(n, 1)), dim3(256), 0, S(stream), x, y, flip, (size_t)rows_per_image, W, n);
  ITCV_CHECK_LAUNCH("itcv_hflip");
  return 0;
}

int itcv_fill(float* x, size_t n, float value, void* stream) {
  ITCV_REQUIRE(x, "itcv_fill");
  if (!n) return 0;
  hipLaunchKernelGGL(fill_kernel, dim3(stream_grid(n, 1)), dim3(256), 0, S(stream), x, n, value);
  ITCV_CHECK_LAUNCH("itcv_fill");
  return 0;
}

}
```

Measured before the change: 4402.

## Fuse two-stage reductions via last-block counters and pipeline wgrad5 planes kernel

Adds a device counter ring and a last-block-arrives pattern. Two-kernel reductions (bias grad, sumsq, recon loss, TC finish, rows reduce) and the Adam step-bump each run as one kernel, with the final combine done by the last block. Separately, it adds a software-pipelined variant of the 5x5 wgrad planes kernel that prefetches the next row segment's operands while the MFMAs run on the current one. This removes launch overhead and exposes load latency, at the cost of atomics, fences, more registers and graph-capture slot bookkeeping.

After: 4277. 0.972x the previous value.

```diff
diff --git a/intro-tc-vae_amd/csrc/abi.hip b/intro-tc-vae_amd/csrc/abi.hip
--- a/intro-tc-vae_amd/csrc/abi.hip
+++ b/intro-tc-vae_amd/csrc/abi.hip
@@ -1,5 +1,6 @@
 #include "conv_shared.h"
 
+#include <mutex>
 #include <vector>
 
 namespace itcv {
@@ -36,6 +37,41 @@
 thread_local hipEvent_t g_prof_start = nullptr, g_prof_stop = nullptr;
 Options g_opt;
 extern int g_sw_lds_rows, g_sw_max_blocks;
+
+__device__ unsigned g_finish_counters[kFinishRing + kFinishCaptured];
+static int g_finish_in_kernel = 1;
+static std::mutex g_finish_mutex;
+static unsigned* g_finish_base = nullptr;
+static int g_finish_ring_next = 0, g_finish_captured_next = 0;
+
+unsigned* finish_slots(hipStream_t st, int n) {
+  if (!g_finish_in_kernel || n < 1 || n > kFinishMaxRun) return nullptr;
+  hipStreamCaptureStatus cs = hipStreamCaptureStatusNone;
+  if (hipStreamIsCapturing(st, &cs) != hipSuccess) {
+    (void)hipGetLastError();
+    return nullptr;
+  }
+  const bool capturing = cs != hipStreamCaptureStatusNone;
+  std::lock_guard<std::mutex> lock(g_finish_mutex);
+  if (!g_finish_base) {
+    void* p = nullptr;
+    if (capturing || hipGetSymbolAddress(&p, HIP_SYMBOL(g_finish_counters)) != hipSuccess || !p) {
+      (void)hipGetLastError();
+      return nullptr;
+    }
+    g_finish_base = static_cast<unsigned*>(p);
+  }
+  if (capturing) {
+    if (g_finish_captured_next + n > kFinishCaptured) return nullptr;
+    unsigned* p = g_finish_base + kFinishRing + g_finish_captured_next;
+    g_finish_captured_next += n;
+    return p;
+  }
+  if (g_finish_ring_next + n > kFinishRing) g_finish_ring_next = 0;
+  unsigned* p = g_finish_base + g_finish_ring_next;
+  g_finish_ring_next += n;
+  return p;
+}
 }
 
 extern "C" {
@@ -63,6 +99,16 @@
     itcv::g_opt.planes_mfma_waves = value;
     return 0;
   }
+  if (!strcmp(name, "wgrad5_pipeline")) {
+    if (value != 0 && value != 1) return itcv::fail("%s: wgrad5_pipeline takes 0 or 1 (got %lld)", "itcv_set_option", value);
+    itcv::g_opt.wgrad5_pipeline = value;
+    return 0;
+  }
+  if (!strcmp(name, "finish_in_kernel")) {
+    if (value != 0 && value != 1) return itcv::fail("%s: finish_in_kernel takes 0 or 1 (got %lld)", "itcv_set_option", value);
+    itcv::g_finish_in_kernel = value;
+    return 0;
+  }
   if (!strcmp(name, "sw_lds_rows")) {
     if (value < 0 || value > 4096) return itcv::fail("%s: sw_lds_rows takes 0..4096 (got %lld)", "itcv_set_option", value);
     itcv::g_sw_lds_rows = value;
@@ -80,6 +126,8 @@
   if (name && !strcmp(name, "band_persist_blocks")) return itcv::g_opt.band_persist_blocks;
   if (name && !strcmp(name, "wgrad_m16")) return itcv::g_opt.wgrad_m16;
   if (name && !strcmp(name, "planes_mfma_waves")) return itcv::g_opt.planes_mfma_waves;
+  if (name && !strcmp(name, "wgrad5_pipeline")) return itcv::g_opt.wgrad5_pipeline;
+  if (name && !strcmp(name, "finish_in_kernel")) return itcv::g_finish_in_kernel;
   if (name && !strcmp(name, "sw_lds_rows")) return itcv::g_sw_lds_rows;
   if (name && !strcmp(name, "sw_max_blocks")) return itcv::g_sw_max_blocks;
   return -1;
diff --git a/intro-tc-vae_amd/csrc/common.h b/intro-tc-vae_amd/csrc/common.h
--- a/intro-tc-vae_amd/csrc/common.h
+++ b/intro-tc-vae_amd/csrc/common.h
@@ -95,6 +95,39 @@
   for (int i = 0; i < nw; ++i) r += scratch[i];
   return r;
 }
+
+__device__ __forceinline__ bool finish_arrive(unsigned* counter, unsigned blocks) {
+  __shared__ unsigned last;
+  asm volatile("s_waitcnt vmcnt(0)" ::: "memory");
+  __syncthreads();
+  if (threadIdx.x == 0) {
+    __builtin_amdgcn_fence(__ATOMIC_RELEASE, "agent");
+    asm volatile("s_waitcnt vmcnt(0)" ::: "memory");
+    const unsigned t = __hip_atomic_fetch_add(counter, 1u, __ATOMIC_RELAXED, __HIP_MEMORY_SCOPE_AGENT);
+    last = t == blocks - 1;
+    if (t == blocks - 1) {
+      __hip_atomic_store(counter, 0u, __ATOMIC_RELAXED, __HIP_MEMORY_SCOPE_AGENT);
+      __builtin_amdgcn_fence(__ATOMIC_ACQUIRE, "agent");
+      asm volatile("s_waitcnt vmcnt(0)" ::: "memory");
+    }
+  }
+  __syncthreads();
+  return last != 0;
+}
+__device__ __forceinline__ bool finish_arrive_ticket(unsigned* counter, unsigned blocks) {
+  __shared__ unsigned last;
+  asm volatile("s_waitcnt vmcnt(0) lgkmcnt(0)" ::: "memory");
+  __syncthreads();
+  if (threadIdx.x == 0) {
+    const unsigned t = __hip_atomic_fetch_add(counter, 1u, __ATOMIC_RELAXED, __HIP_MEMORY_SCOPE_AGENT);
+    last = t == blocks - 1;
+    if (t == blocks - 1) __hip_atomic_store(counter, 0u, __ATOMIC_RELAXED, __HIP_MEMORY_SCOPE_AGENT);
+  }
+  __syncthreads();
+  return last != 0;
+}
+constexpr int kFinishRing = 4096, kFinishCaptured = 61440, kFinishMaxRun = 1024;
+unsigned* finish_slots(hipStream_t st, int n);
 
 __device__ __forceinline__ __amdgpu_buffer_rsrc_t make_rsrc(const void* p, uint32_t num_bytes) {
   return __builtin_amdgcn_make_buffer_rsrc(const_cast<void*>(p), 0, num_bytes, 0x00020000);
diff --git a/intro-tc-vae_amd/csrc/conv_igemm.hip b/intro-tc-vae_amd/csrc/conv_igemm.hip
--- a/intro-tc-vae_amd/csrc/conv_igemm.hip
+++ b/intro-tc-vae_amd/csrc/conv_igemm.hip
@@ -1694,7 +1694,7 @@
   }
 }
 
-template <int SG, bool F16 = false>
+template <int SG, bool F16 = false, int PIPE = 0>
 __global__ __launch_bounds__(256) void conv_wgrad5_planes_kernel(const float* __restrict__ sm, const u32x4* __restrict__ tp,
                                                                 float* __restrict__ slab, int B, int CS, int H, int W,
                                                                 int rows_per_job, int njobs, size_t plane_stride,
@@ -1724,6 +1724,106 @@
 #pragma unroll
     for (int nt = 0; nt < 4; ++nt) acc[dh][nt] = f32x4_t{0.f, 0.f, 0.f, 0.f};
 
+  if constexpr (PIPE != 0) {
+    constexpr int NH = PIPE, TQ = 16 / NH;
+    const int wu = __builtin_amdgcn_readfirstlane(wv);
+    const int ju = blockIdx.x * 4 + wu, bu = ju / jobs_per_img;
+    const int hu_lo = (ju - bu * jobs_per_img) * rows_per_job, hu_hi = min(H, hu_lo + rows_per_job);
+    const int segw = NH == 2 ? 64 : W;
+    const __amdgpu_buffer_rsrc_t srs = make_rsrc(sm, (uint32_t)((size_t)B * CS * HW * 4));
+    const __amdgpu_buffer_rsrc_t trs[2] = {make_rsrc(tp + (size_t)bu * 8 * HW, (uint32_t)(8 * HW * 16)),
+                                           make_rsrc(tp + plane_stride + (size_t)bu * 8 * HW, (uint32_t)(8 * HW * 16))};
+    const uint32_t tvo = (uint32_t)min(lane, segw - 1) * 16;
+    u32x4 tn[16];
+    float sa[5][8], sb[5][8];
+    auto load_t = [&](int first, int hh, int sg) {
+#pragma unroll
+      for (int i = first; i < first + TQ; ++i) {
+        const uint32_t soff = (uint32_t)(((i & 7) * (int)HW + hh * W + sg) * 16);
+        tn[i] = __builtin_bit_cast(u32x4, __builtin_amdgcn_raw_buffer_load_b128(trs[i >> 3], tvo, __builtin_amdgcn_readfirstlane(soff), 0));
+      }
+    };
+    auto load_s = [&](float (&s)[5][8], int hh, int col0) {
+      const int ws0 = col0 + 8 * kg + SG * (dw - 2);
+      uint32_t vo[8];
+#pragma unroll
+      for (int j = 0; j < 8; ++j)
+        vo[j] = (row_used && (unsigned)(ws0 + j) < (unsigned)W) ? (uint32_t)(cs * (int)HW + ws0 + j) * 4 : kOobBase;
+#pragma unroll
+      for (int dh = 0; dh < 5; ++dh) {
+        const int hs = hh + SG * (dh - 2);
+        const bool hok = (unsigned)hs < (unsigned)H;
+        const uint32_t soff = (uint32_t)((bu * CS * H + (hok ? hs : hh)) * W) * 4, bad = hok ? 0u : kOobBase;
+#pragma unroll
+        for (int j = 0; j < 8; ++j) s[dh][j] = buf_load_s(srs, vo[j] | bad, soff);
+      }
+    };
+    auto mfma_half = [&](const float (&s)[5][8], int w0) {
+      bf16x8 bfr[4][2];
+#pragma unroll
+      for (int nt = 0; nt < 4; ++nt)
+#pragma unroll
+        for (int pl = 0; pl < 2; ++pl) {
+          const uint32_t ad = rbase + (uint32_t)(((pl * 8 + 2 * nt + (pp >> 1)) * PXS + w0 + 8 * kg + q) * 16 + (pp & 1) * 8);
+          tr_read8(bfr[nt][pl], ad, ad + 64);
+        }
+#pragma unroll
+      for (int dh = 0; dh < 5; ++dh) {
+        u32x4 ap[2];
+        split8<2, F16>(s[dh], ap, sscale);
+        const bf16x8 a0 = __builtin_bit_cast(bf16x8, ap[0]), a1 = __builtin_bit_cast(bf16x8, ap[1]);
+#pragma unroll
+        for (int nt = 0; nt < 4; ++nt) {
+          f32x4_t c = acc[dh][nt];
+          c = mma16x16x32<F16>(a0, bfr[nt][1], c);
+          c = mma16x16x32<F16>(a1, bfr[nt][0], c);
+          c = mma16x16x32<F16>(a0, bfr[nt][0], c);
+          acc[dh][nt] = c;
+        }
+      }
+    };
+    int h = hu_lo, seg = 0;
+#pragma unroll
+    for (int part = 0; part < NH; ++part) load_t(part * TQ, h, 0);
+    load_s(sa, h, 0);
+    auto step = [&](float (&cur)[5][8], float (&nxt)[5][8]) {
+      int hn = h, segn = seg + 64;
+      if (segn >= W) hn = h + 1, segn = 0;
+      const bool last = hn >= hu_hi;
+      const int hc = last ? h : hn, segc = last ? seg : segn;
+      asm volatile("s_waitcnt lgkmcnt(0)" ::: "memory");
+      if (NH == 2 || lane < segw) {
+#pragma unroll
+        for (int i = 0; i < 16; ++i) rows[wv][i * PXS + lane] = tn[i];
+      }
+      asm volatile("s_waitcnt lgkmcnt(0)" ::: "memory");
+      if constexpr (NH == 2) {
+        load_s(nxt, h, seg + 32);
+        load_t(0, hc, segc);
+        load_t(TQ, hc, segc);
+        __builtin_amdgcn_sched_barrier(0);
+        mfma_half(cur, 0);
+        __builtin_amdgcn_sched_barrier(0);
+        load_s(cur, hc, segc);
+        __builtin_amdgcn_sched_barrier(0);
+        mfma_half(nxt, 32);
+      } else {
+        load_s(nxt, hc, segc);
+        load_t(0, hc, segc);
+        __builtin_amdgcn_sched_barrier(0);
+        mfma_half(cur, 0);
+        __builtin_amdgcn_sched_barrier(0);
+#pragma unroll
+        for (int dh = 0; dh < 5; ++dh)
+#pragma unroll
+          for (int j = 0; j < 8; ++j) cur[dh][j] = nxt[dh][j];
+      }
+      h = hn, seg = segn;
+      return last;
+    };
+    while (!step(sa, sb)) {
+    }
+  } else
   for (int h = h_lo; h < h_hi; ++h) {
    for (int seg = 0; seg < W; seg += 64) {
     const int segw = min(64, W - seg);
@@ -2076,8 +2176,8 @@
   }
 }
 
-__global__ __launch_bounds__(256) void bias_grad_partial(const float* __restrict__ dy, double* __restrict__ part, int B,
-                                                         int C, int HW, int splits) {
+__device__ __forceinline__ void bias_grad_partial_block(const float* __restrict__ dy, double* part, int B, int C, int HW,
+                                                        int splits) {
   __shared__ double scratch[4];
   const int c = blockIdx.x, s = blockIdx.y;
   const size_t total = (size_t)B * HW;
@@ -2091,12 +2191,26 @@
   acc = block_sum(acc, scratch);
   if (threadIdx.x == 0) part[(size_t)s * C + c] = acc;
 }
+__device__ __forceinline__ void bias_grad_combine_one(const double* part, float* db, int c, int C, int splits,
+                                                      int accumulate) {
+  const double s = fold_strided(0.0, part + c, (size_t)C, splits);
+  db[c] = (accumulate ? db[c] : 0.f) + (float)s;
+}
+__global__ __launch_bounds__(256) void bias_grad_partial(const float* __restrict__ dy, double* __restrict__ part, int B,
+                                                         int C, int HW, int splits) {
+  bias_grad_partial_block(dy, part, B, C, HW, splits);
+}
 __global__ void bias_grad_combine(const double* __restrict__ part, float* __restrict__ db, int C, int splits,
                                   int accumulate) {
   const int c = blockIdx.x * blockDim.x + threadIdx.x;
   if (c >= C) return;
-  const double s = fold_strided(0.0, part + c, (size_t)C, splits);
-  db[c] = (accumulate ? db[c] : 0.f) + (float)s;
+  bias_grad_combine_one(part, db, c, C, splits, accumulate);
+}
+__global__ __launch_bounds__(256) void bias_grad_fused(const float* __restrict__ dy, double* part, float* db, int B, int C,
+                                                       int HW, int splits, int accumulate, unsigned* counter) {
+  bias_grad_partial_block(dy, part, B, C, HW, splits);
+  if (!finish_arrive(counter, gridDim.x * gridDim.y)) return;
+  for (int c = threadIdx.x; c < C; c += 256) bias_grad_combine_one(part, db, c, C, splits, accumulate);
 }
 
 static inline int pad_to(int c, int m) { return (c + m - 1) / m * m; }
@@ -3052,11 +3166,15 @@
   const size_t plane_stride = (size_t)B * 8 * H * W;
   {
     ProfScope prof(st, kProfWgrad5, 5, Cs, stem ? 1 : 0, ns, 2.0 * B * H * W * 64.0 * Cs * 25);
+    const bool fits = (size_t)B * Cs * H * W * sizeof(float) < ((size_t)1 << 31);
+    const int pipe = !g_opt.wgrad5_pipeline || !fits ? 0 : W == 32 ? 1 : W % 64 == 0 ? 2 : 0;
     pick<2>(stem ? 1 : 0, [&](auto stem_c) {
       pick<2>(f16 ? 1 : 0, [&](auto f16_c) {
-        launch_timed((conv_wgrad5_planes_kernel<(stem_c.value ? 1 : -1), f16_c.value != 0>), dim3(cdiv(njobs, 4)), dim3(256), 0,
-                     st, small, static_cast<const u32x4*>(big_planes), static_cast<float*>(ws), B, Cs, H, W, rpj, njobs,
-                     plane_stride, small_amax);
+        pick<3>(pipe, [&](auto pipe_c) {
+          launch_timed((conv_wgrad5_planes_kernel<(stem_c.value ? 1 : -1), f16_c.value != 0, pipe_c.value>),
+                       dim3(cdiv(njobs, 4)), dim3(256), 0, st, small, static_cast<const u32x4*>(big_planes),
+                       static_cast<float*>(ws), B, Cs, H, W, rpj, njobs, plane_stride, small_amax);
+        });
       });
     });
   }
@@ -3089,6 +3207,12 @@
   const int splits = bias_splits(B, C, HW);
   ITCV_REQUIRE(ws && ws_bytes >= (size_t)splits * C * sizeof(double), "itcv_bias_grad(workspace)");
   double* part = static_cast<double*>(ws);
+  if (unsigned* counter = finish_slots(S(stream), 1)) {
+    hipLaunchKernelGGL(bias_grad_fused, dim3(C, splits), dim3(256), 0, S(stream), dy, part, db, B, C, HW, splits, accumulate,
+                       counter);
+    ITCV_CHECK_LAUNCH("itcv_bias_grad");
+    return 0;
+  }
   hipLaunchKernelGGL(bias_grad_partial, dim3(C, splits), dim3(256), 0, S(stream), dy, part, B, C, HW, splits);
   ITCV_CHECK_LAUNCH("itcv_bias_grad");
   hipLaunchKernelGGL(bias_grad_combine, dim3(cdiv(C, 256)), dim3(256), 0, S(stream), part, db, C, splits, accumulate);
diff --git a/intro-tc-vae_amd/csrc/conv_shared.h b/intro-tc-vae_amd/csrc/conv_shared.h
--- a/intro-tc-vae_amd/csrc/conv_shared.h
+++ b/intro-tc-vae_amd/csrc/conv_shared.h
@@ -93,6 +93,7 @@
   int band_persist_blocks = 256;
   int wgrad_m16 = 1;
   int planes_mfma_waves = 8;
+  int wgrad5_pipeline = 1;
 };
 extern Options g_opt;
 inline int band_m16() { return g_opt.band_m16; }
diff --git a/intro-tc-vae_amd/csrc/latent.hip b/intro-tc-vae_amd/csrc/latent.hip
--- a/intro-tc-vae_amd/csrc/latent.hip
+++ b/intro-tc-vae_amd/csrc/latent.hip
@@ -157,10 +157,10 @@
 __device__ __forceinline__ float prior_lp(float zz) { return logdens<false>(zz, 0.f); }
 
 template <bool MWS>
-__global__ __launch_bounds__(256) void tc_fwd_finish_kernel(const float* __restrict__ pmax, const float* __restrict__ psum,
-                                                            const float* __restrict__ sjoint, float* __restrict__ prodm,
-                                                            float* __restrict__ logqz, float* __restrict__ lse, int Bt, int D,
-                                                            int nch, TcConst c, TcKlOut kk, TcFullOut ff) {
+__device__ __forceinline__ void tc_fwd_finish_block(const float* __restrict__ pmax, const float* __restrict__ psum,
+                                                    const float* __restrict__ sjoint, float* __restrict__ prodm,
+                                                    float* __restrict__ logqz, float* __restrict__ lse, int Bt, int D,
+                                                    int nch, const TcConst& c, const TcKlOut& kk, const TcFullOut& ff) {
   __shared__ float red[4];
   const int j = blockIdx.x, tid = threadIdx.x, lane = tid & 63, wid = tid >> 6;
   float prod_acc = 0.f;
@@ -220,13 +220,39 @@
   }
 }
 
-__global__ __launch_bounds__(256) void rows_reduce_kernel(const float* __restrict__ rows, float* __restrict__ out, int B,
-                                                         int mean, float scale) {
+template <bool MWS>
+__global__ __launch_bounds__(256) void tc_fwd_finish_kernel(const float* __restrict__ pmax, const float* __restrict__ psum,
+                                                            const float* __restrict__ sjoint, float* __restrict__ prodm,
+                                                            float* __restrict__ logqz, float* __restrict__ lse, int Bt, int D,
+                                                            int nch, TcConst c, TcKlOut kk, TcFullOut ff) {
+  tc_fwd_finish_block<MWS>(pmax, psum, sjoint, prodm, logqz, lse, Bt, D, nch, c, kk, ff);
+}
+
+__device__ __forceinline__ void rows_reduce_block(const float* rows, float* out, int B, int mean, float scale) {
   __shared__ double red[4];
   double a = 0.0;
   for (int j = threadIdx.x; j < B; j += 256) a += (double)rows[j];
   a = block_sum(a, red);
   if (threadIdx.x == 0) out[0] = scale * (float)(mean ? a / (double)B : a);
+}
+__global__ __launch_bounds__(256) void rows_reduce_kernel(const float* __restrict__ rows, float* __restrict__ out, int B,
+                                                         int mean, float scale) {
+  rows_reduce_block(rows, out, B, mean, scale);
+}
+struct TcRowsReduce {
+  const float* rows;
+  float* out;
+  int mean;
+  unsigned* counter;
+};
+template <bool MWS>
+__global__ __launch_bounds__(256) void tc_fwd_finish_reduce_kernel(const float* __restrict__ pmax, const float* __restrict__ psum,
+                                                                   const float* __restrict__ sjoint, float* __restrict__ prodm,
+                                                                   float* __restrict__ logqz, float* __restrict__ lse, int Bt,
+                                                                   int D, int nch, TcConst c, TcKlOut kk, TcFullOut ff,
+                                                                   TcRowsReduce rr) {
+  tc_fwd_finish_block<MWS>(pmax, psum, sjoint, prodm, logqz, lse, Bt, D, nch, c, kk, ff);
+  if (finish_arrive(rr.counter, gridDim.x)) rows_reduce_block(rr.rows, rr.out, (int)gridDim.x, rr.mean, 1.f);
 }
 
 struct TcGrad {
@@ -668,7 +694,7 @@
 static int tc_fwd_impl(const float* z, const float* mu_all, const float* logvar, float* prodm, float* logqz, float* lse,
                        float* sjoint, int Bl, int Bt, int row_offset, int D, int64_t dataset_size, int flags, void* ws,
                        size_t ws_bytes, const TcKlOut& kk, void* stream, int ldm = 0, float* ivar = nullptr,
-                       const TcFullOut& ff = TcFullOut{}) {
+                       const TcFullOut& ff = TcFullOut{}, TcRowsReduce* reduce = nullptr) {
   ITCV_REQUIRE(z && mu_all && logvar && prodm && logqz && lse && sjoint && Bl > 0 && D > 0, "itcv_tc_fwd");
   ITCV_REQUIRE(row_offset >= 0 && row_offset + Bl <= Bt, "itcv_tc_fwd(rows must lie inside the global batch)");
   if (D > 64 * kTcDLMax) return fail("%s: latent size %lld > 512 is not supported", "itcv_tc_fwd", D);
@@ -714,6 +740,15 @@
 #undef ITCV_TC_DL
 #undef ITCV_TC_PART
   ITCV_CHECK_LAUNCH("itcv_tc_fwd(partials)");
+  if (reduce && reduce->rows && (reduce->counter = finish_slots(st, 1))) {
+    if (mws)
+      hipLaunchKernelGGL(tc_fwd_finish_reduce_kernel<true>, dim3(Bl), block, 0, st, pmax, psum, sjoint, prodm, logqz, lse, Bt, D, nch, c, kk, ff, *reduce);
+    else
+      hipLaunchKernelGGL(tc_fwd_finish_reduce_kernel<false>, dim3(Bl), block, 0, st, pmax, psum, sjoint, prodm, logqz, lse, Bt, D, nch, c, kk, ff, *reduce);
+    ITCV_CHECK_LAUNCH("itcv_tc_fwd(finish)");
+    reduce->rows = nullptr;
+    return 0;
+  }
   if (mws)
     hipLaunchKernelGGL(tc_fwd_finish_kernel<true>, dim3(Bl), block, 0, st, pmax, psum, sjoint, prodm, logqz, lse, Bt, D, nch, c, kk, ff);
   else
@@ -735,10 +770,11 @@
   ITCV_REQUIRE(out && (reduction == 0 || rows) && reduction >= 0 && reduction <= 2, "itcv_tc_kl_fwd");
   ITCV_REQUIRE(mu_all && row_offset >= 0 && row_offset + Bl <= Bt, "itcv_tc_kl_fwd(rows must lie inside the global batch)");
   const TcKlOut kk{mu_all + (size_t)row_offset * D, logvar, reduction == 0 ? out : rows, coef_tc, coef_kl};
+  TcRowsReduce rr{reduction ? rows : nullptr, out, reduction == 2 ? 1 : 0, nullptr};
   if (int e = tc_fwd_impl(z, mu_all, logvar, prodm, logqz, lse, sjoint, Bl, Bt, row_offset, D, dataset_size, ITCV_TC_LIVE, ws,
-                          ws_bytes, kk, stream))
+                          ws_bytes, kk, stream, 0, nullptr, TcFullOut{}, &rr))
     return e;
-  if (reduction) {
+  if (rr.rows) {
     hipLaunchKernelGGL(rows_reduce_kernel, dim3(1), dim3(256), 0, S(stream), rows, out, Bl, reduction == 2 ? 1 : 0, 1.f);
     ITCV_CHECK_LAUNCH("itcv_tc_kl_fwd(reduce)");
   }
diff --git a/intro-tc-vae_amd/csrc/loss_optim.hip b/intro-tc-vae_amd/csrc/loss_optim.hip
--- a/intro-tc-vae_amd/csrc/loss_optim.hip
+++ b/intro-tc-vae_amd/csrc/loss_optim.hip
@@ -6,9 +6,8 @@
 namespace itcv {
 
 template <int LT>
-__global__ __launch_bounds__(256) void recon_partial_kernel(const float* __restrict__ x,
-                                                           const float* __restrict__ recon,
-                                                           double* __restrict__ part, size_t P, int splits, int vec4) {
+__device__ __forceinline__ void recon_partial_block(const float* __restrict__ x, const float* __restrict__ recon,
+                                                    double* part, size_t P, int splits, int vec4) {
   __shared__ double scratch[4];
   const int b = blockIdx.x, s = blockIdx.y;
   size_t beg, end;
@@ -17,6 +16,12 @@
   acc = block_sum(acc, scratch);
   if (threadIdx.x == 0) part[(size_t)b * splits + s] = acc;
 }
+template <int LT>
+__global__ __launch_bounds__(256) void recon_partial_kernel(const float* __restrict__ x,
+                                                           const float* __restrict__ recon,
+                                                           double* __restrict__ part, size_t P, int splits, int vec4) {
+  recon_partial_block<LT>(x, recon, part, P, splits, vec4);
+}
 __global__ void recon_combine_kernel(const double* __restrict__ part, float* __restrict__ rows, int B, int splits) {
   const int b = blockIdx.x * blockDim.x + threadIdx.x;
   if (b >= B) return;
@@ -29,8 +34,8 @@
     drecon[i] = g[i / P] * rec_derr<LT>(recon[i], x[i]);
 }
 
-__global__ __launch_bounds__(256) void recon_finish_kernel(const double* __restrict__ part, float* __restrict__ out, int B,
-                                                          int splits, int reduction, float scale) {
+__device__ __forceinline__ void recon_finish_block(const double* part, float* out, int B, int splits, int reduction,
+                                                   float scale) {
   __shared__ double scratch[4];
   double acc = 0.0;
   for (int b = threadIdx.x; b < B; b += 256) {
@@ -41,6 +46,17 @@
   if (reduction == 0) return;
   acc = block_sum(acc, scratch);
   if (threadIdx.x == 0) out[0] = scale * (float)(reduction == 2 ? acc / (double)B : acc);
+}
+__global__ __launch_bounds__(256) void recon_finish_kernel(const double* __restrict__ part, float* __restrict__ out, int B,
+                                                          int splits, int reduction, float scale) {
+  recon_finish_block(part, out, B, splits, reduction, scale);
+}
+template <int LT>
+__global__ __launch_bounds__(256) void recon_loss_fused_kernel(const float* __restrict__ x, const float* __restrict__ recon,
+                                                              double* part, float* out, size_t P, int splits, int vec4,
+                                                              int reduction, float scale, unsigned* counter) {
+  recon_partial_block<LT>(x, recon, part, P, splits, vec4);
+  if (finish_arrive(counter, gridDim.x * gridDim.y)) recon_finish_block(part, out, (int)gridDim.x, splits, reduction, scale);
 }
 template <int LT>
 __global__ void recon_loss_bwd_kernel(const float* __restrict__ x, const float* __restrict__ recon,
@@ -88,9 +104,29 @@
   if (k < a.n) grads[k] = g[0] * a.weight[k];
 }
 
+static bool recon_vec4(const float* x, const float* recon, size_t P) {
+  return (P & 3) == 0 && (((uintptr_t)x | (uintptr_t)recon) & 15) == 0;
+}
+static bool launch_recon_fused(const float* x, const float* recon, double* part, float* out, int B, size_t P, int splits,
+                               int loss_type, int reduction, float scale, unsigned* counter, hipStream_t st) {
+  const int vec4 = recon_vec4(x, recon, P);
+  dim3 grid(B, splits);
+  if (loss_type == ITCV_LOSS_MSE)
+    hipLaunchKernelGGL(recon_loss_fused_kernel<ITCV_LOSS_MSE>, grid, dim3(256), 0, st, x, recon, part, out, P, splits, vec4,
+                       reduction, scale, counter);
+  else if (loss_type == ITCV_LOSS_L1)
+    hipLaunchKernelGGL(recon_loss_fused_kernel<ITCV_LOSS_L1>, grid, dim3(256), 0, st, x, recon, part, out, P, splits, vec4,
+                       reduction, scale, counter);
+  else if (loss_type == ITCV_LOSS_BCE)
+    hipLaunchKernelGGL(recon_loss_fused_kernel<ITCV_LOSS_BCE>, grid, dim3(256), 0, st, x, recon, part, out, P, splits, vec4,
+                       reduction, scale, counter);
+  else
+    return false;
+  return true;
+}
 static bool launch_recon_partial(const float* x, const float* recon, double* part, int B, size_t P, int splits,
                                  int loss_type, hipStream_t st) {
-  const int vec4 = (P & 3) == 0 && (((uintptr_t)x | (uintptr_t)recon) & 15) == 0;
+  const int vec4 = recon_vec4(x, recon, P);
   dim3 grid(B, splits);
   if (loss_type == ITCV_LOSS_MSE)
     hipLaunchKernelGGL(recon_partial_kernel<ITCV_LOSS_MSE>, grid, dim3(256), 0, st, x, recon, part, P, splits, vec4);
@@ -103,8 +139,7 @@
   return true;
 }
 
-__global__ __launch_bounds__(256) void sumsq_partial_kernel(const float* __restrict__ x, size_t n,
-                                                           double* __restrict__ part) {
+__device__ __forceinline__ void sumsq_partial_block(const float* __restrict__ x, size_t n, double* part) {
   __shared__ double scratch[4];
   double acc = 0.0;
   const size_t n4 = n / 4;
@@ -117,13 +152,25 @@
   acc = block_sum(acc, scratch);
   if (threadIdx.x == 0) part[blockIdx.x] = acc;
 }
-__global__ __launch_bounds__(256) void sumsq_final_kernel(const double* __restrict__ part, int nparts,
-                                                         double* __restrict__ out) {
+__device__ __forceinline__ void sumsq_final_block(const double* part, int nparts, double* out) {
   __shared__ double scratch[4];
   double acc = 0.0;
   for (int i = threadIdx.x; i < nparts; i += 256) acc += part[i];
   acc = block_sum(acc, scratch);
   if (threadIdx.x == 0) out[0] = acc;
+}
+__global__ __launch_bounds__(256) void sumsq_partial_kernel(const float* __restrict__ x, size_t n,
+                                                           double* __restrict__ part) {
+  sumsq_partial_block(x, n, part);
+}
+__global__ __launch_bounds__(256) void sumsq_final_kernel(const double* __restrict__ part, int nparts,
+                                                         double* __restrict__ out) {
+  sumsq_final_block(part, nparts, out);
+}
+__global__ __launch_bounds__(256) void sumsq_fused_kernel(const float* __restrict__ x, size_t n, double* part, double* out,
+                                                         unsigned* counter) {
+  sumsq_partial_block(x, n, part);
+  if (finish_arrive(counter, gridDim.x)) sumsq_final_block(part, (int)gridDim.x, out);
 }
 __global__ void clip_coef_kernel(const double* sumsq, int nparts, double clip, float* norm_out, float* coef_out) {
   double s = 0.0;
@@ -157,10 +204,9 @@
     p[i] -= step_size * (mi / (sqrtf(vi) / sqrt_bc2 + eps));
   }
 }
-__global__ void adam_dev_kernel(float* __restrict__ p, const float* __restrict__ g, float* __restrict__ m,
-                                float* __restrict__ v, size_t n, float lr, float b1, float b2, float eps,
-                                const int* __restrict__ step_dev) {
-  const int step = step_dev[0] + 1;
+__device__ __forceinline__ void adam_dev_block(float* __restrict__ p, const float* __restrict__ g, float* __restrict__ m,
+                                               float* __restrict__ v, size_t n, float lr, float b1, float b2, float eps,
+                                               int step) {
   const double bc1 = 1.0 - pow((double)b1, (double)step), bc2 = 1.0 - pow((double)b2, (double)step);
   const float step_size = (float)((double)lr / bc1), sqrt_bc2 = (float)sqrt(bc2);
   for (size_t i = (size_t)blockIdx.x * blockDim.x + threadIdx.x; i < n; i += (size_t)gridDim.x * blockDim.x) {
@@ -172,7 +218,20 @@
     p[i] -= step_size * (mi / (sqrtf(vi) / sqrt_bc2 + eps));
   }
 }
+__global__ void adam_dev_kernel(float* __restrict__ p, const float* __restrict__ g, float* __restrict__ m,
+                                float* __restrict__ v, size_t n, float lr, float b1, float b2, float eps,
+                                const int* __restrict__ step_dev) {
+  adam_dev_block(p, g, m, v, n, lr, b1, b2, eps, step_dev[0] + 1);
+}
 __global__ void bump_step_kernel(int* step_dev) { step_dev[0] += 1; }
+__global__ __launch_bounds__(256) void adam_dev_bump_kernel(float* __restrict__ p, const float* __restrict__ g,
+                                                           float* __restrict__ m, float* __restrict__ v, size_t n, float lr,
+                                                           float b1, float b2, float eps, int* step_dev,
+                                                           unsigned* counter) {
+  const int step = step_dev[0] + 1;
+  adam_dev_block(p, g, m, v, n, lr, b1, b2, eps, step);
+  if (finish_arrive_ticket(counter, gridDim.x) && threadIdx.x == 0) step_dev[0] = step;
+}
 
 __global__ void hflip_kernel(const float* __restrict__ x, float* __restrict__ y, const unsigned char* __restrict__ flip,
                              size_t rows_per_image, int W, size_t n) {
@@ -240,6 +299,12 @@
   ITCV_REQUIRE(ws && ws_bytes >= (size_t)B * splits * sizeof(double), "itcv_recon_loss_fwd(workspace)");
   double* part = static_cast<double*>(ws);
   hipStream_t st = S(stream);
+  if (unsigned* counter = finish_slots(st, 1)) {
+    if (!launch_recon_fused(x, recon, part, out, B, P, splits, loss_type, reduction, scale, counter, st))
+      return fail("%s: unknown loss type %lld", "itcv_recon_loss_fwd", loss_type);
+    ITCV_CHECK_LAUNCH("itcv_recon_loss_fwd");
+    return 0;
+  }
   if (!launch_recon_partial(x, recon, part, B, P, splits, loss_type, st))
     return fail("%s: unknown loss type %lld", "itcv_recon_loss_fwd", loss_type);
   ITCV_CHECK_LAUNCH("itcv_recon_loss_fwd");
@@ -315,7 +380,12 @@
   int blocks = stream_grid(n, 4);
   if (blocks > kSumsqBlocks) blocks = kSumsqBlocks;
   double* part = static_cast<double*>(ws);
-  hipLaunchKernelGGL(sumsq_partial_kernel, dim3(blocks), dim3(256), 0, S(stream), x, n, part);
+  if (unsigned* counter = finish_slots(S(stream), 1)) {
+    hipLaunchKernelGGL(sumsq_fused_kernel, dim3(blocks), dim3(256), 0, S(stream), x, n, part, out, counter);
+    ITCV_CHECK_LAUNCH("itcv_sumsq");
+    return 0;
+  }
+  hipLaunchKernelGGL(sumsq_partial_kernel,dim3(blocks), dim3(256), 0, S(stream), x, n, part);
   ITCV_CHECK_LAUNCH("itcv_sumsq");
   hipLaunchKernelGGL(sumsq_final_kernel, dim3(1), dim3(256), 0, S(stream), part, blocks, out);
   ITCV_CHECK_LAUNCH("itcv_sumsq(final)");
@@ -354,7 +424,13 @@
                        float eps, int* step_dev, void* stream) {
   ITCV_REQUIRE(p && g && m && v && step_dev, "itcv_adam_step_dev");
   if (!n) return 0;
-  hipLaunchKernelGGL(adam_dev_kernel, dim3(stream_grid(n, 1)), dim3(256), 0, S(stream), p, g, m, v, n, lr, beta1, beta2,
+  if (unsigned* counter = finish_slots(S(stream), 1)) {
+    hipLaunchKernelGGL(adam_dev_bump_kernel, dim3(stream_grid(n, 1)), dim3(256), 0, S(stream), p, g, m, v, n, lr, beta1,
+                       beta2, eps, step_dev, counter);
+    ITCV_CHECK_LAUNCH("itcv_adam_step_dev");
+    return 0;
+  }
+  hipLaunchKernelGGL(adam_dev_kernel,dim3(stream_grid(n, 1)), dim3(256), 0, S(stream), p, g, m, v, n, lr, beta1, beta2,
                      eps, step_dev);
   ITCV_CHECK_LAUNCH("itcv_adam_step_dev");
   hipLaunchKernelGGL(bump_step_kernel, dim3(1), dim3(1), 0, S(stream), step_dev);
```
